# RomanJuranek/librectify

Hardware: AMD Instinct MI355X
Metric: Mpix/s end-to-end (detect+VP) on 4K frames, batch call of 64 frames, 5 in flight (higher is better)
Workload: dtype f32

## Files before the change

### include/librectify_amd.h

```cpp
#pragma once
#include <stddef.h>
#include <stdint.h>

#include "librectify.h"

#if defined(__GNUC__)
#pragma GCC visibility push(default)
#endif

#ifdef __cplusplus
using librectify::ImageTransform;
using librectify::LineSegment;
using librectify::Point;
using librectify::RectificationConfig;
extern "C" {
#endif

typedef struct lr_context lr_context;
enum lr_pixel_format { LR_PIX_U8 = 0, LR_PIX_U8X3 = 1, LR_PIX_F32 = 2 };

int lr_context_create(int device, lr_context** out);
void lr_context_destroy(lr_context* ctx);
void lr_release_thread_context(void);
int lr_context_trim(lr_context* ctx);
// ... 89 lines not shown
                                      d_dst, dst_bytes, 0, 0, 0);
}
static inline size_t lr_jpeg_bound(int width, int height, int format, int layout) {
    size_t mcu, bpm, ri, mcus;
    if (width < 1 || height < 1 || width > 65535 || height > 65535) return 0;
    if (format == LR_PIX_U8 && layout == 0) {
        mcu = 8; bpm = 1; ri = 96;
    } else if (format == LR_PIX_U8X3 && layout == 0) {
        mcu = 16; bpm = 6; ri = 16;
    } else if (format == LR_PIX_U8X3 && layout == 1) {
        mcu = 8; bpm = 3; ri = 32;
    } else {
        return 0;
    }
    mcus = (((size_t)width + mcu - 1) / mcu) * (((size_t)height + mcu - 1) / mcu);
    return 640 + 2 * ((mcus + ri - 1) / ri) + 416 * mcus * bpm;
}

typedef struct lr_jpeg_decode_args {
    const void* h_src;
    const double* frames;
    int32_t* info;
} lr_jpeg_decode_args;
enum lr_warp_jpeg_decode { LR_WARP_JPEG_DECODE = 0x4000 };
static inline int lr_decode_jpeg_device(lr_context* ctx, const void* d_src, const void* h_src, size_t src_bytes, int format,
                                        const double* frames, int batch, void* d_dst, size_t dst_bytes, int32_t* info) {
    lr_jpeg_decode_args a;
    a.h_src = h_src;
    a.frames = frames;
    a.info = info;
    return lr_warp_perspective_device(ctx, d_src, src_bytes, batch, 0, 0, 0, format | LR_WARP_JPEG_DECODE,
                                      (const double*)(const void*)&a, d_dst, dst_bytes, 0, 0, 0);
}
static inline int lr_jpeg_info(const void* h_src, size_t src_bytes, const double* frames, int batch, int32_t* info) {
    return lr_decode_jpeg_device((lr_context*)0, (const void*)0, h_src, src_bytes, LR_PIX_U8X3, frames, batch, (void*)0, 0, info);
}

int lr_stage_filter(lr_context* ctx, const float* d_image, int width, int height, int stride);
int lr_stage_filter_host(lr_context* ctx, const float* buffer, int width, int height, int stride);
int lr_stage_seeds(lr_context* ctx, int* n_seeds);
int lr_stage_flood(lr_context* ctx, int* n_components);
int lr_stage_fit(lr_context* ctx, LineSegment* out, int capacity, int* n_lines);

enum lr_buffer_id {
    LR_BUF_DX = 0,
    LR_BUF_DY = 1,
    LR_BUF_DMASK = 2,
    LR_BUF_LABEL = 3,
    LR_BUF_SEED_IDX = 4,
    LR_BUF_SEED_BIN = 5,
    LR_BUF_SEED_THR = 6,
    LR_BUF_MAXMAG = 7,
    LR_BUF_SEED_SIZE = 8,
};
int lr_download(lr_context* ctx, int buffer_id, void* dst, size_t bytes);

enum lr_stage_id {
    LR_T_UPLOAD = 0,
    LR_T_FILTER = 1,
    LR_T_SEEDS = 2,
    LR_T_FLOOD = 3,
    LR_T_FIT = 4,
    LR_T_RANSAC = 5,
    LR_T_TOTAL = 6,
    LR_T_FILTER_KERNEL = 7,
    LR_T_COUNT = 8,
};
int lr_stage_times(lr_context* ctx, float* ms, int count);
void lr_set_stage_timing(lr_context* ctx, int on);
int lr_filter_kernel_ms(lr_context* ctx, float* ms);
int lr_stage_counters(lr_context* ctx, int64_t* out, int count);

int lr_ransac_best(lr_context* ctx, const LineSegment* lines_norm, int n, const int32_t* indices, int n_idx, float tol,
                   int n_iter, uint64_t seed, uint32_t round, float* best_h3, float* best_score, int* best_iter);
int lr_estimate_line_pencils(lr_context* ctx, LineSegment* lines, int n, int max_models, float inlier_deg,
                             float garbage_deg, int n_iter, uint64_t seed);

int lr_cht_vanishing_point(lr_context* ctx, const LineSegment* lines, int n, int d, Point* vp, uint64_t* acc_out);
int lr_refine_lines(lr_context* ctx, const LineSegment* in, int n, LineSegment* out, int* n_out);

void lr_set_estimator(lr_context* ctx, int kind, int param);
int lr_estimate_line_pencils_cht(lr_context* ctx, LineSegment* lines, int n, int max_models, float inlier_deg,
                                 float garbage_deg, int d, float* models3, int* n_models, uint32_t* peak_cells,
                                 uint64_t* votes);
int lr_ht_weights(lr_context* ctx, const LineSegment* lines_norm, int n, const int32_t* indices, int n_idx, float* weights);
int lr_prosac_solve(lr_context* ctx, const LineSegment* lines_norm, int n, const int32_t* indices, int n_idx, float tol,
                    int T_N, uint64_t seed, uint32_t round, float* h3, int32_t* trace4);
int lr_estimate_line_pencils_prosac(lr_context* ctx, LineSegment* lines, int n, int max_models, float inlier_deg,
                                    float garbage_deg, int T_N, uint64_t seed);
int lr_direct_solve(lr_context* ctx, const LineSegment* lines_norm, int n, const int32_t* indices, int n_idx, float* h3);
int lr_estimate_line_pencils_direct(lr_context* ctx, LineSegment* lines, int n, int max_models, float inlier_deg,
                                    float garbage_deg);

#ifdef __cplusplus
}
#endif

#if defined(__GNUC__)
#pragma GCC visibility pop
#endif
```

### librectify_amd/__init__.py

```python
import ctypes as C
import os

import numpy as np

_HERE = os.path.dirname(os.path.abspath(__file__))
LIB_PATH = os.path.join(_HERE, "librectify_amd.so")

LINE_DTYPE = np.dtype(
    [("x1", "<f4"), ("y1", "<f4"), ("x2", "<f4"), ("y2", "<f4"), ("weight", "<f4"), ("err", "<f4"), ("group_id", "<i4")]
)


class Point(C.Structure):
    _fields_ = [("x", C.c_float), ("y", C.c_float), ("z", C.c_float)]


class ImageTransform(C.Structure):
    _fields_ = [
        ("width", C.c_int),
        ("height", C.c_int),
        ("top_left", Point),
        ("top_right", Point),
        ("bottom_left", Point),
        ("bottom_right", Point),
        ("horizontal_vp", Point),
        ("vertical_vp", Point),
    ]

    def as_array(self):
        pts = [self.top_left, self.top_right, self.bottom_left, self.bottom_right, self.horizontal_vp, self.vertical_vp]
        return np.array([[p.x, p.y, p.z] for p in pts], np.float32)


ROTATE_H, ROTATE_V, RECTIFY, KEEP = 0, 1, 2, 3


class RectificationConfig(C.Structure):
    _fields_ = [
        ("vertical_vp_angular_tolerance", C.c_float),
        ("vertical_vp_min_distance", C.c_float),
        ("v_strategy", C.c_int),
        ("horizontal_vp_min_distance", C.c_float),
        ("h_strategy", C.c_int),
    ]

    def __init__(self, tol=40.0, vmin=1.5, v_strategy=RECTIFY, hmin=1.5, h_strategy=RECTIFY):
        super().__init__(tol, vmin, v_strategy, hmin, h_strategy)


class Frame(C.Structure):
    _fields_ = [("data", C.c_void_p), ("width", C.c_int32), ("height", C.c_int32), ("stride", C.c_int32),
                ("min_length", C.c_float)]


class DrawLinesArgs(C.Structure):
    _fields_ = [("lines", C.c_void_p), ("n_lines", C.c_size_t), ("frames", C.c_void_p), ("H", C.c_void_p)]


class JpegArgs(C.Structure):
    _fields_ = [("frames", C.c_void_p), ("sizes", C.c_void_p)]


class JpegDecodeArgs(C.Structure):
    _fields_ = [("h_src", C.c_void_p), ("frames", C.c_void_p), ("info", C.c_void_p)]


BUF_DX, BUF_DY, BUF_DMASK, BUF_LABEL, BUF_SEED_IDX, BUF_SEED_BIN, BUF_SEED_THR, BUF_MAXMAG, BUF_SEED_SIZE = range(9)
T_UPLOAD, T_FILTER, T_SEEDS, T_FLOOD, T_FIT, T_RANSAC, T_TOTAL, T_FILTER_KERNEL, T_COUNT = range(9)
PIX_U8, PIX_U8X3, PIX_F32 = range(3)
WARP_PREPARE = 0x100
WARP_PACKED = 0x200
WARP_RAGGED = 0x800
WARP_LINES = 0x1000
WARP_JPEG = 0x2000
WARP_JPEG_DECODE = 0x4000
JPEG_OK, JPEG_NOT_JPEG, JPEG_UNSUPPORTED, JPEG_SIZE_MISMATCH, JPEG_DAMAGED = range(5)
FRAMES_U8, FRAMES_U8X3, FRAMES_F32 = 0x100, 0x200, 0x300


def frames_word(fmt, refine=False):
    if fmt not in (PIX_U8, PIX_U8X3, PIX_F32):
        raise ValueError("frames_word: fmt is PIX_U8, PIX_U8X3 or PIX_F32")
    flag = 1 if refine else 0
    return flag if fmt == PIX_F32 else ((fmt + 1) << 8) | flag


def split_frames_word(word):
    word = int(word)
    if word >= 0 and 1 <= (word >> 8) <= 3:
        return (word >> 8) - 1, (word & 0xFF) != 0
    return PIX_F32, word != 0

EXPORTS = [
    "find_line_segment_groups", "release_line_segments", "compute_rectification_transform",
    "compute_rectification_transform_from_vp", "fit_vanishing_point", "assign_to_group",
    "lr_context_create", "lr_context_destroy", "lr_last_error", "lr_synchronize", "lr_set_ransac_seed",
    "lr_set_ransac_iterations", "lr_set_flood_mode", "lr_device_count", "lr_find_line_segment_groups_device",
    "lr_find_line_segment_groups_host", "lr_find_line_segment_groups_batch_device", "lr_stage_filter",
    "lr_stage_filter_host", "lr_stage_seeds", "lr_stage_flood", "lr_stage_fit", "lr_download", "lr_stage_times",
    "lr_stage_counters", "lr_filter_kernel_ms", "lr_ransac_best", "lr_estimate_line_pencils",
    "lr_find_line_segment_groups_batch_host", "lr_find_line_segment_groups_batch_host_ptrs", "lr_host_alloc", "lr_host_free",
    "lr_set_seed_capacity", "lr_set_flood_blind_rounds", "lr_set_flood_staged", "lr_set_batch_streams", "lr_device_malloc", "lr_device_free", "lr_memcpy_h2d", "lr_cht_vanishing_point", "lr_refine_lines", "lr_set_estimator", "lr_ht_weights", "lr_prosac_solve", "lr_estimate_line_pencils_prosac", "lr_direct_solve", "lr_estimate_line_pencils_direct",
    "lr_estimate_line_pencils_cht", "lr_set_stage_timing", "lr_release_thread_context", "lr_set_flood_partial_commits", "lr_set_flood_logs", "lr_set_flood_just_in_time", "lr_set_flood_giant_step", "lr_context_trim", "lr_trim_thread_context",
    "lr_find_line_segment_groups_batch_host_multi", "lr_memcpy_d2h", "lr_rectification_homography", "lr_warp_perspective_device",
]

_lib = None


class LibrectifyError(RuntimeError):
    pass


def lib():
    global _lib
    if _lib is None:
        if not os.path.exists(LIB_PATH):
            raise LibrectifyError(
                "librectify_amd.so is missing: build it with `python -m librectify_amd.build` (hipcc, gfx950); "
                "there is no CPU fallback"
# ... 348 lines not shown
        lib().lr_set_ransac_seed(self._h, C.c_uint64(seed))

    def set_iterations(self, n):
        lib().lr_set_ransac_iterations(self._h, int(n))

    def set_flood_mode(self, mode):
        lib().lr_set_flood_mode(self._h, int(mode))

    def synchronize(self):
        _check(lib().lr_synchronize(self._h))

    def stage_filter_host(self, img):
        img = np.ascontiguousarray(img, np.float32)
        h, w = img.shape
        self.shape = (h, w)
        _check(lib().lr_stage_filter_host(self._h, _ptr(img), w, h, w))

    def stage_filter_device(self, dptr, w, h, stride=None):
        self.shape = (h, w)
        _check(lib().lr_stage_filter(self._h, C.c_void_p(dptr), w, h, stride or w))

    def stage_seeds(self):
        n = C.c_int(0)
        _check(lib().lr_stage_seeds(self._h, C.byref(n)))
        self.n_seeds = n.value
        return n.value

    def stage_flood(self):
        n = C.c_int(0)
        _check(lib().lr_stage_flood(self._h, C.byref(n)))

    def stage_fit(self):
        h, w = self.shape
        cap = h * w // 6 + 16
        out = np.zeros(cap, LINE_DTYPE)
        n = C.c_int(0)
        _check(lib().lr_stage_fit(self._h, _ptr(out), cap, C.byref(n)))
        return out[: n.value].copy()

    def download(self, buf):
        h, w = self.shape
        if buf in (BUF_DX, BUF_DY):
            a = np.zeros((h, w), np.float32)
        elif buf == BUF_DMASK:
            a = np.zeros((h, w), np.uint8)
        elif buf == BUF_LABEL:
            a = np.zeros((h, w), np.int32)
        elif buf in (BUF_SEED_IDX, BUF_SEED_BIN, BUF_SEED_SIZE):
            a = np.zeros(self.n_seeds, np.int32)
        elif buf == BUF_SEED_THR:
            a = np.zeros(self.n_seeds, np.float32)
        elif buf == BUF_MAXMAG:
            a = np.zeros(1, np.float32)
        else:
            raise ValueError(buf)
        if a.nbytes:
            _check(lib().lr_download(self._h, buf, _ptr(a), a.nbytes))
        return a

    def stage_times(self):
        t = np.zeros(T_COUNT, np.float32)
        _check(lib().lr_stage_times(self._h, _ptr(t), T_COUNT))
        return t

    def stage_times_partial(self):
        ms = C.c_float(0)
        _check(lib().lr_filter_kernel_ms(self._h, C.byref(ms)))
        return ms.value

    def stage_counters(self):
        c = np.zeros(16, np.int64)
        _check(lib().lr_stage_counters(self._h, _ptr(c), 16))
        return dict(seeds=int(c[0]), components=int(c[1]), flood_rounds=int(c[2]), labelled_px=int(c[3]),
                    second_tier_seeds=int(c[4]), slabs=int(c[5]), ordered_tail_seeds=int(c[6]), frame_laps=int(c[7]),
                    walked_px=int(c[8]), walk_steps=int(c[9]), log_rewalks=int(c[11]), log_give_ups=int(c[12]), giants_held=int(c[13]), giant_steps=int(c[14]),
                    quiet_round_misses=int(c[15]))

    def find_line_segment_groups(self, img, min_length, refine=False, num_threads=-1, capacity=None):
        img, fmt, _, stride = _host_frame(img, "find_line_segment_groups")
        h, w = img.shape[:2]
        cap = capacity or (h * w // 6 + 16)
        out = np.zeros(cap, LINE_DTYPE)
        n = C.c_int(0)
        self.shape = (h, w)
        _check(lib().lr_find_line_segment_groups_host(self._h, _ptr(img), w, h, stride, min_length, frames_word(fmt, refine), num_threads, _ptr(out), cap, C.byref(n)))
        return out[: min(n.value, cap)].copy()

    def find_line_segment_groups_device(self, dptr, w, h, min_length, refine=False, stride=None, capacity=None, out=None, fmt=PIX_F32):
        cap = capacity or (h * w // 6 + 16)
        if out is None:
            out = np.zeros(cap, LINE_DTYPE)
        n = C.c_int(0)
        self.shape = (h, w)
        _check(lib().lr_find_line_segment_groups_device(self._h, C.c_void_p(dptr), w, h, stride or w, min_length, frames_word(fmt, refine), -1, _ptr(out), cap, C.byref(n)))
        return out[: min(n.value, cap)]

    def device_upload(self, array):
        a = np.ascontiguousarray(array)
        p = C.c_void_p()
        _check(lib().lr_device_malloc(self._h, a.nbytes, C.byref(p)))
        _check(lib().lr_memcpy_h2d(self._h, p, _ptr(a), a.nbytes))
        return p.value

    def device_free(self, ptr):
        _check(lib().lr_device_free(self._h, C.c_void_p(ptr)))

# ... 793 lines not shown
```

### librectify_amd/csrc/api.cpp

```cpp
#include <cstdio>
#include <cstdlib>
#include <cstring>
#include <memory>
#include <new>
#include <stdexcept>
#include <string>

#include "context.h"

using namespace lramd;

namespace {

struct CtxDeleter {
    void operator()(lr_context* c) const { ctx_destroy(c); }
};

std::unique_ptr<lr_context, CtxDeleter>& thread_context_slot() {
    thread_local std::unique_ptr<lr_context, CtxDeleter> ctx;
    return ctx;
}

lr_context* thread_context() {
    std::unique_ptr<lr_context, CtxDeleter>& ctx = thread_context_slot();
// ... 404 lines not shown
            set_error("image smaller than the 5x5 filter");
            return 1;
        }
        if (upload_host_image(ctx, buffer, width, height, stride, -1)) return 1;
        return ctx_stage_filter(ctx, ctx->frames.slot[0], width, height, width);
    } catch (...) {
        return guard_fail("lr_stage_filter_host");
    }
}
int lr_stage_seeds(lr_context* ctx, int* n_seeds) {
    try {
        if (ctx_stage_seeds(ctx)) return 1;
        if (n_seeds) *n_seeds = (int)ctx->n_seeds;
        return 0;
    } catch (...) {
        return guard_fail("lr_stage_seeds");
    }
}
int lr_stage_flood(lr_context* ctx, int* n_components) {
    try {
        if (ctx_stage_flood(ctx)) return 1;
        LR_HIP(hipStreamSynchronize(ctx->stream));
        if (n_components) *n_components = -1;
        return 0;
    } catch (...) {
        return guard_fail("lr_stage_flood");
    }
}
int lr_stage_fit(lr_context* ctx, LineSegment* out, int capacity, int* n_lines) {
    try {
        std::vector<LineSegment> res;
        if (ctx_stage_fit(ctx, res)) return 1;
        return copy_out(res, out, capacity, n_lines);
    } catch (...) {
        return guard_fail("lr_stage_fit");
    }
}

int lr_download(lr_context* ctx, int buffer_id, void* dst, size_t bytes) {
    try {
        const size_t npix = (size_t)ctx->w * ctx->h;
        const void* src = nullptr;
        size_t have = 0;
        switch (buffer_id) {
            case LR_BUF_DX: src = ctx->ws.dx; have = npix * 4; break;
            case LR_BUF_DY: src = ctx->ws.dy; have = npix * 4; break;
            case LR_BUF_DMASK: src = ctx->ws.dmask; have = npix; break;
            case LR_BUF_LABEL: src = ctx->ws.label; have = npix * 4; break;
            case LR_BUF_SEED_IDX: src = ctx->ws.seed_idx; have = (size_t)ctx->n_seeds * 4; break;
            case LR_BUF_SEED_BIN: src = ctx->ws.seed_bin; have = (size_t)ctx->n_seeds * 4; break;
            case LR_BUF_SEED_THR: src = ctx->ws.seed_thr; have = (size_t)ctx->n_seeds * 4; break;
            case LR_BUF_MAXMAG: src = ctx->maxmag; have = 4; break;
            case LR_BUF_SEED_SIZE: src = ctx->ws.seed_size; have = (size_t)ctx->n_seeds * 4; break;
            default: set_error("lr_download: unknown buffer id"); return 1;
        }
        if (buffer_id == LR_BUF_DMASK && ctx->dmask_consumed) {
            set_error("lr_download: LR_BUF_DMASK was consumed by lr_stage_flood (labelled pixels are cleared); download it after lr_stage_filter");
            return 1;
        }
        if (bytes > have) {
            set_error("lr_download: request larger than the buffer");
            return 1;
        }
        LR_HIP(hipSetDevice(ctx->device));
        LR_HIP(hipStreamSynchronize(ctx->stream));
        LR_HIP(hipMemcpy(dst, src, bytes, hipMemcpyDeviceToHost));
        return 0;
    } catch (...) {
        return guard_fail("lr_download");
    }
}

int lr_filter_kernel_ms(lr_context* ctx, float* ms) {
    try {
        LR_HIP(hipStreamSynchronize(ctx->stream));
        LR_HIP(hipEventElapsedTime(ms, ctx->ev[0], ctx->ev[1]));
        return 0;
    } catch (...) {
        return guard_fail("lr_filter_kernel_ms");
    }
}

int lr_stage_times(lr_context* ctx, float* ms, int count) {
    try {
        for (int i = 0; i < count && i < LR_T_COUNT; ++i) ms[i] = ctx->stage_ms[i];
        return 0;
    } catch (...) {
        return guard_fail("lr_stage_times");
    }
}

int lr_stage_counters(lr_context* ctx, int64_t* out, int count) {
    try {
        const int64_t v[16] = {(int64_t)ctx->n_seeds,        (int64_t)ctx->n_comp,         (int64_t)ctx->flood_rounds,
                               (int64_t)ctx->n_px,           (int64_t)ctx->flood_tiers[0], (int64_t)ctx->flood_tiers[1],
                               (int64_t)ctx->flood_tiers[2], (int64_t)ctx->frame_laps,
                               (int64_t)(((uint64_t)ctx->flood_tiers[5] << 32) | ctx->flood_tiers[4]),
                               (int64_t)(((uint64_t)ctx->flood_tiers[7] << 32) | ctx->flood_tiers[6]),
                               0 , (int64_t)ctx->flood_tiers[10], (int64_t)ctx->flood_tiers[11], (int64_t)ctx->flood_tiers[12],
                               (int64_t)ctx->flood_tiers[13], (int64_t)ctx->flood_tiers[15]};
        for (int i = 0; i < count && i < 16; ++i) out[i] = v[i];
        return 0;
    } catch (...) {
        return guard_fail("lr_stage_counters");
    }
}
// ... 162 lines not shown
```

### librectify_amd/csrc/common.h

```cpp
#pragma once
#include <hip/hip_runtime.h>

#include <cstdint>
#include <string>

#include "../../include/librectify_amd.h"

namespace lramd {

constexpr float kEps = 1e-6f;
constexpr int kMaxModels = 4;
constexpr int kMaxPeelModels = 5;
constexpr float kInlierDeg = 2.0f;
constexpr float kGarbageDeg = 4.0f;
constexpr int kRansacMaxIter = 10000;
constexpr int kEdgeKernelSize = 2;
constexpr float kEdgeKernelSigma = 1.0f;
constexpr int kSeedDist = 2;
constexpr float kSeedRatio = 0.95f;
constexpr float kTraceTolerance = 0.25f;
constexpr float kLineMaxErr = 2.0f;
constexpr float kLineMinLength = 5.f;
constexpr int kComponentMinSize = 5;
constexpr int kBins = 8;
// ... 22 lines not shown
__host__ __device__ inline float directional(float dx, float dy, float s, float c) {
    return fabsf(fmaf(dx, s, dy * c));
}

__host__ __device__ inline uint64_t splitmix64(uint64_t x) {
    x += 0x9E3779B97F4A7C15ull;
    x = (x ^ (x >> 30)) * 0xBF58476D1CE4E5B9ull;
    x = (x ^ (x >> 27)) * 0x94D049BB133111EBull;
    return x ^ (x >> 31);
}
__host__ __device__ inline void sample_pair(uint64_t seed, uint32_t round, uint32_t iter, uint32_t n, uint32_t& a,
                                            uint32_t& b) {
    const uint64_t z = splitmix64(seed ^ splitmix64(((uint64_t)round << 32) | iter));
    const uint32_t u1 = (uint32_t)z, u2 = (uint32_t)(z >> 32);
    const uint32_t i = (uint32_t)(((uint64_t)u1 * n) >> 32);
    uint32_t j = (uint32_t)(((uint64_t)u2 * (n - 1)) >> 32);
    if (j >= i) ++j;
    a = i < j ? i : j;
    b = i < j ? j : i;
}

void set_error(const std::string& msg);

#define LR_HIP(expr)                                                                                     \
    do {                                                                                                 \
        hipError_t _e = (expr);                                                                          \
        if (_e != hipSuccess) {                                                                          \
            (void)hipGetLastError();        \
            ::lramd::set_error(std::string(#expr) + ": " + hipGetErrorString(_e) + " (" + __FILE__ + ":" + \
                               std::to_string(__LINE__) + ")");                                          \
            return 1;                                                                                    \
        }                                                                                                \
    } while (0)

inline int pix_bytes(int format) { return format == LR_PIX_U8 ? 1 : format == LR_PIX_U8X3 ? 3 : format == LR_PIX_F32 ? 4 : 0; }
int launch_filter(const void* img, int format, int w, int h, int stride, const FilterConsts& fc, float* dx, float* dy,
                  uint8_t* dmask, uint64_t* cand, uint32_t* cand_count, uint32_t* tile_max, hipStream_t s);
int filter_band_rows();
int filter_band_last_row(int by);
int launch_filter_rows(const void* img, int format, int w, int h, int stride, const FilterConsts& fc, float* dx, float* dy,
                       uint8_t* dmask, uint64_t* cand, uint32_t* cand_count, uint32_t* tile_max, int by_begin, int by_end,
                       hipStream_t s);
struct FilterGeom {
    int n_tiles;
    int cand_cap;
};
FilterGeom filter_geometry(int w, int h);

size_t seeds_temp_bytes(int n_tiles, size_t max_seeds);
int launch_seed_select(const uint64_t* cand, const uint32_t* cand_count, const uint32_t* tile_max, int n_tiles,
                       int cand_cap, float seed_keep_ratio, float* maxmag, uint32_t* tile_pass, uint32_t* tile_off, uint64_t* keys,
                       uint32_t key_cap, uint32_t* n_seeds, uint32_t frame_tag, hipStream_t s);
int launch_seed_order(uint64_t* keys, uint64_t* keys_alt, const uint32_t* n_seeds, uint32_t cap, const float* dx, const float* dy,
                      BinTrig trig, float trace_tolerance, int32_t* seed_idx, int32_t* seed_bin, float* seed_thr, hipStream_t s);

int launch_label_init(uint32_t* label, size_t n, hipStream_t s);
int launch_flood_ordered(const float* dx, const float* dy, const uint8_t* dmask, int w, int h, const int32_t* seed_idx,
                         const int32_t* seed_bin, const float* seed_thr, const uint32_t* d_n_seeds, uint32_t seed_cap,
                         BinTrig trig, uint32_t* label, int32_t* seed_size, int32_t* queue, hipStream_t s);

constexpr size_t kFloodHandWords = 1024;
struct FloodBuffers {
    uint32_t* blocked = nullptr;
    uint32_t* count = nullptr;
    uint32_t* flags = nullptr;
    uint8_t* state = nullptr;
    uint8_t* tier = nullptr;
    uint32_t* blk = nullptr;
    uint32_t* act_a = nullptr;
    uint32_t* act_b = nullptr;
    uint32_t* ctrl = nullptr;
    uint8_t* dirty = nullptr;
    uint32_t* big_list = nullptr;
    uint32_t* handover = nullptr;
    bool rewalk_logs = false;
    uint32_t* rewalk_list = nullptr;
    int log_min_tiles = 0, log_walk_tiles = 0;
    bool giant_hold = false;
    bool giant_step = true;
    void* giant_mask = nullptr;
    uint32_t* giant_parent = nullptr;
    bool log_sweep = false;
    bool rewalk_big = false;
    uint32_t log_seeds = 0, log_cap = 0;
    uint32_t* log_off = nullptr;
    uint32_t* log_len = nullptr;
    uint32_t* log_buf = nullptr;
    void* slab_ring = nullptr;
    void* slab_hash = nullptr;
    uint32_t n_slabs = 0, slab_ring_cap = 0, slab_hash_cap = 0;
    int win_first_shift = 0, win_growth = 2;
    int win_hold_pct = 80;
    bool partial_commits = true;
    bool second_tier = true;
    bool second_tier_from_start = true;
    bool hold_from_start = false;
    bool staged_from_start = false;
    int blind_rounds = 10;
    uint32_t* host_progress = nullptr;
    bool calm_hint = false;
    uint32_t* host_ctrl = nullptr;
    int jit_first = 0;
    int jit_sleep_us = 0;
    uint32_t big_cap_override = 0;
    uint32_t team_tile_cap = 0;
};
struct FloodFrame {
    const float* dx;
    const float* dy;
    const uint8_t* dmask;
    int w, h;
    const int32_t* seed_idx;
    const int32_t* seed_bin;
    const float* seed_thr;
    const uint32_t* d_n_seeds;
    uint32_t seed_cap;
    BinTrig trig;
    uint32_t* label;
    int32_t* seed_size;
    int32_t* queue;
};
struct FloodProgress {
    int enqueued = 0;
    bool use_big = false;
    int win_growth = 2;
    bool sizes_known = false;
    uint32_t max_flood = 0;
};
constexpr int kFloodCtrlWords = 56;
int flood_enqueue(const FloodBuffers& B, const FloodFrame& F, FloodProgress* P, uint32_t* h_ctrl, hipStream_t s);
int flood_finish(const FloodBuffers& B, const FloodFrame& F, FloodProgress* P, uint32_t* h_ctrl, int* rounds_out,
                 uint32_t* tiers_out ,
                 bool* extra, hipStream_t s);

size_t fit_temp_bytes(size_t max_pixels, uint32_t max_segments);
struct HugeSort {
    uint32_t* tab = nullptr;
    uint32_t* list = nullptr;
    uint32_t* jobs = nullptr;
    uint32_t max = 0;
};
int launch_component_offsets(const int32_t* seed_size, const uint32_t* d_n_seeds, uint32_t seed_cap, int min_size,
                             uint32_t* comp_rank, uint32_t* comp_seed, uint32_t* comp_off,
                             uint32_t* totals , uint32_t* large_list, uint32_t large_cap,
                             uint32_t* n_large, void* temp, size_t temp_bytes, uint32_t frame_tag, uint32_t* cursor, const HugeSort& hs,
                             hipStream_t s);
int launch_component_scatter(const uint32_t* label, size_t npix, const uint32_t* comp_rank, const uint32_t* comp_off,
                             uint32_t* cursor, uint32_t* px, const HugeSort& hs, uint32_t* n_large, bool with_huge, hipStream_t s);
int launch_component_sort(const uint32_t* px_in, uint32_t* px_out, const uint32_t* comp_off, const uint32_t* d_n_comp,
                          uint32_t comp_cap, const uint32_t* large_list, uint32_t large_cap, const uint32_t* n_large,
                          uint32_t* scratch, const uint32_t* cursor, const HugeSort& hs, bool with_huge, hipStream_t s);
int launch_fit(const uint32_t* px_sorted, const uint32_t* px_unsorted, const uint32_t* comp_off, const uint32_t* comp_seed, const uint32_t* d_n_comp,
               uint32_t comp_cap, const int32_t* seed_bin, const float* dx, const float* dy, int w, BinTrig trig,
               float* scratch_w, LineSegment* out, const uint32_t* cursor, const HugeSort& hs, const uint32_t* n_large, bool with_huge,
               hipStream_t s);

struct PencilSoA {
    const float* ax;
    const float* ay;
    const float* dx;
    const float* dy;
    const float* len;
    const float* hx;
    const float* hy;
    const float* hz;
};
constexpr int kRansacBestSlots = 32;
int launch_ransac_score(PencilSoA m, uint32_t n, float tol, float degeneracy_tol, uint32_t n_iter, uint64_t seed,
                        uint32_t round, unsigned long long* best_slots, uint32_t* host_best, hipStream_t s);
int launch_ransac_score_dev(PencilSoA m, const uint32_t* gctl, int max_models, float tol, float degeneracy_tol,
                            uint32_t n_iter, uint64_t seed, unsigned long long* best_slots, hipStream_t s);

struct PencilTable {
// ... 45 lines not shown
```

### librectify_amd/csrc/context.h

```cpp
#pragma once
#include <atomic>
#include <functional>
#include <memory>
#include <mutex>
#include <vector>

#include "buffers.h"
#include "common.h"
#include "vp_host.h"

namespace lramd {
struct StagingCrew;

struct Settings {
    uint64_t ransac_seed = 0;
    int ransac_iters = kRansacMaxIter;
    int estimator = 0;
    int prosac_T_N = -1;
    int cht_d = 128;
    int batch_streams = 5;
    int flood_mode = 1;
    bool flood_giant_step = true;
    bool flood_jit = true;
    bool flood_partial = true;
    bool flood_log_sweep = false;
    bool flood_logs = true;
    bool flood_staged = false;
    bool timing_on = false;
};


struct Workspace {
    size_t cap_pix = 0;
    int cap_tiles = 0;
    DeviceBuffer<float> dx, dy;
    DeviceBuffer<uint8_t> dmask;
    DeviceBuffer<uint64_t> cand;
    DeviceBuffer<uint32_t> cand_count, tile_max;
    DeviceBuffer<uint32_t> tile_pass;
    DeviceBuffer<uint32_t> tile_off;
    DeviceBuffer<uint64_t> keys_a, keys_b;
    DeviceBuffer<int32_t> seed_idx, seed_bin;
    DeviceBuffer<float> seed_thr;
    DeviceBuffer<int32_t> seed_size;
    DeviceBuffer<uint32_t> label;
    DeviceBuffer<int32_t> queue;
    DeviceBuffer<uint32_t> comp_rank, comp_seed, comp_off, cursor, px_a, px_b;
    DeviceBuffer<float> scratch_w;
    DeviceBuffer<LineSegment> d_lines;
    DeviceBuffer<unsigned char> temp;
    DeviceBuffer<uint32_t> comp_large;
    DeviceBuffer<uint32_t> huge_tab, huge_list, huge_jobs;
    HugeSort huge;
};

struct FloodStore {
    DeviceBuffer<uint32_t> blocked, count, flags, blk, act_a, act_b, ctrl, big_list, handover, rewalk_list, log_off, log_len, log_buf;
    DeviceBuffer<uint8_t> state, tier, dirty;
    DeviceBuffer<uint64_t> giant_mask;
    DeviceBuffer<uint4> slab_ring, slab_hash;
    FloodBuffers fb;
    size_t cap_seeds = 0;
};

struct FrameSlots {
    DeviceBuffer<float> slot[2];
    PinnedBuffer<float> stage[2];
    DeviceBuffer<float> packed;
    DeviceBuffer<float> luma;
};

struct UploadRing {
    std::vector<DeviceBuffer<float>> img;
    std::vector<PinnedBuffer<float>> stage;
    size_t cap_pix = 0, stage_cap_pix = 0;
    void drop() {
        for (auto& b : img) b.reset();
        for (auto& b : stage) b.reset();
        cap_pix = stage_cap_pix = 0;
    }
};

struct PrepareSpans {
    MirroredBuffer<unsigned char> spans;
    int key[4] = {0, 0, 0, 0};
    float w_in[2] = {0.f, 0.f};
    MirroredBuffer<unsigned char> ragged;
};

struct OverlayStore {
    MirroredBuffer<unsigned char> block;
};

struct JpegStore {
    MirroredBuffer<unsigned char> block;
    DeviceBuffer<int16_t> coef;
// ... 195 lines not shown
```

### librectify_amd/csrc/context.hip

```cpp
#include "host.h"

#include <cmath>
#include <cstdlib>

#ifndef M_PI
#define M_PI 3.14159265358979323846
#endif

lr_context::lr_context() = default;
lr_context::~lr_context() = default;

namespace lramd {

namespace {

thread_local std::string g_error;

void gauss_deriv_factors(int size, float sigma, float* d, float* g) {
    const int n = 2 * size + 1;
    for (int t = 0; t < n; ++t) {
        const float x = float(t - size);
        const float a = float(2 * M_PI * std::pow(sigma, 4.0f));
        const float e = std::exp(-std::pow(x, 2.0f) / (2 * std::pow(sigma, 2.0f)));
        d[t] = x / a * e;
// ... 27 lines not shown
    if (frames_too) {
        c->frames = FrameSlots{};
        c->ring.drop();
        c->prep = PrepareSpans{};
        c->warp_m = MirroredBuffer<double>{};
        c->overlay = OverlayStore{};
        c->jpeg = JpegStore{};
        c->jpeg_decode = JpegDecodeStore{};
    }
    c->small_frames = 0;
    c->w = c->h = 0;
    c->seed_cap = 0;
    c->flood_hold_hint = c->flood_staged_hint = c->flood_calm_hint = false;
    c->flood_staged_streak = 0;
    for (bool& v : c->stage_valid) v = false;
    if (frames_too)
        for (lr_context* wc : c->workers)
            if (ctx_trim(wc, true)) return 1;
    return 0;
}

int ctx_ensure_image_capacity(lr_context* c, int w, int h) {
    const size_t npix = (size_t)w * h;
    if (c->w != 0 && (c->w != w || c->h != h)) {
        c->flood_hold_hint = false;
        c->flood_staged_hint = false;
        c->flood_calm_hint = false;
        c->flood_staged_streak = 0;
    }
    const FilterGeom fg = filter_geometry(w, h);
    const int ntiles = fg.n_tiles;
    if (!c->keep_workspace) {
        if (c->ws.cap_pix != 0 && npix * 4 <= c->ws.cap_pix) {
            if (++c->small_frames >= 8 && ctx_trim(c, false)) return 1;
        } else {
            c->small_frames = 0;
        }
    }
    return ctx_reserve_workspace(c, npix, ntiles);
}

int ctx_reserve_workspace(lr_context* c, size_t npix, int ntiles) {
    const FilterGeom fg = filter_geometry(5, 5);
    if (npix <= c->ws.cap_pix && ntiles <= c->ws.cap_tiles) return 0;
    LR_HIP(hipStreamSynchronize(c->stream));
    const size_t cp = std::max(npix, c->ws.cap_pix);
    const int ct = std::max(ntiles, c->ws.cap_tiles);
    const size_t tile_off_words = std::max(ct, 2);
    Workspace& s = c->ws;
    s.cap_pix = 0;
    s.cap_tiles = 0;
    if (s.dx.grow(cp) || s.dy.grow(cp) || s.dmask.grow(cp + 16) || s.cand.grow((size_t)ct * fg.cand_cap) || s.cand_count.grow(ct) ||
        s.tile_max.grow(ct) || s.tile_pass.grow(ct) || s.tile_off.grow(tile_off_words) || s.keys_a.grow(cp) || s.keys_b.grow(cp) ||
        s.seed_idx.grow(cp) || s.seed_bin.grow(cp) || s.seed_thr.grow(cp) || s.seed_size.grow(cp) || s.label.grow(cp) ||
        s.queue.grow(cp) || s.comp_rank.grow(cp) || s.comp_seed.grow(cp) || s.comp_off.grow(cp + 1) || s.cursor.grow(cp) ||
        s.px_a.grow(cp) || s.px_b.grow(cp) || s.scratch_w.grow(cp) || s.d_lines.grow(cp / 6 + 16) || s.comp_large.grow(cp / 64 + 16))
        return 1;
    LR_HIP(hipMemsetAsync(s.tile_off, 0, tile_off_words * sizeof(uint32_t), c->stream));
    {
        const size_t nb = (cp + 16383) >> 14;
        const uint32_t max = 256;
        if (s.huge_tab.grow(max * nb) || s.huge_jobs.grow(4 * max * nb) || s.huge_list.grow(max)) return 1;
        s.huge = HugeSort{s.huge_tab, s.huge_list, s.huge_jobs, max};
        LR_HIP(hipMemsetAsync(s.huge.tab, 0, max * nb * sizeof(uint32_t), c->stream));
    }
    const size_t tb = std::max(seeds_temp_bytes(ct, cp), fit_temp_bytes(cp, (uint32_t)std::min<size_t>(cp / 6 + 16, 0xFFFFFFFFu)));
    if (s.temp.grow(tb)) return 1;
    LR_HIP(hipMemsetAsync(s.temp, 0, tb, c->stream));
    s.cap_pix = cp;
    s.cap_tiles = ct;
    return 0;
}

template <class T, class P>
static int grow_into(DeviceBuffer<T>& own, P*& raw, size_t count) {
    raw = nullptr;
    if (own.grow(count)) return 1;
    raw = own.get();
    return 0;
}

static int ensure_flood_slabs(lr_context* c) {
    FloodBuffers& f = c->flood.fb;
    static const bool giant_step_off = std::getenv("LIBRECTIFY_FLOOD_GIANT_STEP") && std::atoi(std::getenv("LIBRECTIFY_FLOOD_GIANT_STEP")) == 0;
    uint32_t want = (c->opt.flood_mode == 1 && c->opt.flood_giant_step && !giant_step_off) ? 16u : 128u;
    if (const char* e = std::getenv("LIBRECTIFY_FLOOD_SLABS")) want = (uint32_t)std::max(1, std::atoi(e));
    if (f.slab_ring && f.n_slabs >= want) return 0;
    LR_HIP(hipStreamSynchronize(c->stream));
    f.n_slabs = want;
    f.slab_ring_cap = 1u << 14;
    f.slab_hash_cap = 1u << 16;
    if (grow_into(c->flood.slab_ring, f.slab_ring, (size_t)f.n_slabs * f.slab_ring_cap) ||
        grow_into(c->flood.slab_hash, f.slab_hash, (size_t)f.n_slabs * f.slab_hash_cap * 2))
        return 1;
    LR_HIP(hipMemsetAsync(f.slab_hash, 0, (size_t)f.n_slabs * f.slab_hash_cap * 32, c->stream));
    if (f.ctrl) LR_HIP(hipMemsetAsync(f.ctrl, 0, kFloodCtrlWords * sizeof(uint32_t), c->stream));
    return 0;
}

int ensure_flood_buffers(lr_context* c) {
    FloodStore& o = c->flood;
    FloodBuffers& f = o.fb;
    if (c->flood.cap_seeds >= c->ws.cap_pix && f.ctrl) return ensure_flood_slabs(c);
    LR_HIP(hipStreamSynchronize(c->stream));
    const size_t cs = c->ws.cap_pix;
    if (grow_into(o.blocked, f.blocked, cs) || grow_into(o.count, f.count, cs) || grow_into(o.flags, f.flags, cs) ||
        grow_into(o.state, f.state, cs) || grow_into(o.tier, f.tier, cs) || grow_into(o.blk, f.blk, cs) ||
        grow_into(o.act_a, f.act_a, cs) || grow_into(o.act_b, f.act_b, cs) || grow_into(o.ctrl, f.ctrl, kFloodCtrlWords) ||
        grow_into(o.big_list, f.big_list, 8192) || grow_into(o.handover, f.handover, 8192 * kFloodHandWords) ||
        grow_into(o.dirty, f.dirty, cs / 256 + 16) ||
        grow_into(o.giant_mask, f.giant_mask, cs / 16 + 64))
        return 1;
    constexpr size_t kLogCapDiv = 8;
    f.log_seeds = (uint32_t)std::min<size_t>(std::max<size_t>(cs / 16, 4096), cs);
    f.log_cap = (uint32_t)std::min<size_t>(std::max<size_t>(cs / kLogCapDiv, 65536), 1u << 28);
    if (grow_into(o.rewalk_list, f.rewalk_list, 8192) || grow_into(o.log_off, f.log_off, f.log_seeds) ||
        grow_into(o.log_len, f.log_len, f.log_seeds) || grow_into(o.log_buf, f.log_buf, (size_t)f.log_cap * 3))
        return 1;
    LR_HIP(hipMemsetAsync(f.ctrl, 0, kFloodCtrlWords * sizeof(uint32_t), c->stream));
    o.cap_seeds = cs;
    return ensure_flood_slabs(c);
}


int ctx_ensure_ransac_capacity(lr_context* c, size_t n_lines) {
    if (8 * n_lines <= c->model.cap()) return 0;
    LR_HIP(hipStreamSynchronize(c->stream));
    return c->model.grow(8 * std::max<size_t>(n_lines, 4096));
}

int ensure_group_capacity(lr_context* c, size_t n_lines) {
    if (n_lines > c->cap_glines) {
        LR_HIP(hipStreamSynchronize(c->stream));
        const size_t cl = std::max<size_t>(n_lines, 4096);
        c->cap_glines = 0;
        if (c->d_tables.grow(3 * 8 * cl) || c->d_orig.grow(3 * cl) || c->d_inl.grow(4 * cl)) return 1;
        c->cap_glines = cl;
    }
    if (n_lines > c->d_flines.cap()) {
        LR_HIP(hipStreamSynchronize(c->stream));
        if (c->d_flines.grow(n_lines + 16)) return 1;
    }
    return 0;
}

int ctx_create(int device, lr_context** out) {
    int ndev = 0;
    if (hipGetDeviceCount(&ndev) != hipSuccess || ndev <= 0) {
        set_error("no HIP device available: librectify_amd has no CPU fallback");
        return 1;
    }
    if (device < 0 || device >= ndev) {
        set_error("device index out of range");
        return 1;
    }
    LR_HIP(hipSetDevice(device));
    lr_context* c = new lr_context();
    c->device = device;
    if (hipStreamCreateWithFlags(c->stream.put(), hipStreamNonBlocking) != hipSuccess) {
        delete c;
// ... 60 lines not shown
```

### librectify_amd/csrc/frame.hip

```cpp
#include "host.h"

#include <cstdio>
#include <cstdlib>
#include <cstring>

namespace lramd {


namespace {

uint32_t round_up(uint32_t v, uint32_t m) { return (v + m - 1) / m * m; }

uint32_t initial_seed_cap(size_t npix) {
    return (uint32_t)std::min<size_t>(npix, std::max<size_t>(round_up((uint32_t)(npix / 32), 1024), 4096));
}

uint32_t line_cap_for(const lr_context* c) {
    return (uint32_t)std::min<size_t>(c->seed_cap, c->ws.cap_pix / 6 + 16);
}


PencilTable table_of(lr_context* c, int which) {
    const size_t cl = c->cap_glines;
    float* b = c->d_tables + (size_t)which * 8 * cl;
// ... 3 lines not shown

int ensure_result_block(lr_context* c, size_t lines) {
    if (lines <= c->res_lines_cap && c->h_res) return 0;
    LR_HIP(hipStreamSynchronize(c->stream));
    if (c->h_res.grow(kResHeaderBytes + lines * sizeof(LineSegment))) return 1;
    c->res_lines_cap = lines;
    return 0;
}

FloodBuffers flood_buffers_for(lr_context* c) {
    FloodBuffers fbuf = c->flood.fb;
    if (c->opt.flood_mode >= 2 && c->opt.flood_mode <= 4) fbuf.second_tier = false;
    fbuf.second_tier_from_start = c->flood_big_hint;
    fbuf.hold_from_start = c->flood_hold_hint;
    fbuf.staged_from_start = c->flood_staged_hint;
    if (c->opt.flood_mode == 2) fbuf.n_slabs = 0;
    if (c->opt.flood_mode == 3) fbuf.n_slabs = 2;
    if (c->opt.flood_mode == 5) {
        fbuf.n_slabs = 0;
        fbuf.big_cap_override = 1;
    }
    if (c->opt.flood_mode == 6) fbuf.team_tile_cap = 200;
    if (c->opt.flood_mode == 7) {
        fbuf.team_tile_cap = 200;
        fbuf.n_slabs = 0;
    }
    static const bool partial_off = std::getenv("LIBRECTIFY_FLOOD_PARTIAL") && std::atoi(std::getenv("LIBRECTIFY_FLOOD_PARTIAL")) == 0;
    fbuf.partial_commits = !partial_off && c->opt.flood_partial;
    fbuf.rewalk_logs = c->opt.flood_logs;
    fbuf.log_sweep = c->opt.flood_log_sweep;
    fbuf.log_min_tiles = c->flood_log_min;
    fbuf.log_walk_tiles = c->flood_log_walk;
    fbuf.giant_hold = c->opt.flood_mode == 1;
    static const bool giant_step_off = std::getenv("LIBRECTIFY_FLOOD_GIANT_STEP") && std::atoi(std::getenv("LIBRECTIFY_FLOOD_GIANT_STEP")) == 0;
    fbuf.giant_step = !giant_step_off && c->opt.flood_giant_step;
    fbuf.giant_parent = reinterpret_cast<uint32_t*>(c->ws.queue.get());
    fbuf.rewalk_big = c->flood_logbig_hint && !c->flood_logbig_off;
    if (c->opt.flood_staged) fbuf.win_first_shift = 3;
    fbuf.blind_rounds = c->flood_rounds_hint;
    static const bool jit_off = std::getenv("LIBRECTIFY_FLOOD_JIT") && std::atoi(std::getenv("LIBRECTIFY_FLOOD_JIT")) == 0;
    static_assert(16 + kFloodCtrlWords <= 72, "the control block's copy ends where the report word begins");
    fbuf.host_progress = c->h_counts + 72;
    fbuf.host_ctrl = c->h_counts + 16;
    static const int calm_hint_env = std::getenv("LIBRECTIFY_FLOOD_CALM_HINT") ? std::atoi(std::getenv("LIBRECTIFY_FLOOD_CALM_HINT")) : 1;
    fbuf.calm_hint = calm_hint_env != 0 && c->flood_calm_hint;
    fbuf.jit_sleep_us = c->flood_jit_sleep_us;
    constexpr int kJitFirstMax = 4;
    fbuf.jit_first = (c->opt.flood_jit && !jit_off) ? std::min(c->flood_rounds_last > 0 ? std::max(c->flood_rounds_last - 1, 2) : 3, kJitFirstMax) : 0;
    return fbuf;
}

FloodFrame flood_frame_for(lr_context* c) {
    return FloodFrame{c->ws.dx, c->ws.dy, c->ws.dmask, c->w, c->h, c->ws.seed_idx, c->ws.seed_bin, c->ws.seed_thr,
                      c->d_counts + kCntSeeds, c->seed_cap, c->trig, c->ws.label, c->ws.seed_size, c->ws.queue};
}

int prepare_frame(lr_context* c, int w, int h) {
    LR_HIP(hipSetDevice(c->device));
    if (w < 5 || h < 5) {
        set_error("image smaller than the 5x5 filter");
        return 1;
    }
    if (ctx_ensure_image_capacity(c, w, h)) return 1;
    if (c->w != w || c->h != h || c->seed_cap == 0) c->seed_cap = initial_seed_cap((size_t)w * h);
    if (c->seed_cap_once) {
        c->seed_cap = (uint32_t)std::min<size_t>((size_t)w * h, c->seed_cap_once);
        c->seed_cap_once = 0;
    }
    c->w = w;
    c->h = h;
    c->n_seeds = c->n_comp = c->n_px = 0;
    c->dmask_consumed = false;
    for (bool& v : c->stage_valid) v = false;
    return 0;
}

int enqueue_filter(lr_context* c, const void* d_image, int format, int w, int h, int stride) {
    if (prepare_frame(c, w, h)) return 1;
    const size_t bpp = (size_t)pix_bytes(format);
    if (bpp == 0 || d_image == nullptr || stride < w) {
        set_error(bpp == 0 ? "unknown pixel format of the frames" : "launch_filter: bad geometry");
        return 1;
    }
    const size_t npix = (size_t)w * h;
    if (format == LR_PIX_U8X3) {
        if (npix >= ((size_t)1 << 29)) {
            set_error("launch_filter: image larger than 2^29 pixels is not supported (seed key packs index in 29 bits)");
            return 1;
        }
        if (c->frames.luma.cap() < npix) {
            LR_HIP(hipStreamSynchronize(c->stream));
            if (c->frames.luma.grow(npix)) return 1;
        }
        if (ctx_prepare_frames(c, d_image, 0, 1, w, h, (size_t)stride * bpp, LR_PIX_U8X3, c->frames.luma.get(), 0, w, h, (size_t)w * sizeof(float)))
            return 1;
        d_image = c->frames.luma.get();
        format = LR_PIX_F32;
        stride = w;
    }
    const size_t fbpp = (size_t)pix_bytes(format);
    if (stride > w && (uint64_t)w * (uint64_t)h < (1ull << 29) &&
        ((uint64_t)(h - 1) * (uint64_t)stride + (uint64_t)w) * fbpp >= (1ull << 32)) {
        if (c->frames.packed.cap() < npix) {
            LR_HIP(hipStreamSynchronize(c->stream));
            if (c->frames.packed.grow(npix)) return 1;
        }
        LR_HIP(hipMemcpy2DAsync(c->frames.packed, (size_t)w * fbpp, d_image, (size_t)stride * fbpp,
                                (size_t)w * fbpp, (size_t)h, hipMemcpyDeviceToDevice, c->stream));
        d_image = c->frames.packed;
        stride = w;
    }
    if (c->opt.timing_on) LR_HIP(hipEventRecord(c->ev[0], c->stream));
    if (launch_filter(d_image, format, w, h, stride, c->fconsts, c->ws.dx, c->ws.dy, c->ws.dmask, c->ws.cand, c->ws.cand_count, c->ws.tile_max,
                      c->stream))
        return 1;
    if (c->opt.timing_on) LR_HIP(hipEventRecord(c->ev[1], c->stream));
    return 0;
}

int enqueue_seeds(lr_context* c) {
    const FilterGeom fg = filter_geometry(c->w, c->h);
    if (launch_seed_select(c->ws.cand, c->ws.cand_count, c->ws.tile_max, fg.n_tiles, fg.cand_cap, c->seed_keep_ratio, c->maxmag,
                           c->ws.tile_pass, c->ws.tile_off, c->ws.keys_a, c->seed_cap, c->d_counts + kCntSeeds, ++c->select_tag ? c->select_tag : ++c->select_tag,
                           c->stream))
        return 1;
    if (launch_seed_order(c->ws.keys_a, c->ws.keys_b, c->d_counts + kCntSeeds, c->seed_cap, c->ws.dx, c->ws.dy, c->trig, kTraceTolerance,
                          c->ws.seed_idx, c->ws.seed_bin, c->ws.seed_thr, c->stream))
        return 1;
    if (c->opt.timing_on) LR_HIP(hipEventRecord(c->ev[2], c->stream));
    return 0;
}

int enqueue_flood(lr_context* c) {
    const size_t npix = (size_t)c->w * c->h;
    c->flood_rounds = 1;
    if (c->opt.flood_mode == 0) {
        if (launch_label_init(c->ws.label, npix, c->stream)) return 1;
        if (launch_flood_ordered(c->ws.dx, c->ws.dy, c->ws.dmask, c->w, c->h, c->ws.seed_idx, c->ws.seed_bin, c->ws.seed_thr,
                                 c->d_counts + kCntSeeds, c->seed_cap, c->trig, c->ws.label, c->ws.seed_size, c->ws.queue, c->stream))
            return 1;
    } else {
        if (ensure_flood_buffers(c)) return 1;
        if (flood_enqueue(flood_buffers_for(c), flood_frame_for(c), &c->flood_prog, c->h_counts + 16, c->stream)) return 1;
        c->stage_valid[0] = c->stage_valid[1] = false;
        c->dmask_consumed = true;
    }
    if (c->opt.timing_on) LR_HIP(hipEventRecord(c->ev[3], c->stream));
    return 0;
}

int finish_flood(lr_context* c, bool* extra) {
    *extra = false;
    if (c->opt.flood_mode == 0) return 0;
    if (flood_finish(flood_buffers_for(c), flood_frame_for(c), &c->flood_prog, c->h_counts + 16, &c->flood_rounds,
                     c->flood_tiers, extra, c->stream))
        return 1;
    static const bool call_debug = std::getenv("LIBRECTIFY_CALL_DEBUG") != nullptr;
    if (call_debug)
        std::fprintf(stderr, "flood: %d rounds, %u walks in the second tier, %u of them long, hold-back phase %u (started with it: %d)\n",
                     c->flood_rounds, c->flood_tiers[0], c->flood_tiers[8], c->flood_tiers[3], (int)c->flood_hold_hint);
    c->flood_logbig_hint = c->flood_tiers[0] > 0;
    c->flood_calm_hint = c->flood_tiers[0] == 0 && c->flood_tiers[1] == 0 && c->flood_tiers[15] == 0;
    c->flood_big_hint = true;
    c->flood_hold_hint = c->flood_tiers[3] != 0 && c->flood_tiers[8] >= 16;
    constexpr uint32_t kStagedKeep = 64;
    c->flood_staged_hint = c->flood_tiers[14] != 0 && (!c->flood_staged_hint || c->flood_tiers[0] >= kStagedKeep);
    c->flood_staged_streak = c->flood_staged_hint ? c->flood_staged_streak + 1 : 0;
    if (c->flood_staged_streak >= 16) {
        c->flood_staged_hint = false;
        c->flood_staged_streak = 0;
    }
    if (c->flood_staged_hint) c->flood_hold_hint = false;

    c->flood_rounds_hint = std::max(std::max(c->flood_rounds + 2, 6), c->flood_rounds_hint - 1);
    c->flood_rounds_last = c->flood_rounds;
    return 0;
}

int enqueue_fit(lr_context* c) {
    const size_t npix = (size_t)c->w * c->h;
// ... 435 lines not shown
```

### librectify_amd/csrc/kernels_flood.hip

```cpp
#include <algorithm>
#include <atomic>
#include <chrono>
#include <cstdio>
#include <cstdlib>
#include <cstring>
#include <thread>
#include <sys/prctl.h>
#include <vector>

#include "common.h"

namespace lramd {
namespace {

__device__ inline uint32_t ld_agent(const uint32_t* p) {
    return __hip_atomic_load(p, __ATOMIC_RELAXED, __HIP_MEMORY_SCOPE_AGENT);
}

__global__ __launch_bounds__(256) void label_init_kernel(uint32_t* __restrict__ label, size_t n) {
    size_t i = (size_t)blockIdx.x * 256 + threadIdx.x;
    const size_t step = (size_t)gridDim.x * 256;
    for (; i < n; i += step) label[i] = kLabelFree;
}

// ... 55 lines not shown
}

}

int launch_label_init(uint32_t* label, size_t n, hipStream_t s) {
    const int blocks = (int)((n + 255) / 256 < 4096 ? (n + 255) / 256 : 4096);
    hipLaunchKernelGGL(label_init_kernel, dim3(blocks > 0 ? blocks : 1), dim3(256), 0, s, label, n);
    LR_HIP(hipGetLastError());
    return 0;
}

int launch_flood_ordered(const float* dx, const float* dy, const uint8_t* dmask, int w, int h, const int32_t* seed_idx,
                         const int32_t* seed_bin, const float* seed_thr, const uint32_t* d_n_seeds, uint32_t seed_cap,
                         BinTrig trig, uint32_t* label, int32_t* seed_size, int32_t* queue, hipStream_t s) {
    (void)h;
    if (seed_cap == 0) return 0;
    hipLaunchKernelGGL(flood_ordered_kernel, dim3(1), dim3(64), 0, s, dx, dy, dmask, w, seed_idx, seed_bin, seed_thr,
                       d_n_seeds, seed_cap, trig, label, seed_size, queue);
    LR_HIP(hipGetLastError());
    return 0;
}

namespace {


constexpr uint32_t kMarkBit = 0x80000000u;
#ifndef LR_RING_T
#define LR_RING_T 128
#endif
#ifndef LR_HASH_T
#define LR_HASH_T 256
#endif
constexpr int kRingT = LR_RING_T, kHashT = LR_HASH_T;
constexpr int kHashBig = 2048;
constexpr uint32_t kHandTiles = kHashT * 3 / 4, kHandRecs = kRingT;
constexpr uint32_t kHandTable = 4, kHandRing = kHandTable + 3 * kHandTiles;
static_assert(kHandRing + 3 * kHandRecs <= kFloodHandWords, "hand-over record");
constexpr uint32_t kBigCap = 8192;
constexpr uint32_t kFlagIncomplete = 1u, kFlagSelfFail = 2u;
constexpr uint32_t kHugeFlood = 1u << 14;
constexpr uint32_t kFullTiles = 48u;
constexpr uint32_t kGiantProbes = 512u;
constexpr uint32_t kLogShrunk = 0x80000000u;
constexpr uint32_t kMaxSteps = 1u << 22;
constexpr uint32_t kTeamTiles = 1024;
constexpr uint32_t kGiantMany = 64;
constexpr uint32_t kDeferSteps = 512;
constexpr uint32_t kRegionalTiles = 32;
constexpr uint32_t kRegionalMin = 16;
constexpr uint32_t kHoldMinBig = 4;
constexpr uint32_t kHoldRelease = 64;
constexpr uint32_t kPartialSteps = 16;
constexpr int kPartialRounds = 3;
constexpr uint32_t kDenseDiv = 12;
constexpr uint32_t kLogMinTiles = 16;
constexpr uint32_t kLogWalkTiles = 12;

struct FloodArgs {
    const float* dx;
    const float* dy;
    const uint8_t* dmask;
    int w, h, tiles_x;
    const int32_t* seed_idx;
    const int32_t* seed_bin;
    const float* seed_thr;
    uint32_t* label;
    uint32_t* blocked;
    uint32_t* count;
    uint32_t* flags;
    uint8_t* tier;
    uint32_t* ctrl;
    uint8_t* dirty;
    uint4* slab_ring;
    uint4* slab_hash;
    uint32_t n_slabs, slab_ring_cap, slab_hash_cap;
    uint32_t win_shift;
    uint32_t no_rest;
    uint32_t next_reach;
    uint32_t big_cap;
    uint32_t* handover;
    uint32_t team_tiles;
    uint32_t* blk;
    uint32_t wide_tiles, wide_front;
    uint32_t giant_many;
    uint32_t* rewalk_list;
    uint32_t log_min_tiles;
    uint32_t log_walk_tiles;
    uint32_t log_use;
    uint32_t log_max_len;
    uint32_t log_sweep;
    uint32_t* host_progress;
    uint32_t* host_ctrl;
    uint32_t quiet;
    uint32_t giant_hold;
    uint32_t log_seeds;
    uint32_t* log_off;
    uint32_t* log_len;
    uint32_t* log_buf;
    uint32_t log_cap;
    uint32_t giant_step;
    uint32_t* act_a;
    uint32_t* act_b;
    unsigned long long* giant_mask;
    uint32_t* giant_parent;
};
enum {
    kCtrlBarrier = 0,
    kCtrlSlabs = 1,
    kCtrlNAct = 2,
    kCtrlNCommit = 3,
    kCtrlNNext = 4,
    kCtrlPhase = 5,
    kCtrlDone = 6,
    kCtrlRounds = 7,
    kCtrlGen = 8,
    kCtrlStall = 9,
    kCtrlNRemain = 10,
    kCtrlWindow = 11,
    kCtrlNBig = 12,
    kCtrlBigTotal = 13,
    kCtrlSlabTotal = 14,
    kCtrlBelow = 15,
    kCtrlNSeeds = 16,
    kCtrlWinHold = 17,
    kCtrlWalked = 18,
    kCtrlSteps = 20,
    kCtrlBigSeen = 22,
    kCtrlBarrierNext = 24,
    kCtrlBigLong = 23,
    kCtrlNRewalk = 26,
    kCtrlLogTotal = 28,
    kCtrlLogWalks = 29,
    kCtrlLogGiveUp = 30,
    kCtrlLowest = 31,
    kCtrlLowestNext = 32,
    kCtrlGiantLow = 33,
    kCtrlGiantLowNext = 34,
    kCtrlGiantRuled = 35,
    kCtrlGiants = 36,
    kCtrlGiantCountNext = 37,
    kCtrlGiantStep = 38,
    kCtrlGiantDone = 39,
    kCtrlGiantPx = 40,
    kCtrlGiantBlocks = 41,
    kCtrlMaxFlood = 43,
    kCtrlStaged = 44,
    kCtrlDeferLow = 45,
    kCtrlDeferLowNext = 46,
    kCtrlWindowFree = 42,
    kCtrlQuietMiss = 47,
    kCtrlTeamDone = 48,
    kCtrlTeamGiants = 49,
    kCtrlGiantReuse = 52,
    kCtrlWords = 56,
};
static_assert(kCtrlWords == kFloodCtrlWords, "control block size");

__device__ __forceinline__ uint32_t uni(uint32_t v) { return (uint32_t)__builtin_amdgcn_readfirstlane((int)v); }
__device__ __forceinline__ uint64_t uni64(uint32_t lo, uint32_t hi) { return ((uint64_t)uni(hi) << 32) | uni(lo); }
__device__ __forceinline__ uint64_t m_eq(uint32_t a, uint32_t b) { return __builtin_amdgcn_uicmp(a, b, 32); }
__device__ __forceinline__ uint64_t m_ne(uint32_t a, uint32_t b) { return __builtin_amdgcn_uicmp(a, b, 33); }
__device__ __forceinline__ uint64_t m_ne64(uint64_t a, uint64_t b) { return __builtin_amdgcn_uicmpl(a, b, 33); }
__device__ __forceinline__ uint64_t m_lt_s(int a, int b) { return __builtin_amdgcn_sicmp(a, b, 40); }
__device__ __forceinline__ uint64_t m_ge_s(int a, int b) { return __builtin_amdgcn_sicmp(a, b, 39); }
__device__ __forceinline__ uint64_t m_gt_s(int a, int b) { return __builtin_amdgcn_sicmp(a, b, 38); }
__device__ __forceinline__ uint64_t m_gt_f(float a, float b) { return __builtin_amdgcn_fcmpf(a, b, 2); }
__device__ __forceinline__ bool lane_of(uint64_t mask) { return __builtin_amdgcn_inverse_ballot_w64(mask); }
__device__ __forceinline__ uint64_t uni64(uint64_t v) { return uni64((uint32_t)v, (uint32_t)(v >> 32)); }

__device__ __forceinline__ bool giants_many(const uint32_t* ctrl, uint32_t giant_many) {
    const uint32_t n_seeds = uni(ctrl[kCtrlNSeeds]);
    return giant_many != 0u && uni(ctrl[kCtrlStaged]) == 0u && uni(ctrl[kCtrlRounds]) == 0u && n_seeds >= 8192u &&
           uni(ctrl[kCtrlWindow]) > (n_seeds >> 2) && uni(ld_agent(&ctrl[kCtrlGiants])) >= giant_many;
}
__device__ __forceinline__ bool giants_all(const uint32_t* ctrl) {
    if (uni(ctrl[kCtrlRounds]) != 0u) return false;
    const uint32_t g = uni(ld_agent(&ctrl[kCtrlTeamGiants])), t = uni(ld_agent(&ctrl[kCtrlTeamDone]));
    return g >= 64u && g * 8u >= t * 7u;
}
__device__ __forceinline__ const uint32_t* act_now(const FloodArgs& A) { return (uni(A.ctrl[kCtrlRounds]) & 1u) ? A.act_b : A.act_a; }
__device__ __forceinline__ uint32_t* act_other(const FloodArgs& A) { return (uni(A.ctrl[kCtrlRounds]) & 1u) ? A.act_a : A.act_b; }
__device__ __forceinline__ bool giant_pending(const FloodArgs& A) { return uni(A.ctrl[kCtrlGiantStep]) != 0u; }

struct WalkState {
    uint32_t head, tail, cnt, ntiles;
    bool blocked;
    uint32_t steps;
    uint32_t fresh;
    uint32_t blocker = 0xFFFFFFFFu;
};

template <int kRing, int kHash, typename OrdT>
struct LdsStoreT {
    static constexpr bool kDeferStamps = true;
    static constexpr int kRingN = kRing, kHashN = kHash;
    static constexpr int kHashShift = 32 - __builtin_ctz((unsigned)kHash);
    uint32_t* rt;
    uint32_t* rlo;
    uint32_t* rhi;
    uint32_t* hk;
    uint32_t* hv0;
    uint32_t* hv1;
    OrdT* ord;
    __device__ void note_new(uint32_t i, uint32_t slot) { ord[i] = (OrdT)slot; }
    __device__ uint32_t ring_cap() const { return kRing; }
    __device__ uint32_t hash_limit() const { return kHash * 3 / 4; }
    __device__ void get(uint32_t i, uint32_t& tile, uint64_t& m) const {
        const uint32_t j = i & (kRing - 1);
        tile = uni(rt[j]);
        m = uni64(rlo[j], rhi[j]);
    }
    __device__ void put(uint32_t i, uint32_t tile, uint64_t m) {
        const uint32_t j = i & (kRing - 1);
        rt[j] = tile;
        rlo[j] = (uint32_t)m;
        rhi[j] = (uint32_t)(m >> 32);
    }
    __device__ bool lookup(uint32_t tile, uint32_t& slot, uint64_t& V) const {
        const uint32_t key = tile + 1u;
        uint32_t hs = (key * 2654435761u) >> kHashShift;
        uint32_t cur = uni(hk[hs]);
        if (cur != key && cur != 0u) {
            for (int probe = 1; probe < kHash && cur != key && cur != 0u; ++probe) {
                hs = (hs + 1) & (kHash - 1);
                cur = uni(hk[hs]);
            }
        }
        slot = hs;
        V = 0ull;
        if (cur != key) return false;
        V = uni64(hv0[hs], hv1[hs]);
        return true;
    }
    __device__ void value(uint32_t slot, uint64_t& V) const { V = uni64(hv0[slot], hv1[slot]); }
    __device__ void update(uint32_t slot, uint32_t tile, uint64_t V) {
        hk[slot] = tile + 1u;
        hv0[slot] = (uint32_t)V;
        hv1[slot] = (uint32_t)(V >> 32);
    }
};

using LdsStore = LdsStoreT<kRingT, kHashT, uint8_t>;
// ... 47 lines not shown
        slot = hs;
        V = 0ull;
        return false;
    }
    __device__ void value(uint32_t slot, uint64_t& V) const {
        const uint4 v = ld(&hash[2 * slot]);
        V = uni64(v.z, v.w);
    }
    __device__ void update(uint32_t slot, uint32_t tile, uint64_t V) {
        st(&hash[2 * slot], make_uint4(gen, tile + 1u, (uint32_t)V, (uint32_t)(V >> 32)));
        __builtin_amdgcn_fence(__ATOMIC_RELEASE, "workgroup");
    }
};

constexpr int kPend = 64;
struct Pending {
    uint32_t* pt;
    uint32_t* pi;
    template <class Store>
    __device__ __forceinline__ void push(Store& S, WalkState& st, uint32_t tile, uint64_t m) {
        const uint32_t hs = ((tile + 1u) * 2654435761u) >> 26;
        const uint32_t idx = uni(pi[hs]);
        if (uni(pt[hs]) == tile + 1u && (int32_t)(idx - st.head) >= 0 && (int32_t)(st.tail - idx) > 0) {
            uint32_t t2;
            uint64_t m2;
            S.get(idx, t2, m2);
            if (t2 == tile) {
                S.put(idx, tile, m2 | m);
                return;
            }
        }
        S.put(st.tail, tile, m);
        pt[hs] = tile + 1u;
        pi[hs] = st.tail;
        st.tail += 1;
    }
};

__device__ __forceinline__ uint64_t spread_col(uint64_t b) {
    b = (b | (b << 28)) & 0x0000000F0000000Full;
    b = (b | (b << 14)) & 0x0003000300030003ull;
    b = (b | (b << 7)) & 0x0101010101010101ull;
    return b;
}

struct PushLane {
    uint32_t off;
    uint32_t shamt;
    uint32_t msk;
    uint32_t sh;
    bool spread;
    bool dl;
};
__device__ __forceinline__ PushLane push_lane(int lane) {
    const int d = lane & 7;
    const int dy = (d < 2) ? (d == 0 ? -1 : 1) : (d < 4 ? 0 : (d < 6 ? -1 : 1));
    const int dx = (d < 2) ? 0 : ((d & 1) ? 1 : -1);
    PushLane c;
    c.off = (uint32_t)(dy * 0x10000 + dx);
    c.shamt = (d < 4) ? 8u * (uint32_t)d : 32u + (uint32_t)(d - 4);
    c.msk = (d < 4) ? 0xFFu : 1u;
    c.sh = (uint32_t)((0x0007383F00070038ull >> (8 * d)) & 0xFFull);
    c.spread = d == 2 || d == 3;
    c.dl = lane < 8;
    asm volatile("" : "+v"(c.off), "+v"(c.shamt), "+v"(c.msk), "+v"(c.sh));
    return c;
}

struct Forward {
    bool valid;
    uint32_t tile, slot;
    uint64_t entry;
    bool known;
};

template <int kRing, int kHash, typename OrdT>
__device__ __forceinline__ void push8(LdsStoreT<kRing, kHash, OrdT>& S, Pending& P, WalkState& st, uint32_t tile,
                                      uint64_t H, int lane, const PushLane& c, Forward& fw) {
    const uint32_t nt = tile + c.off;
    const uint32_t key = nt + 1u;
    const uint64_t src = (H >> c.shamt) & (uint64_t)c.msk;
    uint64_t E = (c.spread ? spread_col(src) : src) << c.sh;
    uint32_t ts = (key * 2654435761u) >> LdsStoreT<kRing, kHash, OrdT>::kHashShift;
    const uint32_t hs = (key * 2654435761u) >> 26;
    uint32_t hk0 = S.hk[ts];
    uint32_t v0 = S.hv0[ts], v1 = S.hv1[ts];
    const uint32_t pt = P.pt[hs], pi = P.pi[hs];
    const uint64_t m_want = m_ne64(E, 0ull) & 0xFFull;
    uint64_t m_found = m_eq(hk0, key);
    uint64_t m_search = m_want & ~m_found & m_ne(hk0, 0u);
    for (int probe = 1; probe < kHash && m_search != 0ull; ++probe) {
        if (lane_of(m_search)) {
            ts = (ts + 1) & (kHash - 1);
            hk0 = S.hk[ts];
        }
        const uint64_t hit = m_search & m_eq(hk0, key);
        if (lane_of(hit)) {
            v0 = S.hv0[ts];
            v1 = S.hv1[ts];
        }
        m_found |= hit;
        m_search &= ~hit & m_ne(hk0, 0u);
    }
    if (lane_of(m_found)) E &= ~(((uint64_t)v1 << 32) | v0);
    const uint64_t m_active = m_want & m_ne64(E, 0ull);
    const uint64_t m_merge = m_active & m_eq(pt, key) & m_ge_s((int32_t)(pi - st.head), 0) & m_gt_s((int32_t)(st.tail - pi), 0);
    if (m_merge != 0ull) {
        if (lane_of(m_merge)) {
            const uint32_t j = pi & (kRing - 1);
            atomicOr(&S.rlo[j], (uint32_t)E);
            atomicOr(&S.rhi[j], (uint32_t)(E >> 32));
        }
    }
    const uint64_t mf = m_active & ~m_merge;
    if (mf != 0ull) {
        if (lane_of(mf)) {
            const uint32_t pos = st.tail + __builtin_amdgcn_mbcnt_hi((uint32_t)(mf >> 32), __builtin_amdgcn_mbcnt_lo((uint32_t)mf, 0u));
            const uint32_t j = pos & (kRing - 1);
            S.rt[j] = nt;
            S.rlo[j] = (uint32_t)E;
            S.rhi[j] = (uint32_t)(E >> 32);
            P.pt[hs] = key;
            P.pi[hs] = pos;
        }
        const int f = __builtin_ctzll(mf);
        fw.valid = true;
        fw.tile = (uint32_t)__builtin_amdgcn_readlane((int)nt, f);
        fw.slot = (uint32_t)__builtin_amdgcn_readlane((int)ts, f);
        fw.entry = ((uint64_t)(uint32_t)__builtin_amdgcn_readlane((int)(uint32_t)(E >> 32), f) << 32) |
                   (uint32_t)__builtin_amdgcn_readlane((int)(uint32_t)E, f);
        fw.known = (m_found >> f) & 1ull;
    }
    st.tail += (uint32_t)__popcll(mf);
}

__device__ __forceinline__ void push8(SlabStore& S, Pending& P, WalkState& st, uint32_t tile, uint64_t H, int lane,
                                      const PushLane& c, Forward& fw) {
    (void)lane;
    (void)c;
    (void)fw;
    const uint64_t up = H & 0xFFull, dn = (H >> 8) & 0xFFull, lf = (H >> 16) & 0xFFull, rt = (H >> 24) & 0xFFull;
    auto send = [&](uint32_t nt, uint64_t E) {
        uint32_t slot;
        uint64_t V;
        if (S.lookup(nt, slot, V)) E &= ~V;
        if (E != 0ull) P.push(S, st, nt, E);
    };
    if (up) send(tile - 0x10000u, up << 56);
    if (dn) send(tile + 0x10000u, dn);
    if (lf) send(tile - 1u, spread_col(lf) << 7);
    if (rt) send(tile + 1u, spread_col(rt));
    if ((H >> 32) & 1ull) send(tile - 0x10001u, 1ull << 63);
    if ((H >> 33) & 1ull) send(tile - 0xFFFFu, 1ull << 56);
    if ((H >> 34) & 1ull) send(tile + 0xFFFFu, 1ull << 7);
    if ((H >> 35) & 1ull) send(tile + 0x10001u, 1ull);
}

__device__ __forceinline__ void ring_xy(int lane, int& rx, int& ry) {
    const int g = lane >> 3, i = lane & 7;
    rx = (g == 0 || g == 1) ? i : (g == 2 ? -1 : (g == 3 ? 8 : ((i & 1) ? 8 : -1)));
    ry = (g == 0) ? -1 : (g == 1 ? 8 : ((g == 2 || g == 3) ? i : ((i & 2) ? 8 : -1)));
}
__device__ __forceinline__ uint64_t ring_adjacency(int lane) {
    if (lane >= 36) return 0ull;
    int rx, ry;
    ring_xy(lane, rx, ry);
    uint64_t m = 0ull;
    for (int dy = -1; dy <= 1; ++dy)
        for (int dx = -1; dx <= 1; ++dx) {
            const int x = rx + dx, y = ry + dy;
            if (x >= 0 && x < 8 && y >= 0 && y < 8) m |= 1ull << (y * 8 + x);
        }
    return m;
}
__device__ __forceinline__ uint64_t tile_neighbours(int lane) {
    const int lr = lane >> 3, lc = lane & 7;
    uint64_t m = 0ull;
    for (int dy = -1; dy <= 1; ++dy)
        for (int dx = -1; dx <= 1; ++dx) {
            const int x = lc + dx, y = lr + dy;
            if (x >= 0 && x < 8 && y >= 0 && y < 8) m |= 1ull << (y * 8 + x);
        }
    return m;
}
struct TileFetch {
    uint32_t tile, slot;
    uint64_t entry, V;
    size_t q;
    float dx, dy, rdx, rdy;
    uint32_t dm, rdm;
    uint32_t lab, rlab;
    bool known;
    uint64_t inside, rinside;
};

__device__ __forceinline__ uint32_t ld32(const uint32_t* p, uint32_t idx) {
    return *reinterpret_cast<const uint32_t*>(reinterpret_cast<const char*>(p) + (idx << 2));
}
__device__ __forceinline__ float ldf(const float* p, uint32_t idx) {
    return *reinterpret_cast<const float*>(reinterpret_cast<const char*>(p) + (idx << 2));
}
__device__ __forceinline__ uint32_t ld8(const uint8_t* p, uint32_t idx) { return p[idx]; }

struct LaneGeom {
    uint32_t off, roff;
};

template <int kMode, class Store>
__device__ __forceinline__ TileFetch fetch_tile(const FloodArgs& A, const Store& S, uint32_t i, int lr, int lc,
                                                int rx, int ry, bool ring_lane, const Forward& fw,
                                                const LaneGeom& G, bool own) {
    TileFetch f;
    if (fw.valid) {
        f.tile = fw.tile;
        f.entry = fw.entry;
    } else {
        S.get(i, f.tile, f.entry);
    }
    const int ty = (int)(f.tile >> 16), tx = (int)(f.tile & 0xFFFFu);
    const uint32_t base = (uint32_t)(ty * 8) * (uint32_t)A.w + (uint32_t)(tx * 8);
    f.inside = m_lt_s(ty * 8 + lr, A.h) & m_lt_s(tx * 8 + lc, A.w);
    const uint32_t q = lane_of(f.inside) ? base + G.off : 0u;
    f.q = q;
    f.dm = 0u;
    f.dx = f.dy = 0.f;
    f.lab = kLabelFree;
    if constexpr (kMode == 0) {
        f.dm = ld8(A.dmask, q);
        f.dx = ldf(A.dx, q);
        f.dy = ldf(A.dy, q);
    }
    if (kMode == 1 || own) f.lab = ld32(A.label, q);
    const int rr = ty * 8 + ry, rc = tx * 8 + rx;
    f.rinside = __builtin_amdgcn_uicmp((uint32_t)rr, (uint32_t)A.h, 36) & __builtin_amdgcn_uicmp((uint32_t)rc, (uint32_t)A.w, 36) &
                0xFFFFFFFFFull;
    const uint32_t rq = lane_of(f.rinside) ? base + G.roff : 0u;
    f.rdm = 0u;
    f.rdx = f.rdy = 0.f;
    f.rlab = kLabelFree;
    if constexpr (kMode == 0) {
        f.rdm = ld8(A.dmask, rq);
        f.rdx = ldf(A.dx, rq);
        f.rdy = ldf(A.dy, rq);
    }
    if (kMode == 1 || own) f.rlab = ld32(A.label, rq);
    if (fw.valid) {
        f.slot = fw.slot;
        f.known = fw.known;
        f.V = 0ull;
        if (f.known) S.value(f.slot, f.V);
    } else {
        f.known = S.lookup(f.tile, f.slot, f.V);
    }
    return f;
}

#ifdef LR_WALK_TIMING
__device__ unsigned long long g_walk_timing[8];
#define LR_TICK(i)                                        \
    {                                                     \
        const uint64_t t_ = __builtin_amdgcn_s_memtime(); \
        tacc[i] += t_ - tlast;                            \
        tlast = t_;                                       \
    }
#else
#define LR_TICK(i)
#endif

template <class Store, int kMode = 0>
__device__ int walk(const FloodArgs& A, uint32_t k, int b, float thr, float sn, float cs, Store& S, Pending& P,
                    WalkState& st, int lane, bool own = false, uint8_t* dmask_rw = nullptr, uint32_t tile_cap = 0xFFFFFFFFu,
                    uint32_t wide_tiles = 0xFFFFFFFFu, uint32_t wide_front = 0xFFFFFFFFu) {
    const uint32_t mine = kMarkBit | k;
    const int lr = lane >> 3, lc = lane & 7;
    int rx, ry;
    ring_xy(lane, rx, ry);
    const bool ring_lane = lane < 36;
    const uint64_t adj = ring_adjacency(lane);
    uint64_t nbr = tile_neighbours(lane);
    asm volatile("" : "+v"(nbr));
    if (st.head == st.tail) return 0;
    const uint32_t tile_limit = min(S.hash_limit(), tile_cap);
    if ((st.tail - st.head) + 8u > S.ring_cap() || st.ntiles + 2u > tile_limit) return 1;
    const PushLane pc = push_lane(lane);
    const uint32_t bin_bit = 1u << b;
    Forward fw;
    fw.valid = false;
    LaneGeom G;
    G.off = (uint32_t)(lr * A.w + lc);
    G.roff = (uint32_t)(ry * A.w + rx);
    asm volatile("" : "+v"(G.off), "+v"(G.roff));
    TileFetch cur = fetch_tile<kMode>(A, S, st.head, lr, lc, rx, ry, ring_lane, fw, G, own);
#ifdef LR_WALK_TIMING
    uint64_t tacc[5] = {0, 0, 0, 0, 0}, tlast = __builtin_amdgcn_s_memtime();
    uint32_t nknown = 0;
#endif
    for (;;) {
        st.head += 1;
        st.steps += 1;
#ifdef LR_WALK_TIMING
        nknown += cur.known ? 1u : 0u;
#endif
        const uint32_t tile = cur.tile;
        uint64_t Am, Rg;
        if constexpr (kMode == 0) {
            Am = cur.inside & m_ne(cur.dm & bin_bit, 0u) & m_gt_f(directional(cur.dx, cur.dy, sn, cs), thr);
            Rg = cur.rinside & m_ne(cur.rdm & bin_bit, 0u) & m_gt_f(directional(cur.rdx, cur.rdy, sn, cs), thr);
            if (own) {
                Am |= cur.inside & m_eq(cur.lab, k);
                Rg |= cur.rinside & m_eq(cur.rlab, k);
            }
        } else {
            Am = cur.inside & (m_eq(cur.lab, mine) | m_eq(cur.lab, k));
            Rg = cur.rinside & (m_eq(cur.rlab, mine) | m_eq(cur.rlab, k));
        }
        LR_TICK(0)
        uint64_t R = cur.entry & Am;
        uint64_t New = 0ull;
        if (R != 0ull) {
            const uint64_t reach = lane_of(Am) ? nbr : 0ull;
            for (;;) {
                const uint64_t R1 = m_ne64(R & reach, 0ull);
                R = m_ne64(R1 & reach, 0ull);
                if (R == R1) break;
            }
            New = R & ~cur.V;
        }
        LR_TICK(1)
        if (New != 0ull || !cur.known) {
            S.update(cur.slot, tile, cur.V | New);
            if (!cur.known) {
                S.note_new(st.ntiles, cur.slot);
                st.ntiles += 1;
            }
        }
        st.cnt += (uint32_t)__popcll(New);
        if constexpr (kMode == 1) {
            const uint64_t fresh = New & m_eq(cur.lab, mine);
            if (lane_of(fresh)) {
                A.label[cur.q] = k;
                dmask_rw[cur.q] = 0;
            }
            st.fresh += (uint32_t)__popcll(fresh);
        }
// ... 50 lines not shown
#pragma unroll
        for (int j = 0; j < 8; ++j) {
            old[j] = kLabelFree;
            const uint32_t i = i0 + (uint32_t)j;
            if (i < st.ntiles) {
                const uint32_t slot = S.ord[i];
                const uint32_t tile = S.hk[slot] - 1u;
                const uint64_t V = ((uint64_t)S.hv1[slot] << 32) | S.hv0[slot];
                if ((V >> lane) & 1ull) {
                    const size_t q = (size_t)((tile >> 16) * 8 + lr) * A.w + ((tile & 0xFFFFu) * 8 + lc);
                    old[j] = atomicMin(&A.label[q], mine);
                    A.dirty[q >> 8] = 1;
                }
            }
        }
#pragma unroll
        for (int j = 0; j < 8; ++j) {
            if (old[j] > mine) {
                if (old[j] != kLabelFree) A.blocked[old[j] & ~kMarkBit] = 1u;
            } else if (old[j] < mine && old[j] >= kMarkBit) {
                foreign = true;
                fmin = min(fmin, old[j] & ~kMarkBit);
            }
        }
    }
    if (__ballot(foreign)) {
        st.blocked = true;
#pragma unroll
        for (int off = 32; off >= 1; off >>= 1) fmin = min(fmin, (uint32_t)__shfl_xor((int)fmin, off));
        st.blocker = min(st.blocker, fmin);
    }
}

template <class Lds>
__device__ __forceinline__ void save_log(const FloodArgs& A, uint32_t k, const Lds& S, uint32_t ntiles, int lane) {
    uint32_t off = 0u;
    if (lane == 0) off = atomicAdd(&A.ctrl[kCtrlLogTotal], ntiles);
    off = (uint32_t)__shfl((int)off, 0);
    if (off + ntiles > A.log_cap || off + ntiles < off) return;
    uint32_t* rec = A.log_buf + (size_t)off * 3u;
    for (uint32_t i = (uint32_t)lane; i < ntiles; i += 64u) {
        const uint32_t slot = S.ord[i];
        rec[3u * i] = S.hk[slot] - 1u;
        rec[3u * i + 1u] = S.hv0[slot];
        rec[3u * i + 2u] = S.hv1[slot];
    }
    if (lane == 0) {
        A.log_off[k] = off;
        A.log_len[k] = ntiles;
    }
}

__device__ __forceinline__ void explore_seed(const FloodArgs& A, const BinTrig& trig, uint32_t k, LdsStore& L, Pending& P,
                                             uint32_t* __restrict__ big_list, int lane, uint32_t t1_tiles) {
    const int s = (int)uni((uint32_t)A.seed_idx[k]);
    const int b = (int)uni((uint32_t)A.seed_bin[k]);
    const float thr = __uint_as_float(uni(__float_as_uint(A.seed_thr[k])));
    const float sn = trig.st[b], cs = trig.ct[b];
    const uint32_t seed_label = A.label[s];
    const uint32_t seed_mask = A.dmask[s];
    const float seed_dx = A.dx[s], seed_dy = A.dy[s];
    const bool own = seed_label == k;
    if (seed_label < kMarkBit && !own) return;
    if ((uni((uint32_t)A.tier[k]) & 8u) != 0u) return;
    if (!own && !(((seed_mask >> b) & 1) && directional(seed_dx, seed_dy, sn, cs) > thr)) {
        if (lane == 0) A.flags[k] = kFlagSelfFail;
        return;
    }
    WalkState st{0u, 1u, 0u, 0u, false, 0u, 0u};
    int rc = 1;
    const bool outgrown = A.big_cap != 0u && (uni((uint32_t)A.tier[k]) & 1u) != 0u && uni(A.ctrl[kCtrlStaged]) == 0u;
    const uint32_t log_w = (A.log_min_tiles != 0xFFFFFFFFu && k < A.log_seeds) ? uni(A.log_len[k]) : 0u;
    const uint32_t log_n = log_w & ~kLogShrunk;
    const bool has_log = log_n != 0u && log_n <= A.log_max_len && A.log_use != 0u;
    const bool skip_first = outgrown && !has_log;
    if (!skip_first) {
        for (int i = lane; i < LdsStore::kHashN; i += 64) L.hk[i] = 0u;
        P.pt[lane] = 0u;
        const int sr = s / A.w, sc = s - sr * A.w;
        L.put(0u, ((uint32_t)(sr >> 3) << 16) | (uint32_t)(sc >> 3), 1ull << ((sr & 7) * 8 + (sc & 7)));
        const bool hand_over = A.big_cap != 0u;
        if (has_log) {
            const bool direct = (log_w & kLogShrunk) != 0u && log_n >= 2u * A.log_walk_tiles;
            if (!direct) rc = walk(A, k, b, thr, sn, cs, L, P, st, lane, own, nullptr, A.log_walk_tiles);
            if (rc != 0) {
                uint32_t pos = 0;
                if (lane == 0) pos = atomicAdd(&A.ctrl[kCtrlNRewalk], 1u);
                pos = (uint32_t)__shfl((int)pos, 0);
                if (pos < kBigCap) {
                    if (lane == 0) A.rewalk_list[pos] = k;
                    return;
                }
            }
        }
        if (rc != 0)
            rc = walk(A, k, b, thr, sn, cs, L, P, st, lane, own, nullptr, hand_over ? t1_tiles : 0xFFFFFFFFu,
                      hand_over ? A.wide_tiles : 0xFFFFFFFFu, hand_over ? A.wide_front : 0xFFFFFFFFu);
    }
    if (rc != 0 && A.big_cap == 0u && A.quiet != 0u) {
        if (lane == 0) {
            A.flags[k] = kFlagIncomplete;
            atomicMin(&A.ctrl[kCtrlBarrier], k);
            atomicAdd(&A.ctrl[kCtrlQuietMiss], 1u);
        }
        return;
    }
    if (rc != 0 && A.big_cap != 0u) {
        uint32_t pos = 0;
        if (lane == 0) pos = atomicAdd(&A.ctrl[kCtrlNBig], 1u);
        pos = (uint32_t)__shfl((int)pos, 0);
        if (pos < A.big_cap) {
            if (lane == 0) {
                big_list[pos] = k;
                A.tier[k] = 1;
                atomicAdd(&A.ctrl[kCtrlBigTotal], 1u);
            }
            uint32_t* hb = A.handover + (size_t)pos * kFloodHandWords;
            const uint32_t nt = skip_first ? 0u : st.ntiles, nr = skip_first ? 0u : st.tail - st.head;
            if (lane == 0) {
                hb[0] = nt;
                hb[1] = nr;
                hb[2] = st.steps;
            }
            for (uint32_t i = (uint32_t)lane; i < nt; i += 64u) {
                const uint32_t slot = L.ord[i];
                hb[kHandTable + 3u * i] = L.hk[slot];
                hb[kHandTable + 3u * i + 1u] = L.hv0[slot];
                hb[kHandTable + 3u * i + 2u] = L.hv1[slot];
            }
            for (uint32_t i = (uint32_t)lane; i < nr; i += 64u) {
                const uint32_t j = (st.head + i) & (uint32_t)(LdsStore::kRingN - 1);
                hb[kHandRing + 3u * i] = L.rt[j];
                hb[kHandRing + 3u * i + 1u] = L.rlo[j];
                hb[kHandRing + 3u * i + 2u] = L.rhi[j];
            }
            return;
        }
        if (skip_first) {
            for (int i = lane; i < LdsStore::kHashN; i += 64) L.hk[i] = 0u;
            P.pt[lane] = 0u;
            const int sr = s / A.w, sc = s - sr * A.w;
            L.put(0u, ((uint32_t)(sr >> 3) << 16) | (uint32_t)(sc >> 3), 1ull << ((sr & 7) * 8 + (sc & 7)));
            rc = walk(A, k, b, thr, sn, cs, L, P, st, lane, own);
        }
        if (rc != 0 && A.giant_hold != 0u && (A.giant_step != 0u || k != uni(A.ctrl[kCtrlLowest]))) {
            if (lane == 0) {
                A.tier[k] = (uint8_t)(A.tier[k] | 5u);
                A.flags[k] = kFlagIncomplete;
                atomicMin(&A.ctrl[kCtrlBarrier], k);
                atomicAdd(&A.ctrl[kCtrlGiants], 1u);
            }
            return;
        }
    }
    stamp_footprint(A, k, L, st, lane);
    if (rc == 0 && st.ntiles >= A.log_min_tiles && st.ntiles <= A.log_max_len && k < A.log_seeds && uni(A.log_len[k]) == 0u)
        save_log(A, k, L, st.ntiles, lane);
    if (rc != 0) {
        uint32_t slab = 0;
        if (lane == 0) slab = atomicAdd(&A.ctrl[kCtrlSlabs], 1u);
        slab = (uint32_t)__shfl((int)slab, 0);
        if (slab < A.n_slabs) {
            uint32_t gen = 0;
            if (lane == 0) atomicAdd(&A.ctrl[kCtrlSlabTotal], 1u);
            if (lane == 0) gen = atomicAdd(&A.ctrl[kCtrlGen], 1u) + 1u;
            gen = (uint32_t)__shfl((int)gen, 0);
            SlabStore G{A.slab_ring + (size_t)slab * A.slab_ring_cap, A.slab_hash + (size_t)slab * A.slab_hash_cap * 2,
                        A.slab_ring_cap, A.slab_hash_cap, gen};
            for (uint32_t i = st.head; i != st.tail; ++i) {
                uint32_t t;
                uint64_t m;
                L.get(i, t, m);
                G.put(i, t, m);
            }
            for (int i = 0; i < LdsStore::kHashN; ++i) {
                const uint32_t key = L.hk[i];
                if (key) {
                    uint32_t slot;
                    uint64_t v0;
                    (void)G.lookup(key - 1u, slot, v0);
                    G.update(slot, key - 1u, ((uint64_t)L.hv1[i] << 32) | L.hv0[i]);
                }
            }
            rc = walk(A, k, b, thr, sn, cs, G, P, st, lane, own);
        }
        if (rc != 0 && lane == 0) {
            A.flags[k] = kFlagIncomplete;
            atomicMin(&A.ctrl[kCtrlBarrier], k);
        }
    }
    if (lane == 0) {
        A.count[k] = st.cnt;
        if (st.blocked) A.blocked[k] = 1u;
        A.flags[k] |= st.steps << 8;
    }
}

template <bool kRest>
__device__ __forceinline__ void explore_body(const FloodArgs& A, const BinTrig& trig, uint32_t* __restrict__ big_list, uint32_t first) {
    __shared__ uint32_t s_ring[3][kRingT];
    __shared__ uint32_t s_hash[3][kHashT];
    __shared__ uint32_t s_pend[2][kPend];
    __shared__ uint8_t s_ord[kHashT];
#ifdef LR_LDS_PAD
    __shared__ uint32_t s_pad[LR_LDS_PAD / 4];
    asm volatile("" ::"v"(&s_pad[threadIdx.x]) : "memory");
#endif
    const int lane = threadIdx.x & 63;
    if (giant_pending(A)) return;
    const uint32_t* __restrict__ act = act_now(A);
    const uint32_t n_act = uni(A.ctrl[kCtrlNAct]), window = uni(A.ctrl[kCtrlWindow]);
    const uint32_t t1_usual = uni(A.ctrl[kCtrlBigSeen]) != 0u ? kRegionalTiles : 0xFFFFFFFFu;
    const bool tier2_full = A.giant_hold != 0u && A.big_cap != 0u && uni(A.ctrl[kCtrlNBig]) >= A.big_cap;
    const uint32_t lowest = uni(A.ctrl[kCtrlLowest]);
    LdsStore L{s_ring[0], s_ring[1], s_ring[2], s_hash[0], s_hash[1], s_hash[2], s_ord};
    Pending P{s_pend[0], s_pend[1]};
    if (!kRest) {
        const uint32_t ai = uni(blockIdx.x);
        if (ai >= n_act) return;
        const bool fwd = A.no_rest != 0u && n_act > gridDim.x;
        const uint32_t k = uni(act[!fwd ? n_act - 1u - ai : ai]);
        if (k >= window) return;
        const uint32_t t1_tiles = (tier2_full && k != lowest) ? min(t1_usual, kFullTiles) : t1_usual;
        explore_seed(A, trig, k, L, P, big_list, lane, t1_tiles);
    } else {
        for (uint32_t ai = first + uni(blockIdx.x); ai < n_act; ai += gridDim.x) {
            const uint32_t k = uni(act[n_act - 1u - ai]);
            if (k >= window) continue;
            const uint32_t t1_tiles = (tier2_full && k != lowest) ? min(t1_usual, kFullTiles) : t1_usual;
            explore_seed(A, trig, k, L, P, big_list, lane, t1_tiles);
        }
    }
}
__global__ __launch_bounds__(64) __attribute__((amdgpu_waves_per_eu(4, 8))) void flood_explore_kernel(
    FloodArgs A, BinTrig trig, uint32_t* __restrict__ big_list) {
    explore_body<false>(A, trig, big_list, 0u);
}
__global__ __launch_bounds__(64) __attribute__((amdgpu_waves_per_eu(4, 8))) void flood_explore_rest_kernel(
    FloodArgs A, BinTrig trig, uint32_t* __restrict__ big_list, uint32_t first) {
    explore_body<true>(A, trig, big_list, first);
}

#ifndef LR_TEAM_WAVES
#define LR_TEAM_WAVES 8
#endif
constexpr int kTeamWaves = LR_TEAM_WAVES;
#ifndef LR_TEAM_RING
#define LR_TEAM_RING 1024
#endif
constexpr int kRingTeam = LR_TEAM_RING;
#ifndef LR_TEAM_GRID
#define LR_TEAM_GRID 512
#endif
constexpr uint32_t kTeamGrid = LR_TEAM_GRID;
constexpr uint32_t kVoidTile = 0xFFFFFFFFu;

struct TeamShared {
    uint32_t tail, end, ntiles, blocked, overflow, cnt, steps, pad;
    uint32_t blocker, pad2;
};
__device__ __forceinline__ uint32_t lds_now(const uint32_t* p) {
    return __hip_atomic_load(p, __ATOMIC_RELAXED, __HIP_MEMORY_SCOPE_WORKGROUP);
}

struct TeamStore {
    static constexpr int kHashShift = 32 - __builtin_ctz((unsigned)kHashBig);
    uint32_t* rt;
    uint32_t* rlo;
    uint32_t* rhi;
    uint32_t* hk;
    uint32_t* hv0;
    uint32_t* hv1;
    uint16_t* ord;
    TeamShared* sh;
    __device__ uint32_t hash_limit() const { return kHashBig * 3 / 4; }
    __device__ void get(uint32_t i, uint32_t& tile, uint64_t& m) const {
        const uint32_t j = i & (kRingTeam - 1);
        tile = uni(rt[j]);
        m = uni64(rlo[j], rhi[j]);
    }
    __device__ bool lookup(uint32_t tile, uint32_t& slot, uint64_t& V) const {
        const uint32_t key = tile + 1u;
        const bool first_lane = (threadIdx.x & 63u) == 0u;
// ... 183 lines not shown
            if (uni(lds_now(&sh->overflow)) != 0u) break;
            const TileFetch cur = fetch_tile<0>(A, S, i, lr, lc, rx, ry, ring_lane, fw, G, own);
            ++steps;
            const uint32_t tile = cur.tile;
            uint64_t Am = cur.inside & m_ne(cur.dm & bin_bit, 0u) & m_gt_f(directional(cur.dx, cur.dy, sn, cs), thr);
            uint64_t Rg = cur.rinside & m_ne(cur.rdm & bin_bit, 0u) & m_gt_f(directional(cur.rdx, cur.rdy, sn, cs), thr);
            if (own) {
                Am |= cur.inside & m_eq(cur.lab, k);
                Rg |= cur.rinside & m_eq(cur.rlab, k);
            }
            uint64_t R = cur.entry & Am;
            if (R != 0ull) {
                const uint64_t reach = lane_of(Am) ? nbr : 0ull;
                for (;;) {
                    const uint64_t R1 = m_ne64(R & reach, 0ull);
                    R = m_ne64(R1 & reach, 0ull);
                    if (R == R1) break;
                }
                const uint64_t New = R & ~cur.V;
                if (New != 0ull) {
                    uint64_t was = 0ull;
                    if (lane == 0) was = S.add_walked(cur.slot, New);
                    const uint64_t first_here = New & ~uni64(was);
                    if (first_here != 0ull) {
                        const uint64_t H = Rg & m_ne64(first_here & adj, 0ull);
                        if (H != 0ull) team_push8(S, tile, H, lane, pc);
                    }
                }
            }
            if (lane == 0) S.mark_processed(i);
        }
        __syncthreads();
        if (threadIdx.x == 0) sh->end = sh->tail;
        __syncthreads();
        const uint32_t ne = sh->end;
        if (sh->overflow != 0u || ++levels > kMaxSteps) {
            rc = 1;
            break;
        }
        if (ne == ge) break;
        gb = ge;
        ge = ne;
    }
    *begin_out = gb;
    *steps_out = steps;
    return rc;
}

constexpr size_t kTeamLdsBytes = (size_t)(3 * kRingTeam + 3 * kHashBig + 2 * kPend) * 4 + (size_t)kHashBig * 2 + sizeof(TeamShared);
__global__ __launch_bounds__(64 * kTeamWaves) void flood_explore_team_kernel(FloodArgs A, BinTrig trig,
                                                                             const uint32_t* __restrict__ big_list) {
    extern __shared__ uint32_t s_team[];
    const int lane = threadIdx.x & 63, wave = (int)uni(threadIdx.x >> 6);
    if (uni(A.ctrl[kCtrlNAct]) == 0u || giant_pending(A)) return;
    const uint32_t n_big_raw = uni(A.ctrl[kCtrlNBig]);
    const uint32_t n_big = n_big_raw < A.big_cap ? n_big_raw : A.big_cap;
    uint32_t* ring = s_team;
    uint32_t* hash = ring + 3 * kRingTeam;
    uint32_t* pend = hash + 3 * kHashBig;
    uint16_t* ord = reinterpret_cast<uint16_t*>(pend + 2 * kPend);
    TeamShared* sh = reinterpret_cast<TeamShared*>(reinterpret_cast<char*>(ord) + (size_t)kHashBig * 2);
    TeamStore S{ring, ring + kRingTeam, ring + 2 * kRingTeam, hash, hash + kHashBig, hash + 2 * kHashBig, ord, sh};
    for (uint32_t ai = uni(blockIdx.x); ai < n_big; ai += gridDim.x) {
        const uint32_t k = uni(big_list[ai]);
        const int s = (int)uni((uint32_t)A.seed_idx[k]);
        const int b = (int)uni((uint32_t)A.seed_bin[k]);
        const float thr = __uint_as_float(uni(__float_as_uint(A.seed_thr[k])));
        const float sn = trig.st[b], cs = trig.ct[b];
        const uint32_t seed_label = uni(A.label[s]);
        const bool own = seed_label == k;
        if (seed_label < kMarkBit && !own) continue;
        if (!own && !(((uni((uint32_t)A.dmask[s]) >> b) & 1u) &&
                      directional(__uint_as_float(uni(__float_as_uint(A.dx[s]))), __uint_as_float(uni(__float_as_uint(A.dy[s]))), sn, cs) > thr)) {
            if (threadIdx.x == 0) A.flags[k] = kFlagSelfFail;
            continue;
        }
        if (A.giant_hold != 0u && k != uni(A.ctrl[kCtrlLowest]) &&
            ((k >= (uni(A.ctrl[kCtrlNSeeds]) >> 2) && giants_many(A.ctrl, A.giant_many)) || giants_all(A.ctrl))) {
            if (threadIdx.x == 0) {
                A.flags[k] = kFlagIncomplete;
                atomicMin(&A.ctrl[kCtrlBarrier], k);
            }
            continue;
        }
        const uint32_t* hb = A.handover + (size_t)ai * kFloodHandWords;
        const uint32_t h_recs = min(uni(hb[1]), kHandRecs);
        uint32_t begin = 0u, my_steps = 0u;
        __syncthreads();
        for (int i = (int)threadIdx.x; i < kHashBig; i += 64 * kTeamWaves) {
            S.hk[i] = 0u;
            S.hv0[i] = 0u;
            S.hv1[i] = 0u;
        }
        const uint32_t h_tiles = min(uni(hb[0]), kHandTiles);
        const uint32_t first_level = h_recs ? h_recs : 1u;
        __syncthreads();
        if (h_recs) {
            for (uint32_t t = threadIdx.x; t < h_tiles; t += 64u * kTeamWaves) {
                const uint32_t key = hb[kHandTable + 3u * t];
                uint32_t hs = (key * 2654435761u) >> TeamStore::kHashShift;
                while (atomicCAS(&S.hk[hs], 0u, key) != 0u) hs = (hs + 1u) & (uint32_t)(kHashBig - 1);
                S.hv0[hs] = hb[kHandTable + 3u * t + 1u];
                S.hv1[hs] = hb[kHandTable + 3u * t + 2u];
                S.ord[t] = (uint16_t)hs;
            }
            for (uint32_t t = threadIdx.x; t < h_recs; t += 64u * kTeamWaves) {
                S.rt[t] = hb[kHandRing + 3u * t];
                S.rlo[t] = hb[kHandRing + 3u * t + 1u];
                S.rhi[t] = hb[kHandRing + 3u * t + 2u];
            }
        }
        if (threadIdx.x == 0) {
            if (!h_recs) {
                const int sr = s / A.w, sc = s - sr * A.w;
                const uint64_t m = 1ull << ((sr & 7) * 8 + (sc & 7));
                S.rt[0] = ((uint32_t)(sr >> 3) << 16) | (uint32_t)(sc >> 3);
                S.rlo[0] = (uint32_t)m;
                S.rhi[0] = (uint32_t)(m >> 32);
            }
            sh->tail = first_level;
            sh->end = first_level;
            sh->ntiles = h_recs ? h_tiles : 0u;
            sh->blocked = 0u;
            sh->blocker = 0xFFFFFFFFu;
            sh->overflow = 0u;
            sh->cnt = 0u;
            sh->steps = h_recs ? hb[2] : 0u;
        }
        __syncthreads();
        int rc = team_walk(A, k, b, thr, sn, cs, S, lane, wave, own, first_level, A.team_tiles, &begin, &my_steps);
        WalkState st{0u, 0u, 0u, 0u, false, 0u, 0u};
        uint32_t px = 0u;
        bool in_slab = false;
        if (rc != 0 && A.giant_hold != 0u && (A.giant_step != 0u || k != uni(A.ctrl[kCtrlLowest]))) {
            if (threadIdx.x == 0) {
                A.tier[k] = (uint8_t)(A.tier[k] | 4u);
                A.flags[k] = kFlagIncomplete;
                atomicMin(&A.ctrl[kCtrlBarrier], k);
                atomicAdd(&A.ctrl[kCtrlGiants], 1u);
                atomicAdd(&A.ctrl[kCtrlTeamGiants], 1u);
                atomicAdd(&A.ctrl[kCtrlTeamDone], 1u);
            }
            continue;
        }
        if (rc != 0) {
            if (threadIdx.x == 0) {
                const uint32_t slab = atomicAdd(&A.ctrl[kCtrlSlabs], 1u);
// ... 119 lines not shown
__device__ __forceinline__ uint32_t rw_order(uint32_t x) { return x * 0x9E3779B1u; }
__device__ __forceinline__ void rw_union(uint32_t* par, uint32_t a, uint32_t b) {
    for (;;) {
        uint32_t ra = rw_find(par, a), rb = rw_find(par, b);
        if (ra == rb) return;
        if (rw_order(ra) < rw_order(rb)) {
            const uint32_t t = ra;
            ra = rb;
            rb = t;
        }
        if (atomicCAS(&par[ra], ra, rb) == ra) return;
    }
}
constexpr int kRewalkTiles = 256;
constexpr uint32_t kRewalkGrid = 2048;
constexpr int kRewalkThreads = 256;
constexpr int kRewalkTilesBig = 2048, kRewalkThreadsBig = 1024;
template <int kTiles>
constexpr size_t rewalk_lds_bytes() {
    return (size_t)kTiles * 3 * 4 + (size_t)2 * kTiles * 4 + (size_t)2 * kTiles * 3 * 4 + (size_t)4 * kTiles * 4 + (size_t)2 * kTiles * 2 +
           (size_t)kTiles * 2 + (size_t)kTiles;
}
#ifdef LR_REWALK_TIMING
__device__ unsigned long long g_rewalk_timing[8];
#define RW_TICK(i)                                            \
    if (threadIdx.x == 0) {                                   \
        const uint64_t t_ = __builtin_amdgcn_s_memtime();     \
        atomicAdd(&g_rewalk_timing[i], (unsigned long long)(t_ - tlast)); \
        tlast = t_;                                           \
    }
#else
#define RW_TICK(i)
#endif
template <int kThreads, int kTiles>
__global__ __launch_bounds__(kThreads) void flood_rewalk_kernel(FloodArgs A, const uint32_t* __restrict__ list, uint32_t min_len) {
    constexpr int kNodes = 2 * kTiles, kHash = 2 * kTiles, kWaves = kThreads / 64, kEdges = 4 * kTiles;
    static_assert(kNodes <= 65536, "node pairs are packed into 32 bits");
    constexpr int kHashShift = 32 - __builtin_ctz((unsigned)kHash);
    extern __shared__ uint32_t s_rw[];
    uint32_t* tid = s_rw;
    uint32_t* mlo = tid + kTiles;
    uint32_t* mhi = mlo + kTiles;
    uint32_t* hkey = mhi + kTiles;
    uint32_t* nlo = hkey + kHash;
    uint32_t* nhi = nlo + kNodes;
    uint32_t* par = nhi + kNodes;
    uint32_t* edge = par + kNodes;
    uint16_t* hidx = reinterpret_cast<uint16_t*>(edge + kEdges);
    uint16_t* tfirst = hidx + kHash;
    uint8_t* tcomp = reinterpret_cast<uint8_t*>(tfirst + kTiles);
    __shared__ uint32_t s_nnodes, s_over, s_blocked, s_cnt, s_seed_node, s_nout, s_nedges;
    const int lane = threadIdx.x & 63, wave = (int)uni(threadIdx.x >> 6);
    const int lr = lane >> 3, lc = lane & 7;
    if (uni(A.ctrl[kCtrlNAct]) == 0u || giant_pending(A)) return;
    const uint32_t n_list = min(uni(A.ctrl[kCtrlNRewalk]), kBigCap);
    const uint32_t window = uni(A.ctrl[kCtrlWindow]);
    for (uint32_t ai = uni(blockIdx.x); ai < n_list; ai += gridDim.x) {
        const uint32_t k = uni(list[ai]);
        if (k >= window) continue;
        const uint32_t n = uni(A.log_len[k]) & ~kLogShrunk;
        if (n < min_len || n > (uint32_t)kTiles) continue;
        const uint32_t s = uni((uint32_t)A.seed_idx[k]);
        const uint32_t seed_label = uni(A.label[s]);
        const bool own = seed_label == k;
        if (seed_label < kMarkBit && !own) continue;
        const uint32_t mine = kMarkBit | k;
        uint32_t* rec = A.log_buf + (size_t)uni(A.log_off[k]) * 3u;
        __syncthreads();
#ifdef LR_REWALK_TIMING
        uint64_t tlast = __builtin_amdgcn_s_memtime();
        if (threadIdx.x == 0) {
            atomicAdd(&g_rewalk_timing[0], 1ull);
            atomicAdd(&g_rewalk_timing[1], (unsigned long long)n);
        }
#endif
        for (uint32_t i = threadIdx.x; i < n; i += kThreads) {
            tid[i] = rec[3u * i];
            mlo[i] = rec[3u * i + 1u];
            mhi[i] = rec[3u * i + 2u];
        }
        for (uint32_t i = threadIdx.x; i < (uint32_t)kHash; i += kThreads) hkey[i] = 0u;
        if (threadIdx.x == 0) {
            s_nnodes = 0u;
            s_over = 0u;
            s_blocked = 0u;
            s_cnt = 0u;
            s_seed_node = 0xFFFFFFFFu;
            s_nout = 0u;
            s_nedges = 0u;
        }
        __syncthreads();
        RW_TICK(2)
        for (uint32_t i0 = (uint32_t)wave * kRwBatch; i0 < n; i0 += (uint32_t)kWaves * kRwBatch) {
            uint32_t lab[kRwBatch];
            bool in[kRwBatch];
#pragma unroll
            for (int j = 0; j < (int)kRwBatch; ++j) {
                const uint32_t i = i0 + (uint32_t)j;
                lab[j] = 0u;
                in[j] = false;
                if (i < n) {
                    const uint32_t tile = tid[i];
                    const uint64_t V = ((uint64_t)mhi[i] << 32) | mlo[i];
                    in[j] = (V >> lane) & 1ull;
                    if (in[j]) lab[j] = A.label[(size_t)((tile >> 16) * 8 + lr) * A.w + ((tile & 0xFFFFu) * 8 + lc)];
                }
            }
#pragma unroll
            for (int j = 0; j < (int)kRwBatch; ++j) {
                const uint32_t i = i0 + (uint32_t)j;
                const uint64_t M = __ballot(in[j] && (lab[j] >= kMarkBit || lab[j] == k));
                if (i < n && lane == 0) {
                    mlo[i] = (uint32_t)M;
                    mhi[i] = (uint32_t)(M >> 32);
                }
            }
        }
        __syncthreads();
        RW_TICK(3)
        const uint32_t seed_tile = ((s / (uint32_t)A.w) >> 3) << 16 | ((s % (uint32_t)A.w) >> 3);
// ... 192 lines not shown
                rec[3u * pos + 1u] = (uint32_t)V;
                rec[3u * pos + 2u] = (uint32_t)(V >> 32);
            }
            my_cnt += (uint32_t)__popcll(V);
        }
        if (my_cnt) atomicAdd(&s_cnt, my_cnt);
        __syncthreads();
        RW_TICK(6)
        bool foreign = false;
        for (uint32_t i0 = (uint32_t)wave * kRwBatch; i0 < n; i0 += (uint32_t)kWaves * kRwBatch) {
            uint32_t old[kRwBatch];
#pragma unroll
            for (int j = 0; j < (int)kRwBatch; ++j) {
                old[j] = kLabelFree;
                const uint32_t i = i0 + (uint32_t)j;
                if (i < n) {
                    const uint32_t tile = tid[i];
                    const uint64_t V = ((uint64_t)mhi[i] << 32) | mlo[i];
                    if ((V >> lane) & 1ull) {
                        const size_t q = (size_t)((tile >> 16) * 8 + lr) * A.w + ((tile & 0xFFFFu) * 8 + lc);
                        old[j] = atomicMin(&A.label[q], mine);
                        A.dirty[q >> 8] = 1;
                    }
                }
            }
#pragma unroll
            for (int j = 0; j < (int)kRwBatch; ++j) {
                if (old[j] > mine) {
                    if (old[j] != kLabelFree) A.blocked[old[j] & ~kMarkBit] = 1u;
                } else if (old[j] < mine && old[j] >= kMarkBit) {
                    foreign = true;
                }
            }
        }
        if (__ballot(foreign) && lane == 0) s_blocked = 1u;
        __syncthreads();
        RW_TICK(7)
        if (threadIdx.x == 0) {
            A.count[k] = s_cnt;
            A.log_len[k] = s_nout | kLogShrunk;
            if (s_blocked) A.blocked[k] = 1u;
            A.flags[k] |= n << 8;
            atomicAdd(&A.ctrl[kCtrlLogWalks], 1u);
        }
    }
}

__global__ __launch_bounds__(64) void flood_partial_commit_kernel(FloodArgs A, uint8_t* __restrict__ dmask_rw) {
    __shared__ uint32_t s_ring[3][kRingT];
    __shared__ uint32_t s_hash[3][kHashT];
    __shared__ uint32_t s_pend[2][kPend];
    __shared__ uint8_t s_ord[kHashT];
    const int lane = threadIdx.x & 63;
    if (giant_pending(A)) return;
    const uint32_t* __restrict__ act = act_now(A);
    const uint32_t n_act = uni(A.ctrl[kCtrlNAct]), window = uni(A.ctrl[kCtrlWindow]), barrier = uni(A.ctrl[kCtrlBarrier]);
    LdsStore L{s_ring[0], s_ring[1], s_ring[2], s_hash[0], s_hash[1], s_hash[2], s_ord};
    Pending P{s_pend[0], s_pend[1]};
    for (uint32_t ai = uni(blockIdx.x); ai < n_act; ai += gridDim.x) {
        const uint32_t k = uni(act[ai]);
        if (k >= window || k >= barrier) continue;
        const uint32_t fl = uni(A.flags[k]);
        if (uni(A.count[k]) == 0u || uni(A.blocked[k]) == 0u || (fl & (kFlagIncomplete | kFlagSelfFail))) continue;
        const int s = (int)uni((uint32_t)A.seed_idx[k]);
        const uint32_t seed_label = uni(A.label[s]);
        if (seed_label != (kMarkBit | k) && seed_label != k) continue;
        for (int i = lane; i < LdsStore::kHashN; i += 64) L.hk[i] = 0u;
        P.pt[lane] = 0u;
        const int sr = s / A.w, sc = s - sr * A.w;
        L.put(0u, ((uint32_t)(sr >> 3) << 16) | (uint32_t)(sc >> 3), 1ull << ((sr & 7) * 8 + (sc & 7)));
        WalkState st{0u, 1u, 0u, 0u, false, 0u, 0u};
        (void)walk<LdsStore, 1>(A, k, 0, 0.f, 0.f, 0.f, L, P, st, lane, false, dmask_rw);
    }
}

__device__ __forceinline__ bool seed_commits(const FloodArgs& A, uint32_t k, uint32_t barrier) {
    const uint32_t fl = A.flags[k];
    return A.count[k] > 0u && A.blocked[k] == 0u && !(fl & (kFlagIncomplete | kFlagSelfFail)) && k < barrier;
}

__global__ __launch_bounds__(256) void flood_commit_pixels_kernel(FloodArgs A, uint32_t* __restrict__ label, size_t npix,
                                                                  uint8_t* __restrict__ dmask) {
    const uint32_t* __restrict__ ctrl = A.ctrl;
    if (ctrl[kCtrlNAct] == 0u || ctrl[kCtrlGiantStep] != 0u) return;
    const uint32_t barrier = ctrl[kCtrlBarrier];
    const int lane = threadIdx.x & 63;
    const uint32_t n_runs = (uint32_t)((npix + 255) >> 8);
    for (uint32_t run = blockIdx.x * 4u + (threadIdx.x >> 6); run < n_runs; run += gridDim.x * 4u) {
        if (uni((uint32_t)A.dirty[run]) == 0u) continue;
        if (lane == 0) A.dirty[run] = 0;
        const size_t i0 = ((size_t)run << 8) + (size_t)lane * 4;
        uint32_t v[4] = {kLabelFree, kLabelFree, kLabelFree, kLabelFree};
        if (i0 + 3 < npix) {
            const uint4 q = *reinterpret_cast<const uint4*>(label + i0);
            v[0] = q.x, v[1] = q.y, v[2] = q.z, v[3] = q.w;
        } else {
            for (int j = 0; j < 4; ++j)
                if (i0 + j < npix) v[j] = label[i0 + j];
        }
#pragma unroll
        for (int j = 0; j < 4; ++j) {
            if (v[j] >= kMarkBit && v[j] != kLabelFree) {
                const uint32_t k = v[j] & ~kMarkBit;
                const bool committed = seed_commits(A, k, barrier);
                label[i0 + j] = committed ? k : kLabelFree;
                if (committed) dmask[i0 + j] = 0;
            }
        }
    }
}

__device__ __forceinline__ void flood_report(uint32_t* host_progress, uint32_t rounds, uint32_t n_left, bool stalled, bool want_giant,
                                             uint32_t giants_done, bool huge, bool calm = false) {
    const unsigned long long w = (unsigned long long)(n_left & 0x1FFFFFFFu) | ((unsigned long long)(stalled ? 1u : 0u) << 29) |
                                 ((unsigned long long)(want_giant ? 1u : 0u) << 30) | ((unsigned long long)(huge ? 1u : 0u) << 31) |
                                 ((unsigned long long)min(rounds, 0xFFFu) << 32) | ((unsigned long long)min(giants_done, 0xFFFFu) << 44) |
                                 ((unsigned long long)(calm ? 1u : 0u) << 60) | (1ull << 63);
    __hip_atomic_store(reinterpret_cast<unsigned long long*>(host_progress), w, __ATOMIC_RELEASE, __HIP_MEMORY_SCOPE_SYSTEM);
}

__device__ void flood_advance(uint32_t* __restrict__ ctrl, uint32_t win_shift, uint32_t* host_progress, uint32_t giant_step,
                              uint32_t giant_many) {
    const uint32_t n_act = ld_agent(&ctrl[kCtrlNAct]);
    if (n_act == 0u) {
        if (host_progress)
// ... 625 lines not shown
                        }
                    }
                    const uint64_t m = __ballot(claim);
                    if (claim)
                        __hip_atomic_store(&queue[tail + __popcll(m & ((1ull << lane) - 1ull))], q, __ATOMIC_RELAXED,
                                           __HIP_MEMORY_SCOPE_AGENT);
                    tail += (int)__popcll(m);
                    head += nsrc;
                }
                size = tail;
                __builtin_amdgcn_fence(__ATOMIC_ACQ_REL, "workgroup");
                for (int i = lane; i < tail; i += 64) {
                    const int p = __hip_atomic_load(&queue[i], __ATOMIC_RELAXED, __HIP_MEMORY_SCOPE_AGENT);
                    __hip_atomic_store(&label[p], k, __ATOMIC_RELAXED, __HIP_MEMORY_SCOPE_AGENT);
                }
                __builtin_amdgcn_fence(__ATOMIC_ACQ_REL, "workgroup");
            }
        }
        if (lane == 0) seed_size[k] = size;
    }
}

}


static void flood_debug_round(const FloodBuffers& B, const FloodFrame& F, uint32_t n_seeds, hipStream_t s) {
    uint32_t ctrl[kFloodCtrlWords];
    (void)hipStreamSynchronize(s);
    (void)hipMemcpy(ctrl, B.ctrl, sizeof(ctrl), hipMemcpyDeviceToHost);
    const uint32_t n_act = ctrl[kCtrlNAct];
    if (n_act == 0 || ctrl[kCtrlGiantStep] != 0u) return;
    const uint32_t* act = (ctrl[kCtrlRounds] & 1u) ? B.act_b : B.act_a;
    std::vector<uint32_t> cnt(n_seeds), blk(n_seeds), flg(n_seeds), actv(n_act);
    (void)hipMemcpy(flg.data(), B.flags, n_seeds * sizeof(uint32_t), hipMemcpyDeviceToHost);
    (void)hipMemcpy(actv.data(), act, n_act * sizeof(uint32_t), hipMemcpyDeviceToHost);
    (void)hipMemcpy(cnt.data(), B.count, n_seeds * sizeof(uint32_t), hipMemcpyDeviceToHost);
    (void)hipMemcpy(blk.data(), B.blocked, n_seeds * sizeof(uint32_t), hipMemcpyDeviceToHost);
#ifdef LR_REWALK_TIMING
    {
        unsigned long long t[8], z[8] = {0, 0, 0, 0, 0, 0, 0, 0};
        (void)hipMemcpyFromSymbol(t, HIP_SYMBOL(g_rewalk_timing), sizeof(t));
        (void)hipMemcpyToSymbol(HIP_SYMBOL(g_rewalk_timing), z, sizeof(z));
        if (t[0] > 0)
            std::fprintf(stderr, "  re-walks from logs: %llu seeds, %llu records; s_memtime ticks per seed: records in %.0f, pixels %.0f, components %.0f, "
                         "unions %.0f, footprint %.0f, stamps %.0f\n", t[0], t[1], (double)t[2] / t[0], (double)t[3] / t[0], (double)t[4] / t[0],
                         (double)t[5] / t[0], (double)t[6] / t[0], (double)t[7] / t[0]);
    }
#endif
#ifdef LR_WALK_TIMING
    {
        unsigned long long t[8], z[8] = {0, 0, 0, 0, 0, 0, 0, 0};
        (void)hipMemcpyFromSymbol(t, HIP_SYMBOL(g_walk_timing), sizeof(t));
        (void)hipMemcpyToSymbol(HIP_SYMBOL(g_walk_timing), z, sizeof(z));
        if (t[1] > 0)
            std::fprintf(stderr, "  walks of more than 100 steps: %llu, %llu steps (%llu of them on a known tile); s_memtime ticks per step: "
                         "wait for pixels %.1f, closure %.1f, table %.1f, push %.1f, pop + issue %.1f\n",
                         t[0], t[1], t[7], (double)t[2] / t[1], (double)t[3] / t[1], (double)t[4] / t[1], (double)t[5] / t[1],
                         (double)t[6] / t[1]);
    }
#endif
    unsigned long long tsteps = 0, tpx = 0;
    uint32_t mxs = 0, mxk = 0, nb = 0;
    for (uint32_t i = 0; i < n_act; ++i) {
        const uint32_t kk = actv[i], st_ = flg[kk] >> 8;
        tsteps += st_;
        tpx += cnt[kk];
        nb += blk[kk] != 0;
        if (st_ > mxs) {
            mxs = st_;
            mxk = kk;
        }
    }
    {
        unsigned long long steps_commit = 0, steps_other = 0;
        uint32_t longest_commit = 0, longest_other = 0, n_commit = 0;
        for (uint32_t i = 0; i < n_act; ++i) {
            const uint32_t kk = actv[i], st_ = flg[kk] >> 8;
            if (cnt[kk] > 0 && blk[kk] == 0 && !(flg[kk] & (kFlagIncomplete | kFlagSelfFail)) && kk < ctrl[kCtrlBarrier]) {
                steps_commit += st_;
                n_commit += 1;
                longest_commit = std::max(longest_commit, st_);
            } else {
                steps_other += st_;
                longest_other = std::max(longest_other, st_);
            }
        }
        std::fprintf(stderr, "  %u committing seeds: %llu steps, longest %u; blocked or dying seeds: %llu steps, longest %u\n",
                     n_commit, steps_commit, longest_commit, steps_other, longest_other);
    }
    {
        const size_t npix = (size_t)F.w * F.h;
        std::vector<uint32_t> lab(npix);
        std::vector<int32_t> sidx(n_seeds);
        (void)hipMemcpy(lab.data(), F.label, npix * sizeof(uint32_t), hipMemcpyDeviceToHost);
        (void)hipMemcpy(sidx.data(), F.seed_idx, n_seeds * sizeof(int32_t), hipMemcpyDeviceToHost);
        auto commits = [&](uint32_t kk) {
            return cnt[kk] > 0 && blk[kk] == 0 && !(flg[kk] & (kFlagIncomplete | kFlagSelfFail)) && kk < ctrl[kCtrlBarrier];
        };
        unsigned long long steps_dying = 0, steps_dying_own = 0;
        uint32_t n_dying = 0, n_own = 0, longest = 0;
        for (uint32_t i = 0; i < n_act; ++i) {
            const uint32_t kk = actv[i], st_ = flg[kk] >> 8;
            if (commits(kk)) continue;
            const uint32_t v = lab[(size_t)sidx[kk]];
            if (v >= kMarkBit && v != kLabelFree) {
                const uint32_t j = v & ~kMarkBit;
// ... 11 lines not shown
        std::fprintf(stderr, "  %u seeds die with this round (a committing seed takes their pixel): %llu steps, longest %u; "
                     "%u seeds have their own pixel stamped by a lower seed: %llu steps\n",
                     n_dying, steps_dying, longest, n_own, steps_dying_own);
    }
    {
        const uint32_t edges[8] = {8, 16, 32, 48, 64, 128, 192, 0xFFFFFFFFu};
        uint32_t hist[8] = {0, 0, 0, 0, 0, 0, 0, 0}, long_lo = 0xFFFFFFFFu, nlong_strong = 0;
        for (uint32_t i = 0; i < n_act; ++i) {
            const uint32_t kk = actv[i], st_ = flg[kk] >> 8;
            for (int b = 0; b < 8; ++b)
                if (st_ <= edges[b]) {
                    hist[b]++;
                    break;
                }
            if (st_ > 64) {
                long_lo = std::min(long_lo, kk);
                if (kk < n_seeds / 10 * 8) nlong_strong++;
            }
        }
        std::fprintf(stderr, "  steps<=8:%u <=16:%u <=32:%u <=48:%u <=64:%u <=128:%u <=192:%u more:%u; lowest seed with >64 steps: %u; such seeds among the strongest 80%%: %u\n",
                     hist[0], hist[1], hist[2], hist[3], hist[4], hist[5], hist[6], hist[7], long_lo, nlong_strong);
    }
    std::fprintf(stderr,
                 "flood round %u: active %u, %llu px walked in %llu steps, longest walk %u steps (%u px, seed %u), "
                 "blocked %u, barrier %u, slabs %u\n",
                 ctrl[kCtrlRounds] + 1, n_act, tpx, tsteps, mxs, cnt[mxk], mxk, nb, ctrl[kCtrlBarrier],
                 ctrl[kCtrlSlabs]);
    {
        uint8_t t = 0;
        uint32_t ll = 0, full[kCtrlWords];
        (void)hipMemcpy(&t, B.tier + mxk, 1, hipMemcpyDeviceToHost);
        if (B.log_len && mxk < B.log_seeds) (void)hipMemcpy(&ll, B.log_len + mxk, 4, hipMemcpyDeviceToHost);
        (void)hipMemcpy(full, B.ctrl, sizeof(full), hipMemcpyDeviceToHost);
        std::fprintf(stderr, "  ... that seed: tier marks %u (1 outgrew the first tier, 4 held as a giant), log %u records%s; window %u, lowest active %u, lowest held %u, log records handed out %u of %u\n",
                     (unsigned)t, ll & 0x7FFFFFFFu, (ll >> 31) ? " (cut down)" : "", full[kCtrlWindow], full[kCtrlLowest], full[kCtrlGiantLow], full[kCtrlLogTotal], B.log_cap);
    }
}

namespace {

const bool g_flood_debug = std::getenv("LIBRECTIFY_FLOOD_DEBUG") != nullptr;

FloodArgs flood_args(const FloodBuffers& B, const FloodFrame& F, bool use_big) {
    FloodArgs A;
    A.dx = F.dx;
    A.dy = F.dy;
    A.dmask = F.dmask;
    A.w = F.w;
    A.h = F.h;
    A.tiles_x = (F.w + 7) / 8;
    A.seed_idx = F.seed_idx;
    A.seed_bin = F.seed_bin;
    A.seed_thr = F.seed_thr;
    A.label = F.label;
    A.blocked = B.blocked;
    A.count = B.count;
    A.flags = B.flags;
    A.tier = B.tier;
    A.ctrl = B.ctrl;
    A.dirty = B.dirty;
    A.slab_ring = (uint4*)B.slab_ring;
    A.slab_hash = (uint4*)B.slab_hash;
    A.n_slabs = B.n_slabs;
    A.slab_ring_cap = B.slab_ring_cap;
    A.slab_hash_cap = B.slab_hash_cap;
    A.no_rest = 0u;
    A.next_reach = 0xFFFFFFFFu;
    A.win_shift = 2u;
    const uint32_t big_cap = B.big_cap_override ? B.big_cap_override : kBigCap;
    A.big_cap = use_big ? big_cap : 0u;
    A.team_tiles = B.team_tile_cap ? B.team_tile_cap : (B.giant_hold ? kTeamTiles : 0xFFFFFFFFu);
    A.giant_many = B.giant_hold ? kGiantMany : 0u;
    A.wide_tiles = 0xFFFFFFFFu;
    A.wide_front = 6u;
    A.blk = B.giant_hold ? B.blk : nullptr;
    A.handover = B.handover;
    A.rewalk_list = B.rewalk_list;
    const bool logs = B.rewalk_logs && B.log_buf && B.log_off && B.log_len && B.rewalk_list;
    A.log_min_tiles = logs ? (B.log_min_tiles > 0 ? (uint32_t)B.log_min_tiles : kLogMinTiles) : 0xFFFFFFFFu;
    A.log_walk_tiles = B.log_walk_tiles > 0 ? (uint32_t)B.log_walk_tiles : kLogWalkTiles;
    A.log_sweep = B.log_sweep ? 1u : 0u;
    A.host_progress = (B.jit_first > 0 && !g_flood_debug) ? B.host_progress : nullptr;
    static const bool mirror_off = std::getenv("LIBRECTIFY_FLOOD_MIRROR") && std::atoi(std::getenv("LIBRECTIFY_FLOOD_MIRROR")) == 0;
    A.host_ctrl = (A.host_progress && !mirror_off) ? B.host_ctrl : nullptr;
    A.quiet = 0u;
    A.giant_hold = B.giant_hold ? 1u : 0u;
    A.log_max_len = (B.rewalk_big && use_big) ? (uint32_t)kRewalkTilesBig : (uint32_t)kRewalkTiles;
    A.log_seeds = logs ? B.log_seeds : 0u;
    A.log_off = B.log_off;
    A.log_len = B.log_len;
    A.log_buf = B.log_buf;
    A.log_cap = B.log_cap;
    A.act_a = B.act_a;
    A.act_b = B.act_b;
    A.giant_mask = reinterpret_cast<unsigned long long*>(B.giant_mask);
    A.giant_parent = B.giant_parent;
    A.giant_step = (B.giant_hold && B.giant_step && B.giant_mask && B.giant_parent && use_big) ? 1u : 0u;
    return A;
}


constexpr uint32_t kFullGridCap = 1u << 18;
constexpr int kRestRounds = 4;
void enqueue_round(const FloodBuffers& B, const FloodFrame& F, const FloodArgs& A0, bool use_big, int index, hipStream_t s,
                   uint32_t known_len = 0xFFFFFFFFu, bool next_known = false) {
    const size_t npix = (size_t)F.w * F.h;
    const int pix_blocks = (int)std::min<size_t>((npix + 255) / 256, 4096);
    const int seed_blocks = (int)std::min<uint32_t>((F.seed_cap + 255) / 256, 256);
    hipEvent_t dbg0 = nullptr, dbg1 = nullptr;
    if (g_flood_debug) {
        (void)hipEventCreate(&dbg0);
        (void)hipEventCreate(&dbg1);
        (void)hipEventRecord(dbg0, s);
    }
    static const int test_grid = std::getenv("LIBRECTIFY_FLOOD_TEST_GRID") ? std::atoi(std::getenv("LIBRECTIFY_FLOOD_TEST_GRID")) : 0;
    auto grid_of = [&](int idx) {
        const int shift = std::min(std::max(idx - (B.win_first_shift > 0 ? 1 : 0), 0), 2);
        uint32_t g = std::max<uint32_t>(std::min<uint32_t>(F.seed_cap, 2048u), F.seed_cap >> shift);
        if (F.seed_cap <= kFullGridCap) g = F.seed_cap;
        if (test_grid > 0 && idx >= kRestRounds) g = std::min<uint32_t>(g, (uint32_t)test_grid);
        return g;
    };
    auto has_rest = [&](int idx) { return idx < kRestRounds && grid_of(idx) < F.seed_cap; };
    const bool exact = known_len < 0xFFFFFFFEu && known_len <= F.seed_cap && !(test_grid > 0 && index >= kRestRounds);
    const uint32_t grid = exact ? std::max<uint32_t>(known_len, 1u) : grid_of(index);
    const bool rest_now = !exact && (has_rest(index) || (known_len != 0xFFFFFFFFu && known_len > grid));
    FloodArgs A = A0;
    A.no_rest = (grid < F.seed_cap && !rest_now && !exact) ? 1u : 0u;
    A.next_reach = (grid_of(index + 1) < F.seed_cap && !has_rest(index + 1) && !next_known) ? grid_of(index + 1) : 0xFFFFFFFFu;
    const bool logs = A.log_min_tiles != 0xFFFFFFFFu;
    A.log_use = (logs && index >= 1) ? 1u : 0u;
    hipLaunchKernelGGL(flood_explore_kernel, dim3(grid), dim3(64), 0, s, A, F.trig, B.big_list);
    if (rest_now)
        hipLaunchKernelGGL(flood_explore_rest_kernel, dim3(1024), dim3(64), 0, s, A, F.trig, B.big_list, grid);
    if (use_big)
        hipLaunchKernelGGL(flood_explore_team_kernel, dim3(std::min<uint32_t>(F.seed_cap, kTeamGrid)), dim3(64 * kTeamWaves),
                           kTeamLdsBytes, s, A, F.trig, B.big_list);
    if (logs && index >= 1)
        hipLaunchKernelGGL((flood_rewalk_kernel<kRewalkThreads, kRewalkTiles>), dim3(std::min<uint32_t>(F.seed_cap, kRewalkGrid)), dim3(kRewalkThreads),
                           rewalk_lds_bytes<kRewalkTiles>(), s, A, B.rewalk_list, 1u);
    if (logs && index >= 1 && A.log_max_len > (uint32_t)kRewalkTiles)
        hipLaunchKernelGGL((flood_rewalk_kernel<kRewalkThreadsBig, kRewalkTilesBig>), dim3(std::min<uint32_t>(F.seed_cap, 1024u)),
                           dim3(kRewalkThreadsBig), rewalk_lds_bytes<kRewalkTilesBig>(), s, A, B.rewalk_list, (uint32_t)kRewalkTiles + 1u);
    if (g_flood_debug) (void)hipEventRecord(dbg1, s);
    if (g_flood_debug) {
        uint32_t n = 0;
        (void)hipStreamSynchronize(s);
        (void)hipMemcpy(&n, F.d_n_seeds, sizeof(n), hipMemcpyDeviceToHost);
        flood_debug_round(B, F, std::min(n, F.seed_cap), s);
        float ms = 0.f;
        (void)hipEventElapsedTime(&ms, dbg0, dbg1);
        std::fprintf(stderr, "  explore kernels of this round: %.1f us\n", ms * 1e3f);
        (void)hipEventDestroy(dbg0);
        (void)hipEventDestroy(dbg1);
    }
    if (B.partial_commits && index < kPartialRounds)
        hipLaunchKernelGGL(flood_partial_commit_kernel, dim3(grid), dim3(64), 0, s, A, const_cast<uint8_t*>(F.dmask));
    hipLaunchKernelGGL(flood_commit_pixels_kernel, dim3(pix_blocks), dim3(256), 0, s, A, F.label, npix,
                       const_cast<uint8_t*>(F.dmask));
    hipLaunchKernelGGL(flood_survivors_kernel, dim3(seed_blocks), dim3(256), 0, s, A, B.state, F.seed_size);
}

void enqueue_giant_step(const FloodBuffers& B, const FloodFrame& F, const FloodArgs& A, hipStream_t s) {
    const uint32_t tiles_x = (uint32_t)(F.w + 7) / 8, tiles_y = (uint32_t)(F.h + 7) / 8;
    const uint32_t strips = ((tiles_x + 7) / 8) * tiles_y, runs = ((tiles_x + 63) / 64) * tiles_y, n_tiles = tiles_x * tiles_y;
    hipEvent_t dbg0 = nullptr, dbg1 = nullptr;
    if (g_flood_debug) {
        (void)hipEventCreate(&dbg0);
        (void)hipEventCreate(&dbg1);
        (void)hipEventRecord(dbg0, s);
    }
    hipLaunchKernelGGL(giant_mask_kernel, dim3(std::min<uint32_t>((strips + 3) / 4, 8192u)), dim3(256), 0, s, A, F.trig);
    hipLaunchKernelGGL(giant_merge_kernel, dim3(std::min<uint32_t>((n_tiles + 255) / 256, 4096u)), dim3(256), 0, s, A);
    hipLaunchKernelGGL(giant_commit_kernel, dim3(std::min<uint32_t>((runs + 3) / 4, 4096u)), dim3(256), 0, s, A, const_cast<uint8_t*>(F.dmask));
    hipLaunchKernelGGL(giant_finish_kernel, dim3(std::min<uint32_t>((F.seed_cap + 255) / 256, 256u)), dim3(256), 0, s, A);
    if (g_flood_debug) {
        uint32_t ctrl[kCtrlWords];
        (void)hipEventRecord(dbg1, s);
        (void)hipStreamSynchronize(s);
        (void)hipMemcpy(ctrl, B.ctrl, sizeof(ctrl), hipMemcpyDeviceToHost);
        float ms = 0.f;
        (void)hipEventElapsedTime(&ms, dbg0, dbg1);
        std::fprintf(stderr, "giant step %u: %.1f us; lowest active seed now %u, lowest held %u, window %u, next step for seed %d\n", ctrl[kCtrlGiantDone],
                     ms * 1e3f, ctrl[kCtrlLowest], ctrl[kCtrlGiantLow], ctrl[kCtrlWindow], (int)ctrl[kCtrlGiantStep] - 1);
        (void)hipEventDestroy(dbg0);
        (void)hipEventDestroy(dbg1);
    }
}

}

int flood_enqueue(const FloodBuffers& B, const FloodFrame& F, FloodProgress* P, uint32_t* h_ctrl, hipStream_t s) {
    P->enqueued = 0;
    P->sizes_known = false;
    P->max_flood = 0;
    P->use_big = B.second_tier && B.second_tier_from_start;
    if (F.seed_cap == 0) return launch_label_init(F.label, (size_t)F.w * F.h, s);
    int win_first_shift = B.win_first_shift, win_growth = B.win_growth;
    if (B.staged_from_start && win_first_shift <= 0) {
        win_first_shift = 2;
        win_growth = 1;
    }
    P->win_growth = win_growth;
    {
        static std::atomic<uint64_t> done_mask{0};
        int dev = 0;
        LR_HIP(hipGetDevice(&dev));
        const uint64_t bit = 1ull << (dev & 63);
        if (!(done_mask.load(std::memory_order_acquire) & bit)) {
            if (hipFuncSetAttribute(reinterpret_cast<const void*>(flood_explore_team_kernel),
// ... 209 lines not shown
```

### librectify_amd/csrc/kernels_seeds.hip

```cpp
#include <algorithm>
#include <cstdlib>
#include <cstring>

#include "common.h"

namespace lramd {
namespace {

__global__ __launch_bounds__(256) void seed_count_kernel(const uint64_t* __restrict__ cand,
                                                         const uint32_t* __restrict__ cand_count,
                                                         const uint32_t* __restrict__ tile_max, int n_tiles, int cand_cap,
                                                         float keep_ratio, float* __restrict__ maxmag,
                                                         uint32_t* __restrict__ tile_pass) {
    __shared__ uint32_t s_red[4];
    const int lane = threadIdx.x & 63, wave = threadIdx.x >> 6;
    uint32_t m = 0;
    for (int i0 = threadIdx.x; i0 < n_tiles; i0 += 256 * 8) {
        uint32_t v[8];
#pragma unroll
        for (int k = 0; k < 8; ++k) {
            const int i = i0 + k * 256;
            v[k] = i < n_tiles ? tile_max[i] : 0u;
        }
#pragma unroll
// ... 220 lines not shown
                __syncthreads();
#pragma unroll
                for (int r = 0; r < 4; ++r) e[r] = LR_KEEP(e[r], o[r], i0 + r, j, k);
            } else if (j >= 4u) {
                const int lm = (int)(j >> 2);
#pragma unroll
                for (int r = 0; r < 4; ++r) {
                    const uint64_t o = shfl_xor_u64(e[r], lm);
                    e[r] = LR_KEEP(e[r], o, i0 + r, j, k);
                }
            } else {
                const bool two = j == 2u;
                const uint64_t o0 = two ? e[2] : e[1], o1 = two ? e[3] : e[0], o2 = two ? e[0] : e[3], o3 = two ? e[1] : e[2];
                e[0] = LR_KEEP(e[0], o0, i0 + 0u, j, k);
                e[1] = LR_KEEP(e[1], o1, i0 + 1u, j, k);
                e[2] = LR_KEEP(e[2], o2, i0 + 2u, j, k);
                e[3] = LR_KEEP(e[3], o3, i0 + 3u, j, k);
            }
        }
    }
#undef LR_KEEP
#pragma unroll
    for (int r = 0; r < 4; ++r)
        if (base + i0 + r < n) keys[base + i0 + r] = e[r];
}

__device__ __forceinline__ uint32_t count_below(const uint64_t* __restrict__ run, uint32_t L, uint32_t valid, uint64_t key) {
    uint32_t lo = 0;
    for (uint32_t sstep = L >> 1; sstep > 0; sstep >>= 1) {
        const uint32_t pos = lo + sstep - 1u;
        const uint64_t v = pos < valid ? run[pos] : ~0ull;
        lo += v < key ? sstep : 0u;
    }
    return lo + ((lo == L - 1u && L - 1u < valid && run[L - 1u] < key) ? 1u : 0u);
}

__global__ __launch_bounds__(256) void seed_merge_kernel(const uint64_t* __restrict__ in, uint64_t* __restrict__ out, uint32_t L,
                                                         uint32_t cap, const uint32_t* __restrict__ n_ptr) {
    const uint32_t g = blockIdx.x * 256 + threadIdx.x;
    const uint32_t n = min(*n_ptr, cap);
    if (g >= n) return;
    const uint32_t r = g / L, i = g - r * L, q = r ^ 1u;
    const uint64_t key = in[g];
    const uint32_t qbase = q * L;
    const uint32_t valid = qbase < n ? min(L, n - qbase) : 0u;
    const uint32_t below = valid ? count_below(in + qbase, L, valid, key) : 0u;
    out[(size_t)(r & ~1u) * L + i + below] = key;
}

__global__ __launch_bounds__(256) void seed_rank_setup_kernel(const uint64_t* __restrict__ keys, const uint32_t* __restrict__ n_ptr,
                                                              uint32_t cap, uint32_t L, const float* __restrict__ dx,
                                                              const float* __restrict__ dy, BinTrig trig, float trace_tolerance,
                                                              int32_t* __restrict__ seed_idx, int32_t* __restrict__ seed_bin,
                                                              float* __restrict__ seed_thr) {
    const uint32_t g = blockIdx.x * 256 + threadIdx.x;
    const uint32_t n = min(*n_ptr, cap);
    if (g >= n) return;
    const uint32_t n_runs = (n + L - 1u) / L;
    const uint32_t mine = g / L;
    const uint64_t key = keys[g];
    uint32_t rank = g - mine * L;
    for (uint32_t q0 = 0; q0 < n_runs; q0 += 8u) {
        uint32_t lo[8], valid[8];
#pragma unroll
        for (int j = 0; j < 8; ++j) {
            const uint32_t q = q0 + (uint32_t)j;
            lo[j] = 0u;
            valid[j] = (q < n_runs && q != mine) ? min(L, n - q * L) : 0u;
        }
        for (uint32_t sstep = L >> 1; sstep > 0; sstep >>= 1) {
            uint64_t v[8];
#pragma unroll
            for (int j = 0; j < 8; ++j) {
                const uint32_t pos = lo[j] + sstep - 1u;
                v[j] = pos < valid[j] ? keys[(size_t)(q0 + (uint32_t)j) * L + pos] : ~0ull;
            }
#pragma unroll
            for (int j = 0; j < 8; ++j) lo[j] += v[j] < key ? sstep : 0u;
        }
#pragma unroll
        for (int j = 0; j < 8; ++j) {
            if (lo[j] == L - 1u && L - 1u < valid[j] && keys[(size_t)(q0 + (uint32_t)j) * L + L - 1u] < key) lo[j] += 1u;
            rank += lo[j];
        }
    }
    const uint32_t low = (uint32_t)key;
    const uint32_t idx = low >> 3;
    const int bin = (int)(low & 7u);
    const float v = directional(dx[idx], dy[idx], trig.st[bin], trig.ct[bin]);
    seed_idx[rank] = (int32_t)idx;
    seed_bin[rank] = bin;
    seed_thr[rank] = (1 - trace_tolerance) * v;
}

}

int launch_seed_order(uint64_t* keys, uint64_t* keys_alt, const uint32_t* n_seeds, uint32_t cap, const float* dx, const float* dy,
                      BinTrig trig, float trace_tolerance, int32_t* seed_idx, int32_t* seed_bin, float* seed_thr, hipStream_t s) {
    if (cap == 0) return 0;
    const uint32_t runs0 = (cap + kRun0 - 1) / kRun0;
    hipLaunchKernelGGL(seed_run_sort_kernel, dim3(runs0), dim3(kRunThreads), 0, s, keys, cap, n_seeds);
    uint32_t L = kRun0, runs = runs0;
    uint64_t* cur = keys;
    uint64_t* nxt = keys_alt;
    while (runs > 1u && (runs > kFinalRuns || (uint64_t)cap * runs > ((uint64_t)4 << 20))) {
        hipLaunchKernelGGL(seed_merge_kernel, dim3((cap + 255) / 256), dim3(256), 0, s, cur, nxt, L, cap, n_seeds);
        std::swap(cur, nxt);
        L *= 2u;
        runs = (runs + 1u) / 2u;
    }
    hipLaunchKernelGGL(seed_rank_setup_kernel, dim3((cap + 255) / 256), dim3(256), 0, s, cur, n_seeds, cap, L, dx, dy, trig,
                       trace_tolerance, seed_idx, seed_bin, seed_thr);
    LR_HIP(hipGetLastError());
    return 0;
}

size_t seeds_temp_bytes(int n_tiles, size_t max_seeds) {
    (void)n_tiles;
    (void)max_seeds;
    return 256;
}

int launch_seed_select(const uint64_t* cand, const uint32_t* cand_count, const uint32_t* tile_max, int n_tiles,
                       int cand_cap, float seed_keep_ratio, float* maxmag, uint32_t* tile_pass, uint32_t* tile_off, uint64_t* keys,
                       uint32_t key_cap, uint32_t* n_seeds, uint32_t frame_tag, hipStream_t s) {
    static const bool fused = !(std::getenv("LIBRECTIFY_SEED_SELECT_FUSED") && std::atoi(std::getenv("LIBRECTIFY_SEED_SELECT_FUSED")) == 0);
    if (fused && frame_tag != 0u && n_tiles > 0) {
        int wgs = std::min(256, (n_tiles + 3) / 4);
        int per_wg = (n_tiles + wgs - 1) / wgs;
        if (per_wg > kSelBands) {
            per_wg = kSelBands;
            wgs = (n_tiles + per_wg - 1) / per_wg;
        }
        wgs = (n_tiles + per_wg - 1) / per_wg;
        hipLaunchKernelGGL(seed_select_kernel, dim3(wgs), dim3(256), 0, s, cand, cand_count, tile_max, n_tiles, cand_cap, per_wg,
                           seed_keep_ratio, maxmag, reinterpret_cast<unsigned long long*>(tile_off), frame_tag, keys, key_cap, n_seeds);
        LR_HIP(hipGetLastError());
        return 0;
    }
    const int blocks = (n_tiles + 3) / 4;
    hipLaunchKernelGGL(seed_count_kernel, dim3(blocks), dim3(256), 0, s, cand, cand_count, tile_max, n_tiles, cand_cap,
                       seed_keep_ratio, maxmag, tile_pass);
    hipLaunchKernelGGL(seed_scan_kernel, dim3(1), dim3(1024), 0, s, tile_pass, n_tiles, tile_off, n_seeds);
    hipLaunchKernelGGL(seed_write_kernel, dim3(blocks), dim3(256), 0, s, cand, cand_count, n_tiles, cand_cap, maxmag,
                       seed_keep_ratio, tile_pass, tile_off, keys, key_cap);
    LR_HIP(hipGetLastError());
    return 0;
}

}
```

Measured before the change: 10390.

## Pack seed records and precompute lane constants to shorten flood kernel prologues

Seed index, bin and threshold are written as one 16-byte record so flood kernels fetch them with a single vector load instead of three scattered loads. Per-lane constants (ring adjacency, neighbour masks, push offsets) come from a constexpr table in device memory rather than being recomputed in each walk. FloodArgs fields are reordered and scalar-register pinning asm is added to batch the control-word loads in kernel prologues. It also adds timing instrumentation and a compile-time cap on the partial-commit grid, and costs an extra seed buffer plus a redundant write in seed setup.

```diff
diff --git a/include/librectify_amd.h b/include/librectify_amd.h
--- a/include/librectify_amd.h
+++ b/include/librectify_amd.h
@@ -165,6 +165,7 @@
     LR_BUF_SEED_THR = 6,
     LR_BUF_MAXMAG = 7,
     LR_BUF_SEED_SIZE = 8,
+    LR_BUF_SEED_REC = 9,
 };
 int lr_download(lr_context* ctx, int buffer_id, void* dst, size_t bytes);
 
diff --git a/librectify_amd/__init__.py b/librectify_amd/__init__.py
--- a/librectify_amd/__init__.py
+++ b/librectify_amd/__init__.py
@@ -66,6 +66,7 @@
 
 
 BUF_DX, BUF_DY, BUF_DMASK, BUF_LABEL, BUF_SEED_IDX, BUF_SEED_BIN, BUF_SEED_THR, BUF_MAXMAG, BUF_SEED_SIZE = range(9)
+BUF_SEED_REC = 9
 T_UPLOAD, T_FILTER, T_SEEDS, T_FLOOD, T_FIT, T_RANSAC, T_TOTAL, T_FILTER_KERNEL, T_COUNT = range(9)
 PIX_U8, PIX_U8X3, PIX_F32 = range(3)
 WARP_PREPARE = 0x100
@@ -520,6 +521,8 @@
             a = np.zeros(self.n_seeds, np.float32)
         elif buf == BUF_MAXMAG:
             a = np.zeros(1, np.float32)
+        elif buf == BUF_SEED_REC:
+            a = np.zeros((self.n_seeds, 4), np.uint32)
         else:
             raise ValueError(buf)
         if a.nbytes:
diff --git a/librectify_amd/csrc/api.cpp b/librectify_amd/csrc/api.cpp
--- a/librectify_amd/csrc/api.cpp
+++ b/librectify_amd/csrc/api.cpp
@@ -480,6 +480,7 @@
             case LR_BUF_SEED_THR: src = ctx->ws.seed_thr; have = (size_t)ctx->n_seeds * 4; break;
             case LR_BUF_MAXMAG: src = ctx->maxmag; have = 4; break;
             case LR_BUF_SEED_SIZE: src = ctx->ws.seed_size; have = (size_t)ctx->n_seeds * 4; break;
+            case LR_BUF_SEED_REC: src = ctx->ws.seed_rec; have = (size_t)ctx->n_seeds * 16; break;
             default: set_error("lr_download: unknown buffer id"); return 1;
         }
         if (buffer_id == LR_BUF_DMASK && ctx->dmask_consumed) {
diff --git a/librectify_amd/csrc/common.h b/librectify_amd/csrc/common.h
--- a/librectify_amd/csrc/common.h
+++ b/librectify_amd/csrc/common.h
@@ -98,7 +98,7 @@
                        int cand_cap, float seed_keep_ratio, float* maxmag, uint32_t* tile_pass, uint32_t* tile_off, uint64_t* keys,
                        uint32_t key_cap, uint32_t* n_seeds, uint32_t frame_tag, hipStream_t s);
 int launch_seed_order(uint64_t* keys, uint64_t* keys_alt, const uint32_t* n_seeds, uint32_t cap, const float* dx, const float* dy,
-                      BinTrig trig, float trace_tolerance, int32_t* seed_idx, int32_t* seed_bin, float* seed_thr, hipStream_t s);
+                      BinTrig trig, float trace_tolerance, int32_t* seed_idx, int32_t* seed_bin, float* seed_thr, uint4* seed_rec, hipStream_t s);
 
 int launch_label_init(uint32_t* label, size_t n, hipStream_t s);
 int launch_flood_ordered(const float* dx, const float* dy, const uint8_t* dmask, int w, int h, const int32_t* seed_idx,
@@ -165,6 +165,7 @@
     uint32_t* label;
     int32_t* seed_size;
     int32_t* queue;
+    const uint4* seed_rec;
 };
 struct FloodProgress {
     int enqueued = 0;
diff --git a/librectify_amd/csrc/context.h b/librectify_amd/csrc/context.h
--- a/librectify_amd/csrc/context.h
+++ b/librectify_amd/csrc/context.h
@@ -42,6 +42,7 @@
     DeviceBuffer<uint64_t> keys_a, keys_b;
     DeviceBuffer<int32_t> seed_idx, seed_bin;
     DeviceBuffer<float> seed_thr;
+    DeviceBuffer<uint4> seed_rec;
     DeviceBuffer<int32_t> seed_size;
     DeviceBuffer<uint32_t> label;
     DeviceBuffer<int32_t> queue;
diff --git a/librectify_amd/csrc/context.hip b/librectify_amd/csrc/context.hip
--- a/librectify_amd/csrc/context.hip
+++ b/librectify_amd/csrc/context.hip
@@ -103,7 +103,7 @@
     s.cap_tiles = 0;
     if (s.dx.grow(cp) || s.dy.grow(cp) || s.dmask.grow(cp + 16) || s.cand.grow((size_t)ct * fg.cand_cap) || s.cand_count.grow(ct) ||
         s.tile_max.grow(ct) || s.tile_pass.grow(ct) || s.tile_off.grow(tile_off_words) || s.keys_a.grow(cp) || s.keys_b.grow(cp) ||
-        s.seed_idx.grow(cp) || s.seed_bin.grow(cp) || s.seed_thr.grow(cp) || s.seed_size.grow(cp) || s.label.grow(cp) ||
+        s.seed_idx.grow(cp) || s.seed_bin.grow(cp) || s.seed_thr.grow(cp) || s.seed_rec.grow(cp) || s.seed_size.grow(cp) || s.label.grow(cp) ||
         s.queue.grow(cp) || s.comp_rank.grow(cp) || s.comp_seed.grow(cp) || s.comp_off.grow(cp + 1) || s.cursor.grow(cp) ||
         s.px_a.grow(cp) || s.px_b.grow(cp) || s.scratch_w.grow(cp) || s.d_lines.grow(cp / 6 + 16) || s.comp_large.grow(cp / 64 + 16))
         return 1;
@@ -156,7 +156,7 @@
     LR_HIP(hipStreamSynchronize(c->stream));
     const size_t cs = c->ws.cap_pix;
     if (grow_into(o.blocked, f.blocked, cs) || grow_into(o.count, f.count, cs) || grow_into(o.flags, f.flags, cs) ||
-        grow_into(o.state, f.state, cs) || grow_into(o.tier, f.tier, cs) || grow_into(o.blk, f.blk, cs) ||
+        grow_into(o.state, f.state, cs) || grow_into(o.tier, f.tier, cs + 4)  || grow_into(o.blk, f.blk, cs) ||
         grow_into(o.act_a, f.act_a, cs) || grow_into(o.act_b, f.act_b, cs) || grow_into(o.ctrl, f.ctrl, kFloodCtrlWords) ||
         grow_into(o.big_list, f.big_list, 8192) || grow_into(o.handover, f.handover, 8192 * kFloodHandWords) ||
         grow_into(o.dirty, f.dirty, cs / 256 + 16) ||
diff --git a/librectify_amd/csrc/frame.hip b/librectify_amd/csrc/frame.hip
--- a/librectify_amd/csrc/frame.hip
+++ b/librectify_amd/csrc/frame.hip
@@ -79,7 +79,7 @@
 
 FloodFrame flood_frame_for(lr_context* c) {
     return FloodFrame{c->ws.dx, c->ws.dy, c->ws.dmask, c->w, c->h, c->ws.seed_idx, c->ws.seed_bin, c->ws.seed_thr,
-                      c->d_counts + kCntSeeds, c->seed_cap, c->trig, c->ws.label, c->ws.seed_size, c->ws.queue};
+                      c->d_counts + kCntSeeds, c->seed_cap, c->trig, c->ws.label, c->ws.seed_size, c->ws.queue, c->ws.seed_rec};
 }
 
 int prepare_frame(lr_context* c, int w, int h) {
@@ -152,7 +152,7 @@
                            c->stream))
         return 1;
     if (launch_seed_order(c->ws.keys_a, c->ws.keys_b, c->d_counts + kCntSeeds, c->seed_cap, c->ws.dx, c->ws.dy, c->trig, kTraceTolerance,
-                          c->ws.seed_idx, c->ws.seed_bin, c->ws.seed_thr, c->stream))
+                          c->ws.seed_idx, c->ws.seed_bin, c->ws.seed_thr, c->ws.seed_rec, c->stream))
         return 1;
     if (c->opt.timing_on) LR_HIP(hipEventRecord(c->ev[2], c->stream));
     return 0;
diff --git a/librectify_amd/csrc/kernels_flood.hip b/librectify_amd/csrc/kernels_flood.hip
--- a/librectify_amd/csrc/kernels_flood.hip
+++ b/librectify_amd/csrc/kernels_flood.hip
@@ -131,55 +131,61 @@
 constexpr uint32_t kHoldRelease = 64;
 constexpr uint32_t kPartialSteps = 16;
 constexpr int kPartialRounds = 3;
+#ifndef LR_PARTIAL_GRID
+#define LR_PARTIAL_GRID 0
+#endif
+constexpr uint32_t kPartialGrid = LR_PARTIAL_GRID;
 constexpr uint32_t kDenseDiv = 12;
 constexpr uint32_t kLogMinTiles = 16;
 constexpr uint32_t kLogWalkTiles = 12;
 
 struct FloodArgs {
+    uint32_t* ctrl;
+    uint32_t* act_a;
+    uint32_t* act_b;
+    const uint4* seed_rec;
+    uint8_t* tier;
+    uint32_t* log_len;
+    uint32_t* label;
+    const uint8_t* dmask;
     const float* dx;
     const float* dy;
-    const uint8_t* dmask;
-    int w, h, tiles_x;
+    int w, h;
+    uint32_t no_rest;
+    uint32_t big_cap;
+    uint32_t giant_hold;
+    uint32_t log_min_tiles;
+    uint32_t log_seeds;
+    uint32_t log_use;
+    uint32_t log_max_len;
+    uint32_t log_walk_tiles;
+    uint32_t quiet;
+    uint32_t giant_step;
+    int tiles_x;
     const int32_t* seed_idx;
     const int32_t* seed_bin;
     const float* seed_thr;
-    uint32_t* label;
     uint32_t* blocked;
     uint32_t* count;
     uint32_t* flags;
-    uint8_t* tier;
-    uint32_t* ctrl;
     uint8_t* dirty;
     uint4* slab_ring;
     uint4* slab_hash;
     uint32_t n_slabs, slab_ring_cap, slab_hash_cap;
     uint32_t win_shift;
-    uint32_t no_rest;
     uint32_t next_reach;
-    uint32_t big_cap;
     uint32_t* handover;
     uint32_t team_tiles;
     uint32_t* blk;
     uint32_t wide_tiles, wide_front;
     uint32_t giant_many;
     uint32_t* rewalk_list;
-    uint32_t log_min_tiles;
-    uint32_t log_walk_tiles;
-    uint32_t log_use;
-    uint32_t log_max_len;
     uint32_t log_sweep;
     uint32_t* host_progress;
     uint32_t* host_ctrl;
-    uint32_t quiet;
-    uint32_t giant_hold;
-    uint32_t log_seeds;
     uint32_t* log_off;
-    uint32_t* log_len;
     uint32_t* log_buf;
     uint32_t log_cap;
-    uint32_t giant_step;
-    uint32_t* act_a;
-    uint32_t* act_b;
     unsigned long long* giant_mask;
     uint32_t* giant_parent;
 };
@@ -247,6 +253,22 @@
 __device__ __forceinline__ bool lane_of(uint64_t mask) { return __builtin_amdgcn_inverse_ballot_w64(mask); }
 __device__ __forceinline__ uint64_t uni64(uint64_t v) { return uni64((uint32_t)v, (uint32_t)(v >> 32)); }
 
+#define LR_PIN3(a, b, c) asm("" : "+s"(a) : "s"(b), "s"(c))
+#define LR_PIN4(a, b, c, d) asm("" : "+s"(a) : "s"(b), "s"(c), "s"(d))
+#define LR_PIN5(a, b, c, d, e) asm("" : "+s"(a) : "s"(b), "s"(c), "s"(d), "s"(e))
+#define LR_PIN6(a, b, c, d, e, f) asm("" : "+s"(a) : "s"(b), "s"(c), "s"(d), "s"(e), "s"(f))
+#define LR_PIN7(a, b, c, d, e, f, g) asm("" : "+s"(a) : "s"(b), "s"(c), "s"(d), "s"(e), "s"(f), "s"(g))
+#define LR_PIN10(a, b, c, d, e, f, g, h, i, j) asm("" : "+s"(a) : "s"(b), "s"(c), "s"(d), "s"(e), "s"(f), "s"(g), "s"(h), "s"(i), "s"(j))
+__device__ __forceinline__ uint32_t walk_args(const FloodArgs& A) {
+    uint32_t token = 0u;
+    asm("" : "+s"(token) : "s"(A.ctrl), "s"(A.act_a), "s"(A.act_b), "s"(A.seed_rec), "s"(A.tier), "s"(A.log_len), "s"(A.label), "s"(A.dmask),
+        "s"(A.dx), "s"(A.dy), "s"(A.w), "s"(A.h), "s"(A.no_rest), "s"(A.big_cap), "s"(A.giant_hold), "s"(A.log_min_tiles),
+        "s"(A.log_seeds), "s"(A.log_use), "s"(A.log_max_len), "s"(A.log_walk_tiles), "s"(A.quiet), "s"(A.giant_step));
+    return token;
+}
+__device__ __forceinline__ uint32_t ld8_word(const uint8_t* p, uint32_t i) { return reinterpret_cast<const uint32_t*>(p)[i >> 2]; }
+__device__ __forceinline__ uint32_t byte_of(uint32_t word, uint32_t i) { return (word >> ((i & 3u) * 8u)) & 0xFFu; }
+
 __device__ __forceinline__ bool giants_many(const uint32_t* ctrl, uint32_t giant_many) {
     const uint32_t n_seeds = uni(ctrl[kCtrlNSeeds]);
     return giant_many != 0u && uni(ctrl[kCtrlStaged]) == 0u && uni(ctrl[kCtrlRounds]) == 0u && n_seeds >= 8192u &&
@@ -267,6 +289,9 @@
     uint32_t steps;
     uint32_t fresh;
     uint32_t blocker = 0xFFFFFFFFu;
+#ifdef LR_WALK_TIMING
+    uint64_t t_first = 0;
+#endif
 };
 
 template <int kRing, int kHash, typename OrdT>
@@ -420,17 +445,21 @@
     bool spread;
     bool dl;
 };
-__device__ __forceinline__ PushLane push_lane(int lane) {
+constexpr PushLane push_lane_values(int lane) {
     const int d = lane & 7;
     const int dy = (d < 2) ? (d == 0 ? -1 : 1) : (d < 4 ? 0 : (d < 6 ? -1 : 1));
     const int dx = (d < 2) ? 0 : ((d & 1) ? 1 : -1);
-    PushLane c;
+    PushLane c{};
     c.off = (uint32_t)(dy * 0x10000 + dx);
     c.shamt = (d < 4) ? 8u * (uint32_t)d : 32u + (uint32_t)(d - 4);
     c.msk = (d < 4) ? 0xFFu : 1u;
     c.sh = (uint32_t)((0x0007383F00070038ull >> (8 * d)) & 0xFFull);
     c.spread = d == 2 || d == 3;
     c.dl = lane < 8;
+    return c;
+}
+__device__ __forceinline__ PushLane push_lane(int lane) {
+    PushLane c = push_lane_values(lane);
     asm volatile("" : "+v"(c.off), "+v"(c.shamt), "+v"(c.msk), "+v"(c.sh));
     return c;
 }
@@ -524,14 +553,14 @@
     if ((H >> 35) & 1ull) send(tile + 0x10001u, 1ull);
 }
 
-__device__ __forceinline__ void ring_xy(int lane, int& rx, int& ry) {
+constexpr void ring_xy(int lane, int& rx, int& ry) {
     const int g = lane >> 3, i = lane & 7;
     rx = (g == 0 || g == 1) ? i : (g == 2 ? -1 : (g == 3 ? 8 : ((i & 1) ? 8 : -1)));
     ry = (g == 0) ? -1 : (g == 1 ? 8 : ((g == 2 || g == 3) ? i : ((i & 2) ? 8 : -1)));
 }
-__device__ __forceinline__ uint64_t ring_adjacency(int lane) {
+constexpr uint64_t ring_adjacency(int lane) {
     if (lane >= 36) return 0ull;
-    int rx, ry;
+    int rx = 0, ry = 0;
     ring_xy(lane, rx, ry);
     uint64_t m = 0ull;
     for (int dy = -1; dy <= 1; ++dy)
@@ -541,7 +570,7 @@
         }
     return m;
 }
-__device__ __forceinline__ uint64_t tile_neighbours(int lane) {
+constexpr uint64_t tile_neighbours(int lane) {
     const int lr = lane >> 3, lc = lane & 7;
     uint64_t m = 0ull;
     for (int dy = -1; dy <= 1; ++dy)
@@ -551,6 +580,65 @@
         }
     return m;
 }
+struct LaneConsts {
+    int rx, ry;
+    bool ring_lane;
+    uint64_t adj;
+    uint64_t nbr;
+    PushLane pc;
+};
+struct LaneTable {
+    uint32_t w[64][12];
+};
+constexpr LaneTable make_lane_table() {
+    LaneTable t{};
+    for (int lane = 0; lane < 64; ++lane) {
+        const uint64_t nbr = tile_neighbours(lane), adj = ring_adjacency(lane);
+        const PushLane c = push_lane_values(lane);
+        int rx = 0, ry = 0;
+        ring_xy(lane, rx, ry);
+        uint32_t* w = t.w[lane];
+        w[0] = (uint32_t)nbr;
+        w[1] = (uint32_t)(nbr >> 32);
+        w[2] = (uint32_t)adj;
+        w[3] = (uint32_t)(adj >> 32);
+        w[4] = c.off;
+        w[5] = c.shamt;
+        w[6] = c.msk;
+        w[7] = c.sh;
+        w[8] = (uint32_t)rx;
+        w[9] = (uint32_t)ry;
+        w[10] = (lane < 36 ? 1u : 0u) | (c.spread ? 2u : 0u) | (c.dl ? 4u : 0u);
+        w[11] = 0u;
+    }
+    return t;
+}
+__device__ const LaneTable g_lane_table = make_lane_table();
+struct LaneWords {
+    uint4 a, b, c;
+};
+__device__ __forceinline__ LaneWords lane_words(int lane) {
+    const uint4* rec = reinterpret_cast<const uint4*>(g_lane_table.w[lane]);
+    return LaneWords{rec[0], rec[1], rec[2]};
+}
+__device__ __forceinline__ LaneConsts lane_consts(const LaneWords& W) {
+    const uint4 a = W.a, b = W.b, c = W.c;
+    LaneConsts K;
+    K.nbr = ((uint64_t)a.y << 32) | a.x;
+    K.adj = ((uint64_t)a.w << 32) | a.z;
+    K.pc.off = b.x;
+    K.pc.shamt = b.y;
+    K.pc.msk = b.z;
+    K.pc.sh = b.w;
+    K.rx = (int)c.x;
+    K.ry = (int)c.y;
+    K.ring_lane = (c.z & 1u) != 0u;
+    K.pc.spread = (c.z & 2u) != 0u;
+    K.pc.dl = (c.z & 4u) != 0u;
+    return K;
+}
+__device__ __forceinline__ LaneConsts lane_consts(int lane) { return lane_consts(lane_words(lane)); }
+
 struct TileFetch {
     uint32_t tile, slot;
     uint64_t entry, V;
@@ -625,6 +713,12 @@
 
 #ifdef LR_WALK_TIMING
 __device__ unsigned long long g_walk_timing[8];
+__device__ unsigned long long g_prologue_timing[64][8];
+struct WalkClock {
+    uint64_t entry, first, walked, stamped;
+};
+#define LR_CLOCK_PARAM , WalkClock& clk
+#define LR_CLOCK_ARG , clk
 #define LR_TICK(i)                                        \
     {                                                     \
         const uint64_t t_ = __builtin_amdgcn_s_memtime(); \
@@ -633,24 +727,26 @@
     }
 #else
 #define LR_TICK(i)
+#define LR_CLOCK_PARAM
+#define LR_CLOCK_ARG
 #endif
 
 template <class Store, int kMode = 0>
 __device__ int walk(const FloodArgs& A, uint32_t k, int b, float thr, float sn, float cs, Store& S, Pending& P,
-                    WalkState& st, int lane, bool own = false, uint8_t* dmask_rw = nullptr, uint32_t tile_cap = 0xFFFFFFFFu,
-                    uint32_t wide_tiles = 0xFFFFFFFFu, uint32_t wide_front = 0xFFFFFFFFu) {
+                    WalkState& st, int lane, const LaneConsts& K, bool own = false, uint8_t* dmask_rw = nullptr,
+                    uint32_t tile_cap = 0xFFFFFFFFu, uint32_t wide_tiles = 0xFFFFFFFFu, uint32_t wide_front = 0xFFFFFFFFu) {
     const uint32_t mine = kMarkBit | k;
     const int lr = lane >> 3, lc = lane & 7;
-    int rx, ry;
-    ring_xy(lane, rx, ry);
-    const bool ring_lane = lane < 36;
-    const uint64_t adj = ring_adjacency(lane);
-    uint64_t nbr = tile_neighbours(lane);
+    const int rx = K.rx, ry = K.ry;
+    const bool ring_lane = K.ring_lane;
+    const uint64_t adj = K.adj;
+    uint64_t nbr = K.nbr;
     asm volatile("" : "+v"(nbr));
     if (st.head == st.tail) return 0;
     const uint32_t tile_limit = min(S.hash_limit(), tile_cap);
     if ((st.tail - st.head) + 8u > S.ring_cap() || st.ntiles + 2u > tile_limit) return 1;
-    const PushLane pc = push_lane(lane);
+    PushLane pc = K.pc;
+    asm volatile("" : "+v"(pc.off), "+v"(pc.shamt), "+v"(pc.msk), "+v"(pc.sh));
     const uint32_t bin_bit = 1u << b;
     Forward fw;
     fw.valid = false;
@@ -658,6 +754,9 @@
     G.off = (uint32_t)(lr * A.w + lc);
     G.roff = (uint32_t)(ry * A.w + rx);
     asm volatile("" : "+v"(G.off), "+v"(G.roff));
+#ifdef LR_WALK_TIMING
+    if (st.t_first == 0) st.t_first = __builtin_amdgcn_s_memtime();
+#endif
     TileFetch cur = fetch_tile<kMode>(A, S, st.head, lr, lc, rx, ry, ring_lane, fw, G, own);
 #ifdef LR_WALK_TIMING
     uint64_t tacc[5] = {0, 0, 0, 0, 0}, tlast = __builtin_amdgcn_s_memtime();
@@ -814,25 +913,40 @@
 }
 
 __device__ __forceinline__ void explore_seed(const FloodArgs& A, const BinTrig& trig, uint32_t k, LdsStore& L, Pending& P,
-                                             uint32_t* __restrict__ big_list, int lane, uint32_t t1_tiles) {
-    const int s = (int)uni((uint32_t)A.seed_idx[k]);
-    const int b = (int)uni((uint32_t)A.seed_bin[k]);
-    const float thr = __uint_as_float(uni(__float_as_uint(A.seed_thr[k])));
-    const float sn = trig.st[b], cs = trig.ct[b];
-    const uint32_t seed_label = A.label[s];
-    const uint32_t seed_mask = A.dmask[s];
-    const float seed_dx = A.dx[s], seed_dy = A.dy[s];
+                                             uint32_t* __restrict__ big_list, int lane, uint32_t t1_tiles, bool staged LR_CLOCK_PARAM) {
+    const uint4 rec = A.seed_rec[k];
+    const uint32_t tier_w = ld8_word(A.tier, k);
+    uint32_t log_w = 0u;
+    if (A.log_min_tiles != 0xFFFFFFFFu && k < A.log_seeds) log_w = A.log_len[k];
+    uint32_t s_u = uni(rec.x);
+    const uint32_t b_u = uni(rec.y), thr_u = uni(rec.z), tier_u = uni(tier_w);
+    log_w = uni(log_w);
+    LR_PIN5(s_u, b_u, thr_u, tier_u, log_w);
+    const LaneConsts K = lane_consts(lane);
+    const int s = (int)s_u, b = (int)b_u;
+    const float thr = __uint_as_float(thr_u);
+    const uint32_t tier = byte_of(tier_u, k);
+    uint32_t seed_label = uni(A.label[s]);
+    const uint32_t mask_u = uni(ld8_word(A.dmask, (uint32_t)s));
+    const uint32_t dx_u = uni(__float_as_uint(A.dx[s])), dy_u = uni(__float_as_uint(A.dy[s]));
+    const uint32_t sn_u = uni(__float_as_uint(trig.st[b])), cs_u = uni(__float_as_uint(trig.ct[b]));
+    LR_PIN6(seed_label, mask_u, dx_u, dy_u, sn_u, cs_u);
+    const float sn = __uint_as_float(sn_u), cs = __uint_as_float(cs_u);
+    const uint32_t seed_mask = byte_of(mask_u, (uint32_t)s);
+    const float seed_dx = __uint_as_float(dx_u), seed_dy = __uint_as_float(dy_u);
     const bool own = seed_label == k;
-    if (seed_label < kMarkBit && !own) return;
-    if ((uni((uint32_t)A.tier[k]) & 8u) != 0u) return;
-    if (!own && !(((seed_mask >> b) & 1) && directional(seed_dx, seed_dy, sn, cs) > thr)) {
+    const bool dead = (seed_label < kMarkBit) & !own;
+    const bool finished = (tier & 8u) != 0u;
+    const bool in_mask = ((seed_mask >> b) & 1u) != 0u, above = directional(seed_dx, seed_dy, sn, cs) > thr;
+    const bool accepts = in_mask & above;
+    if (dead | finished) return;
+    if (!own & !accepts) {
         if (lane == 0) A.flags[k] = kFlagSelfFail;
         return;
     }
     WalkState st{0u, 1u, 0u, 0u, false, 0u, 0u};
     int rc = 1;
-    const bool outgrown = A.big_cap != 0u && (uni((uint32_t)A.tier[k]) & 1u) != 0u && uni(A.ctrl[kCtrlStaged]) == 0u;
-    const uint32_t log_w = (A.log_min_tiles != 0xFFFFFFFFu && k < A.log_seeds) ? uni(A.log_len[k]) : 0u;
+    const bool outgrown = A.big_cap != 0u && (tier & 1u) != 0u && !staged;
     const uint32_t log_n = log_w & ~kLogShrunk;
     const bool has_log = log_n != 0u && log_n <= A.log_max_len && A.log_use != 0u;
     const bool skip_first = outgrown && !has_log;
@@ -844,7 +958,7 @@
         const bool hand_over = A.big_cap != 0u;
         if (has_log) {
             const bool direct = (log_w & kLogShrunk) != 0u && log_n >= 2u * A.log_walk_tiles;
-            if (!direct) rc = walk(A, k, b, thr, sn, cs, L, P, st, lane, own, nullptr, A.log_walk_tiles);
+            if (!direct) rc = walk(A, k, b, thr, sn, cs, L, P, st, lane, K, own, nullptr, A.log_walk_tiles);
             if (rc != 0) {
                 uint32_t pos = 0;
                 if (lane == 0) pos = atomicAdd(&A.ctrl[kCtrlNRewalk], 1u);
@@ -856,7 +970,7 @@
             }
         }
         if (rc != 0)
-            rc = walk(A, k, b, thr, sn, cs, L, P, st, lane, own, nullptr, hand_over ? t1_tiles : 0xFFFFFFFFu,
+            rc = walk(A, k, b, thr, sn, cs, L, P, st, lane, K, own, nullptr, hand_over ? t1_tiles : 0xFFFFFFFFu,
                       hand_over ? A.wide_tiles : 0xFFFFFFFFu, hand_over ? A.wide_front : 0xFFFFFFFFu);
     }
     if (rc != 0 && A.big_cap == 0u && A.quiet != 0u) {
@@ -903,7 +1017,7 @@
             P.pt[lane] = 0u;
             const int sr = s / A.w, sc = s - sr * A.w;
             L.put(0u, ((uint32_t)(sr >> 3) << 16) | (uint32_t)(sc >> 3), 1ull << ((sr & 7) * 8 + (sc & 7)));
-            rc = walk(A, k, b, thr, sn, cs, L, P, st, lane, own);
+            rc = walk(A, k, b, thr, sn, cs, L, P, st, lane, K, own);
         }
         if (rc != 0 && A.giant_hold != 0u && (A.giant_step != 0u || k != uni(A.ctrl[kCtrlLowest]))) {
             if (lane == 0) {
@@ -915,7 +1029,14 @@
             return;
         }
     }
+#ifdef LR_WALK_TIMING
+    clk.first = st.t_first;
+    clk.walked = __builtin_amdgcn_s_memtime();
+#endif
     stamp_footprint(A, k, L, st, lane);
+#ifdef LR_WALK_TIMING
+    clk.stamped = __builtin_amdgcn_s_memtime();
+#endif
     if (rc == 0 && st.ntiles >= A.log_min_tiles && st.ntiles <= A.log_max_len && k < A.log_seeds && uni(A.log_len[k]) == 0u)
         save_log(A, k, L, st.ntiles, lane);
     if (rc != 0) {
@@ -944,7 +1065,7 @@
                     G.update(slot, key - 1u, ((uint64_t)L.hv1[i] << 32) | L.hv0[i]);
                 }
             }
-            rc = walk(A, k, b, thr, sn, cs, G, P, st, lane, own);
+            rc = walk(A, k, b, thr, sn, cs, G, P, st, lane, K, own);
         }
         if (rc != 0 && lane == 0) {
             A.flags[k] = kFlagIncomplete;
@@ -969,28 +1090,66 @@
     asm volatile("" ::"v"(&s_pad[threadIdx.x]) : "memory");
 #endif
     const int lane = threadIdx.x & 63;
-    if (giant_pending(A)) return;
-    const uint32_t* __restrict__ act = act_now(A);
-    const uint32_t n_act = uni(A.ctrl[kCtrlNAct]), window = uni(A.ctrl[kCtrlWindow]);
-    const uint32_t t1_usual = uni(A.ctrl[kCtrlBigSeen]) != 0u ? kRegionalTiles : 0xFFFFFFFFu;
-    const bool tier2_full = A.giant_hold != 0u && A.big_cap != 0u && uni(A.ctrl[kCtrlNBig]) >= A.big_cap;
-    const uint32_t lowest = uni(A.ctrl[kCtrlLowest]);
+#ifdef LR_WALK_TIMING
+    WalkClock clk{__builtin_amdgcn_s_memtime(), 0, 0, 0};
+    const auto clock_out = [&]() {
+        const uint64_t now = __builtin_amdgcn_s_memtime();
+        unsigned long long* t = g_prologue_timing[blockIdx.x & 63u];
+        if (lane == 0) {
+            if (clk.first != 0 && clk.stamped != 0) {
+                atomicAdd(&t[0], 1ull);
+                atomicAdd(&t[1], (unsigned long long)(clk.first - clk.entry));
+                atomicAdd(&t[2], (unsigned long long)(clk.walked - clk.first));
+                atomicAdd(&t[3], (unsigned long long)(clk.stamped - clk.walked));
+            } else {
+                atomicAdd(&t[4], 1ull);
+                atomicAdd(&t[5], (unsigned long long)(now - clk.entry));
+            }
+        }
+        clk = WalkClock{now, 0, 0, 0};
+    };
+#endif
+    const uint32_t args = walk_args(A);
+    const uint32_t* ctrl = A.ctrl;
+    uint32_t c_giant = uni(ctrl[kCtrlGiantStep]);
+    const uint32_t c_rounds = uni(ctrl[kCtrlRounds]), n_act = uni(ctrl[kCtrlNAct]), window = uni(ctrl[kCtrlWindow]),
+                   c_seen = uni(ctrl[kCtrlBigSeen]), c_nbig = uni(ctrl[kCtrlNBig]), lowest = uni(ctrl[kCtrlLowest]),
+                   c_staged = uni(ctrl[kCtrlStaged]);
+    const uint32_t grid = gridDim.x;
+    LR_PIN10(c_giant, c_rounds, n_act, window, c_seen, c_nbig, lowest, c_staged, args, grid);
+    if (c_giant != 0u) return;
+    const uint32_t* __restrict__ act = (c_rounds & 1u) ? A.act_b : A.act_a;
+    const bool staged = c_staged != 0u;
+    const uint32_t t1_usual = c_seen != 0u ? kRegionalTiles : 0xFFFFFFFFu;
+    const bool tier2_full = A.giant_hold != 0u && A.big_cap != 0u && c_nbig >= A.big_cap;
     LdsStore L{s_ring[0], s_ring[1], s_ring[2], s_hash[0], s_hash[1], s_hash[2], s_ord};
     Pending P{s_pend[0], s_pend[1]};
     if (!kRest) {
         const uint32_t ai = uni(blockIdx.x);
+#ifdef LR_WALK_TIMING
+        if (ai >= n_act && lane == 0) {
+            atomicAdd(&g_prologue_timing[blockIdx.x & 63u][6], 1ull);
+            atomicAdd(&g_prologue_timing[blockIdx.x & 63u][7], (unsigned long long)(__builtin_amdgcn_s_memtime() - clk.entry));
+        }
+#endif
         if (ai >= n_act) return;
-        const bool fwd = A.no_rest != 0u && n_act > gridDim.x;
+        const bool fwd = A.no_rest != 0u && n_act > grid;
         const uint32_t k = uni(act[!fwd ? n_act - 1u - ai : ai]);
         if (k >= window) return;
         const uint32_t t1_tiles = (tier2_full && k != lowest) ? min(t1_usual, kFullTiles) : t1_usual;
-        explore_seed(A, trig, k, L, P, big_list, lane, t1_tiles);
+        explore_seed(A, trig, k, L, P, big_list, lane, t1_tiles, staged LR_CLOCK_ARG);
+#ifdef LR_WALK_TIMING
+        clock_out();
+#endif
     } else {
-        for (uint32_t ai = first + uni(blockIdx.x); ai < n_act; ai += gridDim.x) {
+        for (uint32_t ai = first + uni(blockIdx.x); ai < n_act; ai += grid) {
             const uint32_t k = uni(act[n_act - 1u - ai]);
             if (k >= window) continue;
             const uint32_t t1_tiles = (tier2_full && k != lowest) ? min(t1_usual, kFullTiles) : t1_usual;
-            explore_seed(A, trig, k, L, P, big_list, lane, t1_tiles);
+            explore_seed(A, trig, k, L, P, big_list, lane, t1_tiles, staged LR_CLOCK_ARG);
+#ifdef LR_WALK_TIMING
+            clock_out();
+#endif
         }
     }
 }
@@ -1280,8 +1439,11 @@
                                                                              const uint32_t* __restrict__ big_list) {
     extern __shared__ uint32_t s_team[];
     const int lane = threadIdx.x & 63, wave = (int)uni(threadIdx.x >> 6);
-    if (uni(A.ctrl[kCtrlNAct]) == 0u || giant_pending(A)) return;
-    const uint32_t n_big_raw = uni(A.ctrl[kCtrlNBig]);
+    const uint32_t args = walk_args(A);
+    uint32_t c_nact = uni(A.ctrl[kCtrlNAct]);
+    const uint32_t c_giant = uni(A.ctrl[kCtrlGiantStep]), n_big_raw = uni(A.ctrl[kCtrlNBig]);
+    LR_PIN4(c_nact, c_giant, n_big_raw, args);
+    if (c_nact == 0u || c_giant != 0u) return;
     const uint32_t n_big = n_big_raw < A.big_cap ? n_big_raw : A.big_cap;
     uint32_t* ring = s_team;
     uint32_t* hash = ring + 3 * kRingTeam;
@@ -1291,15 +1453,25 @@
     TeamStore S{ring, ring + kRingTeam, ring + 2 * kRingTeam, hash, hash + kHashBig, hash + 2 * kHashBig, ord, sh};
     for (uint32_t ai = uni(blockIdx.x); ai < n_big; ai += gridDim.x) {
         const uint32_t k = uni(big_list[ai]);
-        const int s = (int)uni((uint32_t)A.seed_idx[k]);
-        const int b = (int)uni((uint32_t)A.seed_bin[k]);
-        const float thr = __uint_as_float(uni(__float_as_uint(A.seed_thr[k])));
-        const float sn = trig.st[b], cs = trig.ct[b];
-        const uint32_t seed_label = uni(A.label[s]);
+        const uint32_t* hb = A.handover + (size_t)ai * kFloodHandWords;
+        const uint4 rec = A.seed_rec[k];
+        uint32_t s_u = uni(rec.x);
+        const uint32_t b_u = uni(rec.y), thr_u = uni(rec.z), hb_tiles = uni(hb[0]), hb_recs = uni(hb[1]);
+        LR_PIN5(s_u, b_u, thr_u, hb_tiles, hb_recs);
+        const int s = (int)s_u, b = (int)b_u;
+        const float thr = __uint_as_float(thr_u);
+        uint32_t seed_label = uni(A.label[s]);
+        const uint32_t mask_u = uni(ld8_word(A.dmask, (uint32_t)s));
+        const uint32_t dx_u = uni(__float_as_uint(A.dx[s])), dy_u = uni(__float_as_uint(A.dy[s]));
+        const uint32_t sn_u = uni(__float_as_uint(trig.st[b])), cs_u = uni(__float_as_uint(trig.ct[b]));
+        LR_PIN6(seed_label, mask_u, dx_u, dy_u, sn_u, cs_u);
+        const float sn = __uint_as_float(sn_u), cs = __uint_as_float(cs_u);
         const bool own = seed_label == k;
-        if (seed_label < kMarkBit && !own) continue;
-        if (!own && !(((uni((uint32_t)A.dmask[s]) >> b) & 1u) &&
-                      directional(__uint_as_float(uni(__float_as_uint(A.dx[s]))), __uint_as_float(uni(__float_as_uint(A.dy[s]))), sn, cs) > thr)) {
+        const bool in_mask = ((byte_of(mask_u, (uint32_t)s) >> b) & 1u) != 0u;
+        const bool above = directional(__uint_as_float(dx_u), __uint_as_float(dy_u), sn, cs) > thr;
+        const bool accepts = in_mask & above;
+        if ((seed_label < kMarkBit) & !own) continue;
+        if (!own & !accepts) {
             if (threadIdx.x == 0) A.flags[k] = kFlagSelfFail;
             continue;
         }
@@ -1311,8 +1483,7 @@
             }
             continue;
         }
-        const uint32_t* hb = A.handover + (size_t)ai * kFloodHandWords;
-        const uint32_t h_recs = min(uni(hb[1]), kHandRecs);
+        const uint32_t h_recs = min(hb_recs, kHandRecs);
         uint32_t begin = 0u, my_steps = 0u;
         __syncthreads();
         for (int i = (int)threadIdx.x; i < kHashBig; i += 64 * kTeamWaves) {
@@ -1320,7 +1491,7 @@
             S.hv0[i] = 0u;
             S.hv1[i] = 0u;
         }
-        const uint32_t h_tiles = min(uni(hb[0]), kHandTiles);
+        const uint32_t h_tiles = min(hb_tiles, kHandTiles);
         const uint32_t first_level = h_recs ? h_recs : 1u;
         __syncthreads();
         if (h_recs) {
@@ -1546,20 +1717,24 @@
     __shared__ uint32_t s_nnodes, s_over, s_blocked, s_cnt, s_seed_node, s_nout, s_nedges;
     const int lane = threadIdx.x & 63, wave = (int)uni(threadIdx.x >> 6);
     const int lr = lane >> 3, lc = lane & 7;
-    if (uni(A.ctrl[kCtrlNAct]) == 0u || giant_pending(A)) return;
-    const uint32_t n_list = min(uni(A.ctrl[kCtrlNRewalk]), kBigCap);
-    const uint32_t window = uni(A.ctrl[kCtrlWindow]);
+    uint32_t c_nact = uni(A.ctrl[kCtrlNAct]);
+    const uint32_t c_giant = uni(A.ctrl[kCtrlGiantStep]), c_nrewalk = uni(A.ctrl[kCtrlNRewalk]), window = uni(A.ctrl[kCtrlWindow]);
+    LR_PIN4(c_nact, c_giant, c_nrewalk, window);
+    if (c_nact == 0u || c_giant != 0u) return;
+    const uint32_t n_list = min(c_nrewalk, kBigCap);
     for (uint32_t ai = uni(blockIdx.x); ai < n_list; ai += gridDim.x) {
         const uint32_t k = uni(list[ai]);
         if (k >= window) continue;
-        const uint32_t n = uni(A.log_len[k]) & ~kLogShrunk;
+        uint32_t len_w = uni(A.log_len[k]);
+        const uint32_t s = uni(A.seed_rec[k].x), log_off = uni(A.log_off[k]);
+        LR_PIN3(len_w, s, log_off);
+        const uint32_t n = len_w & ~kLogShrunk;
         if (n < min_len || n > (uint32_t)kTiles) continue;
-        const uint32_t s = uni((uint32_t)A.seed_idx[k]);
         const uint32_t seed_label = uni(A.label[s]);
         const bool own = seed_label == k;
         if (seed_label < kMarkBit && !own) continue;
         const uint32_t mine = kMarkBit | k;
-        uint32_t* rec = A.log_buf + (size_t)uni(A.log_off[k]) * 3u;
+        uint32_t* rec = A.log_buf + (size_t)log_off * 3u;
         __syncthreads();
 #ifdef LR_REWALK_TIMING
         uint64_t tlast = __builtin_amdgcn_s_memtime();
@@ -1858,17 +2033,26 @@
     __shared__ uint32_t s_pend[2][kPend];
     __shared__ uint8_t s_ord[kHashT];
     const int lane = threadIdx.x & 63;
-    if (giant_pending(A)) return;
-    const uint32_t* __restrict__ act = act_now(A);
-    const uint32_t n_act = uni(A.ctrl[kCtrlNAct]), window = uni(A.ctrl[kCtrlWindow]), barrier = uni(A.ctrl[kCtrlBarrier]);
+    const uint32_t args = walk_args(A);
+    const uint32_t* ctrl = A.ctrl;
+    uint32_t c_giant = uni(ctrl[kCtrlGiantStep]);
+    const uint32_t c_rounds = uni(ctrl[kCtrlRounds]), n_act = uni(ctrl[kCtrlNAct]), window = uni(ctrl[kCtrlWindow]),
+                   barrier = uni(ctrl[kCtrlBarrier]);
+    const uint32_t grid = gridDim.x;
+    LR_PIN7(c_giant, c_rounds, n_act, window, barrier, args, grid);
+    if (c_giant != 0u) return;
+    const uint32_t* __restrict__ act = (c_rounds & 1u) ? A.act_b : A.act_a;
+    LaneWords W = lane_words(lane);
     LdsStore L{s_ring[0], s_ring[1], s_ring[2], s_hash[0], s_hash[1], s_hash[2], s_ord};
     Pending P{s_pend[0], s_pend[1]};
-    for (uint32_t ai = uni(blockIdx.x); ai < n_act; ai += gridDim.x) {
+    for (uint32_t ai = uni(blockIdx.x); ai < n_act; ai += grid) {
         const uint32_t k = uni(act[ai]);
         if (k >= window || k >= barrier) continue;
-        const uint32_t fl = uni(A.flags[k]);
-        if (uni(A.count[k]) == 0u || uni(A.blocked[k]) == 0u || (fl & (kFlagIncomplete | kFlagSelfFail))) continue;
-        const int s = (int)uni((uint32_t)A.seed_idx[k]);
+        uint32_t fl = uni(A.flags[k]);
+        const uint32_t cnt = uni(A.count[k]), blocked = uni(A.blocked[k]), s_u = uni(A.seed_rec[k].x);
+        LR_PIN4(fl, cnt, blocked, s_u);
+        if ((cnt == 0u) | (blocked == 0u) | ((fl & (kFlagIncomplete | kFlagSelfFail)) != 0u)) continue;
+        const int s = (int)s_u;
         const uint32_t seed_label = uni(A.label[s]);
         if (seed_label != (kMarkBit | k) && seed_label != k) continue;
         for (int i = lane; i < LdsStore::kHashN; i += 64) L.hk[i] = 0u;
@@ -1876,7 +2060,9 @@
         const int sr = s / A.w, sc = s - sr * A.w;
         L.put(0u, ((uint32_t)(sr >> 3) << 16) | (uint32_t)(sc >> 3), 1ull << ((sr & 7) * 8 + (sc & 7)));
         WalkState st{0u, 1u, 0u, 0u, false, 0u, 0u};
-        (void)walk<LdsStore, 1>(A, k, 0, 0.f, 0.f, 0.f, L, P, st, lane, false, dmask_rw);
+        asm volatile("" : "+v"(W.c.z));
+        const LaneConsts K = lane_consts(W);
+        (void)walk<LdsStore, 1>(A, k, 0, 0.f, 0.f, 0.f, L, P, st, lane, K, false, dmask_rw);
     }
 }
 
@@ -2608,6 +2794,17 @@
         unsigned long long t[8], z[8] = {0, 0, 0, 0, 0, 0, 0, 0};
         (void)hipMemcpyFromSymbol(t, HIP_SYMBOL(g_walk_timing), sizeof(t));
         (void)hipMemcpyToSymbol(HIP_SYMBOL(g_walk_timing), z, sizeof(z));
+        unsigned long long p[64][8], q[8] = {0, 0, 0, 0, 0, 0, 0, 0};
+        (void)hipMemcpyFromSymbol(p, HIP_SYMBOL(g_prologue_timing), sizeof(p));
+        for (int i = 0; i < 64; ++i)
+            for (int j = 0; j < 8; ++j) q[j] += p[i][j];
+        std::memset(p, 0, sizeof(p));
+        (void)hipMemcpyToSymbol(HIP_SYMBOL(g_prologue_timing), p, sizeof(p));
+        if (q[0] + q[4] + q[6] > 0)
+            std::fprintf(stderr, "  first-tier walks that reached their stamps: %llu; mean s_memtime ticks: prologue %.0f, walk %.0f, epilogue %.0f; "
+                         "entries that ended before a first tile: %llu, mean %.0f ticks; workgroups past the list: %llu, mean %.0f ticks\n",
+                         q[0], q[0] ? (double)q[1] / q[0] : 0., q[0] ? (double)q[2] / q[0] : 0., q[0] ? (double)q[3] / q[0] : 0., q[4],
+                         q[4] ? (double)q[5] / q[4] : 0., q[6], q[6] ? (double)q[7] / q[6] : 0.);
         if (t[1] > 0)
             std::fprintf(stderr, "  walks of more than 100 steps: %llu, %llu steps (%llu of them on a known tile); s_memtime ticks per step: "
                          "wait for pixels %.1f, closure %.1f, table %.1f, push %.1f, pop + issue %.1f\n",
@@ -2725,6 +2922,7 @@
     A.seed_idx = F.seed_idx;
     A.seed_bin = F.seed_bin;
     A.seed_thr = F.seed_thr;
+    A.seed_rec = F.seed_rec;
     A.label = F.label;
     A.blocked = B.blocked;
     A.count = B.count;
@@ -2828,7 +3026,8 @@
         (void)hipEventDestroy(dbg1);
     }
     if (B.partial_commits && index < kPartialRounds)
-        hipLaunchKernelGGL(flood_partial_commit_kernel, dim3(grid), dim3(64), 0, s, A, const_cast<uint8_t*>(F.dmask));
+        hipLaunchKernelGGL(flood_partial_commit_kernel, dim3(kPartialGrid ? std::min(grid, kPartialGrid) : grid), dim3(64), 0, s, A,
+                           const_cast<uint8_t*>(F.dmask));
     hipLaunchKernelGGL(flood_commit_pixels_kernel, dim3(pix_blocks), dim3(256), 0, s, A, F.label, npix,
                        const_cast<uint8_t*>(F.dmask));
     hipLaunchKernelGGL(flood_survivors_kernel, dim3(seed_blocks), dim3(256), 0, s, A, B.state, F.seed_size);
diff --git a/librectify_amd/csrc/kernels_seeds.hip b/librectify_amd/csrc/kernels_seeds.hip
--- a/librectify_amd/csrc/kernels_seeds.hip
+++ b/librectify_amd/csrc/kernels_seeds.hip
@@ -296,7 +296,7 @@
                                                               uint32_t cap, uint32_t L, const float* __restrict__ dx,
                                                               const float* __restrict__ dy, BinTrig trig, float trace_tolerance,
                                                               int32_t* __restrict__ seed_idx, int32_t* __restrict__ seed_bin,
-                                                              float* __restrict__ seed_thr) {
+                                                              float* __restrict__ seed_thr, uint4* __restrict__ seed_rec) {
     const uint32_t g = blockIdx.x * 256 + threadIdx.x;
     const uint32_t n = min(*n_ptr, cap);
     if (g >= n) return;
@@ -334,13 +334,15 @@
     const float v = directional(dx[idx], dy[idx], trig.st[bin], trig.ct[bin]);
     seed_idx[rank] = (int32_t)idx;
     seed_bin[rank] = bin;
-    seed_thr[rank] = (1 - trace_tolerance) * v;
+    const float thr = (1 - trace_tolerance) * v;
+    seed_thr[rank] = thr;
+    seed_rec[rank] = make_uint4(idx, (uint32_t)bin, __float_as_uint(thr), 0u);
 }
 
 }
 
 int launch_seed_order(uint64_t* keys, uint64_t* keys_alt, const uint32_t* n_seeds, uint32_t cap, const float* dx, const float* dy,
-                      BinTrig trig, float trace_tolerance, int32_t* seed_idx, int32_t* seed_bin, float* seed_thr, hipStream_t s) {
+                      BinTrig trig, float trace_tolerance, int32_t* seed_idx, int32_t* seed_bin, float* seed_thr, uint4* seed_rec, hipStream_t s) {
     if (cap == 0) return 0;
     const uint32_t runs0 = (cap + kRun0 - 1) / kRun0;
     hipLaunchKernelGGL(seed_run_sort_kernel, dim3(runs0), dim3(kRunThreads), 0, s, keys, cap, n_seeds);
@@ -354,7 +356,7 @@
         runs = (runs + 1u) / 2u;
     }
     hipLaunchKernelGGL(seed_rank_setup_kernel, dim3((cap + 255) / 256), dim3(256), 0, s, cur, n_seeds, cap, L, dx, dy, trig,
-                       trace_tolerance, seed_idx, seed_bin, seed_thr);
+                       trace_tolerance, seed_idx, seed_bin, seed_thr, seed_rec);
     LR_HIP(hipGetLastError());
     return 0;
 }
```

Result: faster. 10580 (median of 6 runs) (+1.8%).
